# FordyceLab/magnify

Hardware: AMD Instinct MI355X
Metric: megapixels/sec through flatfield+segment+ROI-reduce; markers/sec (higher is better)
Workload: dtype u16

## Files before the change

### include/magnify_hip.h

```cpp
#ifndef MAGNIFY_HIP_H
#define MAGNIFY_HIP_H

#include <stddef.h>
#include <stdint.h>

#ifdef __cplusplus
extern "C" {
#endif

#define MG_OK 0
#define MG_EINVAL (-1)
#define MG_ELAUNCH (-2)
#define MG_EIO (-3)

#define MG_U8 0
#define MG_U16 1
#define MG_F32 2
#define MG_F64 3

#define MG_NO_EDGE 100.0f
#define MG_SCORE_SKIPPED (-2.0f)


int mg_version(void);


int mg_circle_points(int r, int four_connected, int32_t* out_rc, int cap);
int mg_disk_halfwidths(int r, int32_t* out);
int mg_cv_disk_halfwidths(int r, int32_t* out);
int mg_perimeter_table(int min_r, int max_r, int32_t* out_rc, double* out_expected, int32_t* out_starts, int cap);


int64_t mg_flatfield_max_scratch_floats(int dtype, int ty, int tx);
int mg_flatfield_bound(const void* d_flat, int flat_dtype, int dtype, int ty, int tx, float* d_scratch,
                       int64_t scratch_floats, void* stream);
int mg_flatfield_max(const void* d_tiles, int dtype, int64_t n_tiles, int n_groups, int ty, int tx,
                     double dark, const void* d_dark, int dark_dtype,
                     double flat, const void* d_flat, int flat_dtype,
                     double* d_max2, float* d_scratch, int64_t scratch_floats, void* stream);

int mg_flatfield_is_identity(int dtype, double dark, const void* d_dark, double flat, const void* d_flat);

int mg_flatfield_apply_stitch(const void* d_tiles, int dtype, int64_t n_planes, int n_tile_rows, int n_tile_cols,
                              int ty, int tx, int overlap, int apply_flatfield, int planes_per_group,
                              double dark, const void* d_dark, int dark_dtype,
                              double flat, const void* d_flat, int flat_dtype,
                              const double* d_max2, void* d_image, double* d_minmax, void* stream);

int mg_plane_minmax(const void* d_src, int dtype, int n_planes, int64_t plane_stride, int h, int w,
                    int64_t row_stride, double* d_minmax, void* stream);

int64_t mg_shading_workspace_bytes(int n, int w);
int64_t mg_shading_offset(int n, int w, int field);
int mg_shading_downsample(const void* d_tiles, int dtype, int64_t n, int ty, int tx, int w, float* d_out, void* stream);
int mg_shading_prepare(void* d_ws, int n, int w, void* stream);
int mg_shading_dct2(void* d_ws, int n, int w, const double* d_in, double* d_out, int inverse, void* stream);
int mg_shading_alm_begin(void* d_ws, int n, int w, int get_darkfield, int max_iterations, double mu, double lam_f,
                         double lam_d, double tol, double norm_f, double b_up, void* stream);
int mg_shading_alm_iterate(void* d_ws, int n, int w, int k, int get_darkfield, void* stream);
int mg_shading_reweight(void* d_ws, int n, int w, double epsilon, void* stream);
int mg_shading_upsample(const double* d_flat_w, const double* d_dark_w, int w, int ty, int tx, double* d_partial,
                        float* d_flat, float* d_dark, void* stream);
int mg_shading_apply_stitch(const void* d_tiles, int dtype, int n_fields, int64_t planes_per_field, int n_tile_rows,
                            int n_tile_cols, int ty, int tx, int overlap, const float* d_flat, const float* d_dark,
                            void* d_image, double* d_minmax, void* stream);


int mg_to_uint8_blur(const void* d_src, int dtype, int n_planes, int64_t plane_stride, int h, int w,
                     int64_t row_stride, const double* d_minmax, uint8_t* d_blur, uint8_t* d_u8, void* stream);

int mg_scharr_hist(const uint8_t* d_blur, int n_planes, int h, int w, int mode, const uint32_t* d_base,
                   uint32_t* d_hist, uint32_t* d_scratch, int64_t scratch_words, void* stream);
int64_t mg_scharr_hist_scratch_words(int n_planes, int h, int w, int mode);

int mg_to_uint8_blur_hist(const void* d_src, int dtype, int n_planes, int64_t plane_stride, int h, int w,
                          int64_t row_stride, const double* d_minmax, uint8_t* d_blur, uint8_t* d_u8, uint32_t* d_hist,
                          uint32_t* d_scratch, int64_t scratch_words, void* stream);
int64_t mg_blur_hist_scratch_words(int n_planes, int h, int w);

int mg_edge_thresholds(const uint32_t* d_hist, int n_planes, const int64_t* ranks4, float gamma_low, float gamma_high,
                       int32_t* d_thresh, float* d_quantiles, int32_t* d_unresolved, int32_t* d_state,
                       uint32_t* d_win_base, void* stream);
int mg_edge_thresholds_window(const uint32_t* d_hist_win, int n_planes, int pass, float gamma_low, float gamma_high,
                              int32_t* d_state, uint32_t* d_win_base, int32_t* d_thresh, float* d_quantiles,
                              int32_t* d_unresolved, void* stream);


int mg_canny_nms(const uint8_t* d_blur, int n_planes, int h, int w, const int32_t* d_thresh, uint32_t* d_weak,
                 uint32_t* d_strong, uint32_t* d_class, int64_t words_per_plane, void* stream);

int mg_canny_hysteresis(const uint32_t* d_weak, uint32_t* d_strong, int64_t words_per_plane, int n_planes, int h,
                        int w, uint32_t* d_changed, const uint8_t* d_flags_in, uint8_t* d_flags_out, void* stream);
int mg_hysteresis_tiles(int h, int w, int* tiles_x, int* tiles_y);

int mg_unpack_bits(const uint32_t* d_bits, int64_t words_per_plane, int n_planes, int64_t n_bits, uint8_t* d_out,
                   void* stream);

int64_t mg_edge_grid_scan_words(int n_planes, int h, int w, int grid);
int mg_edge_grid(const uint32_t* d_edge_bits, int64_t words_per_plane, int n_planes, int h, int w, int grid,
                 int32_t* d_cell_counts, int32_t* d_cell_starts, int32_t* d_num_edges, int32_t* d_coords,
                 int64_t coord_cap, uint64_t* d_scan_state, int32_t* d_edge_totals, int phases, void* stream);

int mg_edge_angles(const uint8_t* d_blur, int n_planes, int h, int w, const int32_t* d_coords, int64_t coord_cap,
                   const int32_t* d_num_edges, float* d_angle, void* stream);


int mg_dedup_layout(int h, int w, int min_r, int max_r, int* n_tile_rows, int* n_tile_cols, int64_t* n_layers,
                    int64_t* bitmap_words);

int mg_candidate_circles(const int32_t* d_coords, int64_t coord_cap, const int32_t* d_cell_starts,
                         const int32_t* d_cell_counts, const int32_t* d_num_edges, int n_planes, int h, int w,
                         int grid, const uint64_t* d_seeds, int64_t num_iter, int min_r, int max_r,
                         uint32_t* d_bitmap, int64_t bitmap_words, float* d_raw, void* stream);

int mg_candidate_keys(const int32_t* d_coords, int64_t coord_cap, const int32_t* d_cell_starts,
                      const int32_t* d_cell_counts, const int32_t* d_num_edges, int n_planes, int h, int w, int grid,
                      const uint64_t* d_seeds, int64_t num_iter, int min_r, int max_r, uint32_t* d_keys, float* d_raw,
                      void* stream);

int mg_keys_to_circles(const uint32_t* d_keys, int64_t num_iter, const int32_t* d_cell_starts,
                       const int32_t* d_cell_counts, const int32_t* d_num_edges, int n_planes, int h, int w, int grid,
                       int min_r, int max_r, uint32_t* d_unique_keys, int64_t circle_cap, int32_t* d_tile_ranges,
                       int32_t* d_num_circles, int32_t* d_layer_starts, int counters_clear, void* stream);

int mg_bitmap_to_circles(uint32_t* d_bitmap, int64_t bitmap_words, int n_planes, int h, int w, int min_r,
                         int max_r, int32_t* d_layer_offsets, int32_t* d_circles, int64_t circle_cap,
                         int32_t* d_num_circles, void* stream);

int mg_score_circles(const float* d_angle, const uint32_t* d_edge_bits, const uint32_t* d_class_bits,
                     int64_t words_per_plane, int n_planes, int h, int w, int32_t* d_circles, int64_t circle_cap,
                     const int32_t* d_layer_offsets, const uint32_t* d_unique_keys, const int32_t* d_tile_ranges,
                     int min_r, int max_r, const int32_t* d_per_rc, const double* d_per_expected,
                     const int32_t* d_per_starts, int per_total, float min_roundness, int write_skipped,
                     int dedup_centres, float* d_scores, int32_t* d_alive, int32_t* d_num_alive, int32_t* d_max_rc,
                     int32_t* d_num_scored, void* stream);

int mg_score_keyed_supported(int min_r, int max_r);
int mg_score_pair_table(uint64_t* out_entries, int cap);
int mg_score_pairs(int r, int32_t* out_rc, int cap);
int mg_score_circles_keyed(const uint8_t* d_blur, const float* d_angle, const uint32_t* d_edge_bits,
                           const uint32_t* d_class_bits, int64_t words_per_plane, int n_planes, int h, int w,
                           int32_t* d_circles, int64_t circle_cap, const uint32_t* d_unique_keys,
                           const int32_t* d_layer_starts, int min_r, int max_r, const int32_t* d_per_rc,
                           const double* d_per_expected, const int32_t* d_per_starts, int per_total,
                           const uint64_t* d_pair_table, float min_roundness, int write_skipped, float* d_scores,
                           int32_t* d_alive, int32_t* d_num_alive, int32_t* d_max_rc, int32_t* d_num_scored,
                           int32_t* d_surv_list, int64_t surv_cap, int32_t* d_num_surv, int counters_clear,
                           void* stream);

int mg_nms_rounds(const int32_t* d_circles, int64_t circle_cap, const float* d_scores, const int32_t* d_alive,
                  const int32_t* d_num_alive, const int32_t* d_max_rc, int n_planes, int min_dist,
                  const int32_t* d_ring_rc, int ring_len, uint64_t* d_grid, int64_t grid_cap, uint8_t* d_state,
                  int32_t* d_undecided, int64_t undecided_stride, int n_rounds, int counters_clear,
                  const uint32_t* d_tie_keys, int64_t max_alive, const int32_t* d_skip, void* stream);

int mg_nms_same_centre(const int32_t* d_circles, int64_t circle_cap, const float* d_scores, const int32_t* d_alive,
                       const int32_t* d_num_alive, const int32_t* d_max_rc, int n_planes, int min_dist, uint64_t* d_grid,
                       int64_t grid_cap, uint8_t* d_state, const uint32_t* d_tie_keys, int64_t max_alive,
                       const int32_t* d_skip, void* stream);

int mg_nms_cleanup(const int32_t* d_circles, int64_t circle_cap, const float* d_scores, const int32_t* d_alive,
                   const int32_t* d_num_alive, const int32_t* d_max_rc, int n_planes, int min_dist,
                   const int32_t* d_ring_rc, int ring_len, uint64_t* d_grid, int64_t grid_cap, uint8_t* d_state,
                   int64_t max_alive, const int32_t* d_skip, void* stream);

int mg_nms_sparse(const int32_t* d_circles, int64_t circle_cap, const float* d_scores, const int32_t* d_alive,
                  const int32_t* d_num_alive, const int32_t* d_max_rc, int n_planes, int min_dist, const uint32_t* d_dbits,
                  uint8_t* d_state, const uint32_t* d_tie_keys, int32_t* d_done, void* stream);
int mg_nms_sparse_max_dist(void);

int mg_collect_circles(const int32_t* d_circles, int64_t circle_cap, const float* d_scores, const int32_t* d_alive,
                       const int32_t* d_num_alive, const uint8_t* d_state, int keep_all, int n_planes,
                       int32_t* d_out, float* d_out_scores, int64_t out_cap, int32_t* d_num_out,
                       int32_t* d_scratch, const uint32_t* d_tie_keys, int counters_clear, void* stream);


int mg_circle_labels(const int32_t* d_beads, int64_t bead_cap, const int32_t* d_num_beads, int n_planes, int h,
                     int w, const int32_t* d_halfwidths, int max_r, int32_t* d_labels, int reset, void* stream);

int mg_roi_gather_reduce(const void* d_image, int dtype, int n_c, int n_t, int h, int w, const int32_t* d_beads,
                         int m, int roi_len, const int32_t* d_labels, void* d_roi, uint8_t* d_fg, uint8_t* d_bg,
                         double* d_sums, int32_t* d_counts, void* stream);

int mg_roi_gather_reduce_batched(const void* d_image, int dtype, int64_t assay_stride, int n_c, int n_t, int h, int w,
                                 const int32_t* d_beads, const int32_t* d_marker_assay,
                                 const int32_t* d_marker_local, int m, int roi_len, const int32_t* d_labels,
                                 void* d_roi, uint8_t* d_fg, uint8_t* d_bg, double* d_sums, int32_t* d_counts,
                                 void* stream);

int mg_counts_to_offsets(const int32_t* d_counts, int n, int cap, int32_t* d_offsets, void* stream);

int mg_marker_table(const int32_t* d_beads, int64_t bead_stride, const int32_t* d_assay_offsets, int n_assays, int m,
                    int assay_offset, const int32_t* d_counts, const double* d_sums, int n_c, int n_t, int t_index,
                    double* d_table, void* stream);

int mg_roi_segment_reduce(const void* d_image, int dtype, int64_t assay_stride, int n_c, int n_t, int h, int w,
                          int time_major, const int32_t* d_beads, int64_t bead_stride, const int32_t* d_assay_offsets,
                          int n_assays, int m, const int32_t* d_order, int roi_len, const int32_t* d_halfwidths, int max_r,
                          void* d_roi, uint8_t* d_fg, uint8_t* d_bg, double* d_sums, int32_t* d_counts, void* stream);

int mg_roi_window_order(const int32_t* d_beads, int64_t bead_stride, const int32_t* d_assay_offsets, int n_assays, int m,
                        int32_t* d_order, void* stream);

int mg_roi_masked_median(const void* d_roi, int dtype, const uint8_t* d_mask, int64_t mask_stride_m,
                         int64_t mask_stride_t, int m, int n_c, int n_t, int roi_len, double* d_median, void* stream);
int mg_roi_masked_median_u16(const uint16_t* d_roi, const uint8_t* d_mask, int m, int n_c, int n_t, int roi_len,
                             double* d_median, void* stream);


int mg_cluster1d_costs(const double* d_sorted_points, int n_points, int n_offsets, int n_clusters,
                       double cluster_length, const double* d_ideal, double penalty, double* d_costs, void* stream);

int mg_button_masks(const int32_t* d_centers, const int32_t* d_radii, int m, int roi_len, int outer_r, int inner_r,
                    const int32_t* d_cv_halfwidths, int hw_stride, int max_table_r, uint8_t* d_fg, uint8_t* d_bg,
                    void* stream);

int mg_masked_sums(const void* d_roi, int dtype, const uint8_t* d_fg, const uint8_t* d_bg, int m, int n_ct,
                   int roi_len, double* d_sums, int32_t* d_counts, void* stream);


int mg_stream_probe(const void* d_src, void* d_dst, int64_t n_bytes, int mode, uint32_t* d_sink, int blocks, void* stream);


int mg_host_read_runs(const int32_t* fds, const int64_t* offsets, const int64_t* nbytes, void* const* dsts, int n,
                      int n_threads, int64_t* failed);
int mg_host_write_runs(const int32_t* fds, const int64_t* offsets, const int64_t* nbytes, void* const* srcs, int n,
                       int n_threads, int64_t* failed);

#ifdef __cplusplus
}
#endif
#endif
```

### magnify_amd/csrc/mg_flatfield.hip

```cpp
#include <math.h>

#include "mg_common.h"

namespace {

template <typename T>
struct VecOf;
template <>
struct VecOf<uint8_t> {
  static constexpr int N = 16;
};
template <>
struct VecOf<uint16_t> {
  static constexpr int N = 8;
};
template <>
struct VecOf<float> {
  static constexpr int N = 4;
};
template <>
struct VecOf<double> {
  static constexpr int N = 2;
};

template <typename T, int N>
__device__ __forceinline__ void load_vec(const T* p, T (&v)[N]) {
  if ((reinterpret_cast<uintptr_t>(p) & 15) == 0) {
    const uint4 raw = *reinterpret_cast<const uint4*>(p);
    __builtin_memcpy(v, &raw, 16);
  } else {
#pragma unroll
    for (int j = 0; j < N; ++j) v[j] = p[j];
  }
}
template <typename T, int N>
__device__ __forceinline__ void store_vec(T* p, const T (&v)[N]) {
  if ((reinterpret_cast<uintptr_t>(p) & 15) == 0) {
    uint4 raw;
    __builtin_memcpy(&raw, v, 16);
    *reinterpret_cast<uint4*>(p) = raw;
  } else {
#pragma unroll
    for (int j = 0; j < N; ++j) p[j] = v[j];
  }
}

typedef uint32_t mg_u32x4 __attribute__((ext_vector_type(4)));
template <typename T, int N>
__device__ __forceinline__ void load_vec16(const T* p, T (&v)[N], bool nt) {
  const mg_u32x4* q = reinterpret_cast<const mg_u32x4*>(p);
  const mg_u32x4 raw = nt ? __builtin_nontemporal_load(q) : *q;
  __builtin_memcpy(v, &raw, 16);
}
template <typename T, int N>
__device__ __forceinline__ void store_vec16(T* p, const T (&v)[N], bool nt) {
  mg_u32x4 raw;
  __builtin_memcpy(&raw, v, 16);
  mg_u32x4* q = reinterpret_cast<mg_u32x4*>(p);
  if (nt) __builtin_nontemporal_store(raw, q);
  else *q = raw;
}

template <typename T>
__device__ __forceinline__ T cast_trunc(double v);
template <>
__device__ __forceinline__ uint8_t cast_trunc<uint8_t>(double v) {
  return (uint8_t)(unsigned int)v;
}
template <>
__device__ __forceinline__ uint16_t cast_trunc<uint16_t>(double v) {
  return (uint16_t)(unsigned int)v;
}
template <>
__device__ __forceinline__ float cast_trunc<float>(double v) {
  return (float)v;
}
template <>
__device__ __forceinline__ double cast_trunc<double>(double v) {
  return v;
}

template <typename T>
struct IsIntegral {
  static constexpr bool value = false;
};
template <>
struct IsIntegral<uint8_t> {
  static constexpr bool value = true;
};
template <>
struct IsIntegral<uint16_t> {
  static constexpr bool value = true;
};

__device__ __forceinline__ void block_atomic_max2(double m1, double m2, double* out) {
  __shared__ double s1[16], s2[16];
  m1 = mg_wave_nanmax(m1);
  m2 = mg_wave_nanmax(m2);
  const int lane = threadIdx.x & 63, wave = threadIdx.x >> 6;
  if (lane == 0) {
    s1[wave] = m1;
    s2[wave] = m2;
  }
  __syncthreads();
  if (threadIdx.x == 0) {
    const int nw = (blockDim.x + 63) >> 6;
    for (int i = 1; i < nw; ++i) {
      m1 = mg_nanmax(m1, s1[i]);
      m2 = mg_nanmax(m2, s2[i]);
    }
    mg_atomic_nanmax(out, m1);
    mg_atomic_nanmax(out + 1, m2);
  }
}

__device__ __forceinline__ bool flat_in_range(double fl) { return fl > 1e-30 && fl < 1e30; }

__device__ __forceinline__ void max_step(double t, double fl, bool fast_m2, double& m1, double& m2) {
  m1 = mg_nanmax(m1, t);
  if (fast_m2) return;
  if (flat_in_range(fl) && t == t) {
    if (t == 0.0) {
      m2 = mg_nanmax(m2, 0.0);
      return;
    }
    const double qa = t * (double)__builtin_amdgcn_rcpf((float)fl);
    if (m2 == m2 && qa < m2 * (1.0 - 1e-6)) return;
  }
  m2 = mg_nanmax(m2, t / fl);
}

template <int N>
__device__ __forceinline__ void load_field(const void* __restrict__ img, int dt, int64_t p, double scalar,
                                           double (&out)[N]) {
  if (!img) {
#pragma unroll
    for (int j = 0; j < N; ++j) out[j] = scalar;
  } else if (dt == MG_F32) {
    const float* f = (const float*)img + p;
    if ((N % 4) == 0 && (reinterpret_cast<uintptr_t>(f) & 15) == 0) {
#pragma unroll
      for (int q = 0; q < N / 4; ++q) {
        const float4 v = reinterpret_cast<const float4*>(f)[q];
        out[4 * q] = v.x;
        out[4 * q + 1] = v.y;
        out[4 * q + 2] = v.z;
        out[4 * q + 3] = v.w;
      }
    } else {
#pragma unroll
      for (int j = 0; j < N; ++j) out[j] = f[j];
    }
  } else {
    const double* d = (const double*)img + p;
#pragma unroll
    for (int j = 0; j < N; ++j) out[j] = d[j];
  }
}

template <typename T>
__global__ __launch_bounds__(256) void k_flatfield_max(const T* __restrict__ tiles, int64_t tiles_per_group,
                                                        int64_t tile_elems, double dark,
                                                        const void* __restrict__ d_dark, int dark_dt, double flat,
                                                        const void* __restrict__ d_flat, int flat_dt,
                                                        double* __restrict__ out) {
  constexpr int N = VecOf<T>::N;
  const int group = blockIdx.y;
  tiles += (int64_t)group * tiles_per_group * tile_elems;
  out += 2 * group;
  const bool fast_m2 = (d_flat == nullptr) && (flat > 0.0);
  double m1 = -INFINITY, m2 = -INFINITY;
  const int64_t nvec = tile_elems / N;
  const int64_t stride = (int64_t)gridDim.x * blockDim.x;
  for (int64_t v = (int64_t)blockIdx.x * blockDim.x + threadIdx.x; v < nvec; v += stride) {
    double dk[N], fl[N];
    load_field<N>(d_dark, dark_dt, v * N, dark, dk);
    load_field<N>(d_flat, flat_dt, v * N, flat, fl);
    for (int64_t g = 0; g < tiles_per_group; ++g) {
      T x[N];
      load_vec<T, N>(tiles + g * tile_elems + v * N, x);
#pragma unroll
      for (int j = 0; j < N; ++j) {
        double t = (double)x[j] - dk[j];
        t = t < 0.0 ? 0.0 : t;
        max_step(t, fl[j], fast_m2, m1, m2);
      }
    }
  }
  for (int64_t p = nvec * N + (int64_t)blockIdx.x * blockDim.x + threadIdx.x; p < tile_elems; p += stride) {
    const double dk = d_dark ? mg_load_f64(d_dark, dark_dt, p) : dark;
    const double fl = d_flat ? mg_load_f64(d_flat, flat_dt, p) : flat;
    for (int64_t g = 0; g < tiles_per_group; ++g) {
      double t = (double)tiles[g * tile_elems + p] - dk;
      t = t < 0.0 ? 0.0 : t;
      max_step(t, fl, fast_m2, m1, m2);
    }
  }
  if (fast_m2) m2 = (m1 == -INFINITY) ? m1 : m1 / flat;
  block_atomic_max2(m1, m2, out);
// ... 125 lines not shown
  constexpr int N = VecOf<T>::N;
  constexpr int UV = 2;
  const int group = blockIdx.y;
  tiles += (int64_t)group * tiles_per_group * tile_elems;
  out += 2 * group;
  const float dk_f = (float)dark;
  uint32_t xmax = 0;
  bool any = false;
  double m2 = -INFINITY;
  float thr = -INFINITY;
  const int64_t nvec = tile_elems / N;
  const int64_t stride = (int64_t)gridDim.x * blockDim.x;
  const int64_t vend = nvec;
  constexpr int PUBLISHERS = 32;
  float gthr = -INFINITY;
  int trip = 0;
  const bool publish = SHARE && blockIdx.x < PUBLISHERS && (int64_t)(blockIdx.x + 1) * blockDim.x <= nvec;
  for (int64_t v0 = (int64_t)blockIdx.x * blockDim.x + threadIdx.x; v0 < nvec; v0 += UV * stride) {
    float rcm[UV];
#pragma unroll
    for (int u = 0; u < UV; ++u) rcm[u] = d_rcmax[min(v0 + u * stride, nvec - 1)];
    if (SHARE && trip > 0 && (trip & (trip - 1)) == 0) {
      const double gm = __hip_atomic_load(out + 1, __ATOMIC_RELAXED, __HIP_MEMORY_SCOPE_AGENT);
      if (gm == gm && gm < 1e30 && gm > -INFINITY) gthr = fmaxf(gthr, (float)gm * (1.0f - 1e-5f));
    }
    any = true;
    for (int64_t g0 = 0; g0 < tiles_per_group; g0 += 4) {
      T x4[UV][4][N];
#pragma unroll
      for (int u = 0; u < UV; ++u)
#pragma unroll
        for (int q = 0; q < 4; ++q)
          load_vec16<T, N>(tiles + min(g0 + q, tiles_per_group - 1) * tile_elems + min(v0 + u * stride, nvec - 1) * N, x4[u][q],
                           true);
#pragma unroll
      for (int u = 0; u < UV; ++u) {
        const int64_t v = v0 + u * stride;
        if (v >= vend) break;
#pragma unroll
        for (int q = 0; q < 4; ++q) {
          if (g0 + q >= tiles_per_group) break;
          uint32_t cm = 0;
#pragma unroll
          for (int j = 0; j < N; ++j) cm = max(cm, (uint32_t)x4[u][q][j]);
          xmax = max(xmax, cm);
          const float tf = fmaxf((float)cm - dk_f, 0.0f);
          if (rcm[u] >= 0.0f && tf * rcm[u] <= fmaxf(thr, gthr)) continue;
          float fl[N];
#pragma unroll
          for (int k4 = 0; k4 < N / 4; ++k4) {
            const float4 f = reinterpret_cast<const float4*>(d_flat + v * N)[k4];
            fl[4 * k4] = f.x, fl[4 * k4 + 1] = f.y, fl[4 * k4 + 2] = f.z, fl[4 * k4 + 3] = f.w;
          }
#pragma unroll
          for (int j = 0; j < N; ++j) {
            const uint32_t xi = (uint32_t)x4[u][q][j];
            const float t_f = fmaxf((float)xi - dk_f, 0.0f);
            const bool in_range = fl[j] > 1e-30f && fl[j] < 1e30f;
            if (in_range && t_f * __builtin_amdgcn_rcpf(fl[j]) <= fmaxf(thr, gthr)) continue;
            double t = (double)xi - dark;
            t = t < 0.0 ? 0.0 : t;
            m2 = mg_nanmax(m2, t / (double)fl[j]);
            thr = (m2 == m2 && m2 < 1e30) ? (float)m2 * (1.0f - 1e-5f) : -INFINITY;
          }
        }
      }
    }
    if (trip == 0 && publish) {
      const double wm = mg_wave_nanmax(m2);
      if ((threadIdx.x & 63) == 0 && wm == wm && wm > -INFINITY) mg_atomic_nanmax(out + 1, wm);
    }
    ++trip;
  }
  double m1 = -INFINITY;
  if (any) {
    m1 = (double)xmax - dark;
    m1 = m1 < 0.0 ? 0.0 : m1;
  }
  block_atomic_max2(m1, m2, out);
}

constexpr int ROWS_PER_BLOCK = 32;

__device__ __forceinline__ double refined_rcp(double fl) {
  if (!flat_in_range(fl)) return 0.0;
  double r = (double)__builtin_amdgcn_rcpf((float)fl);
  r = r * (2.0 - fl * r);
  r = r * (2.0 - fl * r);
  return r;
}

template <typename T>
__device__ __forceinline__ T correct_pixel(double t, double fl, double r, double m1, double m2, double k, bool fast_ok) {
  if (IsIntegral<T>::value && fast_ok && r != 0.0) {
    if (t == 0.0) return (T)0;
    const double v = t * r * k;
    const double fv = floor(v);
    const double fr = v - fv;
    if (fr > 1e-6 && fr < 1.0 - 1e-6 && v < 4.0e9) return (T)(unsigned int)fv;
  }
  double e = t / fl;
  e = e * m1;
  e = e / m2;
  return cast_trunc<T>(e);
}

template <typename T, int N>
__device__ __forceinline__ void correct_chunk(const T (&x)[N], const double (&dk)[N], const double (&fl)[N],
                                              const double (&r)[N], double m1, double m2, double k, bool fast_ok, T (&o)[N]) {
  double t[N];
  bool unsure = !fast_ok || !IsIntegral<T>::value;
#pragma unroll
  for (int j = 0; j < N; ++j) {
    t[j] = (double)x[j] - dk[j];
    t[j] = t[j] < 0.0 ? 0.0 : t[j];
    if (!IsIntegral<T>::value) continue;
    const double v = t[j] * r[j] * k;
    const double fv = floor(v);
    const double fr = v - fv;
    o[j] = (T)(unsigned int)fv;
    unsure |= !((fr > 1e-6 && fr < 1.0 - 1e-6 && v < 4.0e9) || t[j] == 0.0) || r[j] == 0.0;
  }
  if (unsure) {
#pragma unroll
    for (int j = 0; j < N; ++j) {
      double e = t[j] / fl[j];
      e = e * m1;
      e = e / m2;
      o[j] = cast_trunc<T>(e);
    }
  }
}

constexpr int PLANES_PER_BLOCK = 8;

template <typename T, bool APPLY>
__global__ __launch_bounds__(256) void k_apply_stitch(const T* __restrict__ tiles, int n_planes, int n_tr, int n_tc,
                                                       int ty, int tx, int clip, int hy, int hx, int planes_per_group,
                                                       double dark, const void* __restrict__ d_dark, int dark_dt,
                                                       double flat, const void* __restrict__ d_flat, int flat_dt,
                                                       const double* __restrict__ d_max2, T* __restrict__ image,
                                                       double* __restrict__ d_minmax, int rows_per_block) {
  constexpr int N = VecOf<T>::N;
  constexpr int PB = PLANES_PER_BLOCK;
  const int plane0 = blockIdx.z * PB;
  const int np = min(PB, n_planes - plane0);
  const int h_out = n_tr * hy, w_out = n_tc * hx;
  const int ox0 = (blockIdx.x * blockDim.x + threadIdx.x) * N;
  double m1[PB], m2[PB], kk[PB];
  bool fast_ok[PB];
#pragma unroll
  for (int b = 0; b < PB; ++b) {
    m1[b] = 0.0, m2[b] = 1.0, kk[b] = 1.0, fast_ok[b] = false;
    if (APPLY && b < np) {
      const int group = (plane0 + b) / planes_per_group;
      m1[b] = d_max2[2 * group];
      m2[b] = d_max2[2 * group + 1];
      kk[b] = m1[b] / m2[b];
      fast_ok[b] = kk[b] > 0.0 && kk[b] < 1e30 && m1[b] > 0.0 && m1[b] < 1e300 && m2[b] > 0.0 && m2[b] < 1e300;
    }
  }
  double vmin[PB], vmax[PB];
  uint32_t imin[PB], imax[PB];
#pragma unroll
  for (int b = 0; b < PB; ++b) vmin[b] = INFINITY, vmax[b] = -INFINITY, imin[b] = 0xFFFFFFFFu, imax[b] = 0u;
  const int64_t tile_elems = (int64_t)ty * tx;
  if (ox0 < w_out)
  for (int yg = blockIdx.y; yg * rows_per_block < h_out; yg += gridDim.y) {
    const int row_end = min((yg + 1) * rows_per_block, h_out);
    const int tc0 = ox0 / hx;
    const int x0 = ox0 - tc0 * hx + clip;
    const bool one_tile = (ox0 + N <= w_out) && (x0 - clip + N <= hx);
    for (int oy = yg * rows_per_block; oy < row_end; ++oy) {
      const int tr = oy / hy;
      const int y = oy - tr * hy + clip;
      int64_t pix[N], toff[N];
      const int cnt = one_tile ? N : min(N, w_out - ox0);
#pragma unroll
      for (int j = 0; j < N; ++j) {
        const int ox = ox0 + (one_tile ? j : min(j, cnt - 1));
        const int tc = one_tile ? tc0 : ox / hx;
        const int xx = one_tile ? x0 + j : ox - tc * hx + clip;
        pix[j] = (int64_t)y * tx + xx;
        toff[j] = ((int64_t)tr * n_tc + tc) * tile_elems;
      }
      double dk[N], fl[N], rr[N];
      if (APPLY) {
        if (one_tile) {
          load_field<N>(d_dark, dark_dt, pix[0], dark, dk);
          load_field<N>(d_flat, flat_dt, pix[0], flat, fl);
        } else {
#pragma unroll
          for (int j = 0; j < N; ++j) {
            dk[j] = d_dark ? mg_load_f64(d_dark, dark_dt, pix[j]) : dark;
            fl[j] = d_flat ? mg_load_f64(d_flat, flat_dt, pix[j]) : flat;
          }
        }
#pragma unroll
        for (int j = 0; j < N; ++j) rr[j] = IsIntegral<T>::value ? refined_rcp(fl[j]) : 0.0;
      }
#pragma unroll
      for (int b = 0; b < PB; ++b) {
        if (b >= np) break;
        const int64_t plane_base = (int64_t)(plane0 + b) * n_tr * n_tc * tile_elems;
        T x[N], o[N];
        if (one_tile) {
          load_vec<T, N>(tiles + plane_base + toff[0] + pix[0], x);
        } else {
#pragma unroll
          for (int j = 0; j < N; ++j) x[j] = tiles[plane_base + toff[j] + pix[j]];
        }
#pragma unroll
        for (int j = 0; j < N; ++j) {
          if (APPLY) {
            double t = (double)x[j] - dk[j];
            t = t < 0.0 ? 0.0 : t;
            o[j] = correct_pixel<T>(t, fl[j], rr[j], m1[b], m2[b], kk[b], fast_ok[b]);
          } else {
            o[j] = x[j];
          }
          if (d_minmax && j < cnt) {
            if (IsIntegral<T>::value) {
              imin[b] = min(imin[b], (uint32_t)o[j]);
              imax[b] = max(imax[b], (uint32_t)o[j]);
            } else {
              const double ov = (double)o[j];
              vmin[b] = mg_nanmin(vmin[b], ov);
              vmax[b] = mg_nanmax(vmax[b], ov);
            }
          }
        }
        T* dst = image + ((int64_t)(plane0 + b) * h_out + oy) * w_out + ox0;
        if (cnt == N) {
          store_vec<T, N>(dst, o);
        } else {
          for (int j = 0; j < cnt; ++j) dst[j] = o[j];
        }
      }
    }
  }
  if (d_minmax) mg_block_minmax<PB>(vmin, vmax, imin, imax, np, d_minmax, plane0);
}

__device__ __forceinline__ double uniform_f64(double v) {
  const unsigned long long u = (unsigned long long)__double_as_longlong(v);
  const uint32_t lo = __builtin_amdgcn_readfirstlane((uint32_t)u), hi = __builtin_amdgcn_readfirstlane((uint32_t)(u >> 32));
  return __longlong_as_double((long long)(((unsigned long long)hi << 32) | lo));
}

typedef unsigned short mg_u16x2 __attribute__((ext_vector_type(2)));
template <typename T, int N>
__device__ __forceinline__ void sub_dark_int(const T (&x)[N], uint32_t d, uint32_t (&ti)[N]) {
#pragma unroll
  for (int j = 0; j < N; ++j) {
    const uint32_t xi = (uint32_t)x[j];
    ti[j] = xi > d ? xi - d : 0u;
  }
}
template <>
__device__ __forceinline__ void sub_dark_int<uint16_t, 8>(const uint16_t (&x)[8], uint32_t d, uint32_t (&ti)[8]) {
  uint32_t w[4];
  __builtin_memcpy(w, x, 16);
  const mg_u16x2 dd = {(unsigned short)d, (unsigned short)d};
#pragma unroll
  for (int q = 0; q < 4; ++q) {
    const mg_u16x2 r = __builtin_elementwise_sub_sat(__builtin_bit_cast(mg_u16x2, w[q]), dd);
    ti[2 * q] = r.x;
    ti[2 * q + 1] = r.y;
  }
}

template <typename T, int N>
__device__ __forceinline__ bool fast_chunk_int(const uint32_t (&ti)[N], const double (&rk)[N], T (&o)[N]) {
  bool unsure = false;
#pragma unroll
  for (int j = 0; j < N; ++j) {
    const double v = (double)ti[j] * rk[j];
    const double fr = __builtin_amdgcn_fract(v);
    o[j] = (T)(unsigned int)v;
    unsure |= !(fr > 1e-6 && fr < 1.0 - 1e-6) && ti[j] != 0u;
  }
  return unsure;
}
template <typename T, int N>
__device__ __forceinline__ bool fast_chunk_f64(const double (&t)[N], const double (&rk)[N], T (&o)[N]) {
  bool unsure = false;
#pragma unroll
  for (int j = 0; j < N; ++j) {
    const double v = t[j] * rk[j];
    const double fr = __builtin_amdgcn_fract(v);
    o[j] = (T)(unsigned int)v;
    unsure |= !(fr > 1e-6 && fr < 1.0 - 1e-6) && t[j] != 0.0;
  }
  return unsure;
}

template <typename T, bool APPLY, bool INT_DARK>
__global__ __launch_bounds__(256) void k_apply_stitch_aligned(const T* __restrict__ tiles, int n_planes, int n_tr,
                                                               int n_tc, int ty, int tx, int clip, int hy, int hx,
                                                               int planes_per_group, double dark,
                                                               const void* __restrict__ d_dark, int dark_dt,
                                                               double flat, const void* __restrict__ d_flat,
                                                               int flat_dt, const double* __restrict__ d_max2,
                                                               T* __restrict__ image, double* __restrict__ d_minmax,
                                                               int rows_per_block) {
  constexpr int N = VecOf<T>::N;
  constexpr int PB = PLANES_PER_BLOCK;
  int bx = blockIdx.x, by = blockIdx.y, bz = blockIdx.z;
  if (APPLY && gridDim.z >= 16 && ((gridDim.x * gridDim.y) & 7) == 0) {
    const uint32_t lin = blockIdx.x + gridDim.x * (blockIdx.y + gridDim.y * blockIdx.z);
    const uint32_t xcd = lin & 7, slot = lin >> 3;
    bz = slot % gridDim.z;
    const uint32_t xy = (slot / gridDim.z) * 8 + xcd;
    bx = xy % gridDim.x;
    by = xy / gridDim.x;
  }
  const int plane0 = bz * PB;
  const int np = min(PB, n_planes - plane0);
  const int h_out = n_tr * hy, w_out = n_tc * hx;
  const int ox0 = (bx * blockDim.x + threadIdx.x) * N;
  uint32_t imin[PB], imax[PB];
#pragma unroll
  for (int b = 0; b < PB; ++b) imin[b] = 0xFFFFFFFFu, imax[b] = 0u;
  const int64_t tile_elems = (int64_t)ty * tx, plane_elems = (int64_t)n_tr * n_tc * tile_elems;
  double kka[PB];
  uint32_t ok_mask = 0;
#pragma unroll
  for (int b = 0; b < PB; ++b) {
    kka[b] = 1.0;
    if (APPLY && b < np) {
      const int group = (plane0 + b) / planes_per_group;
      const double m1 = d_max2[2 * group], m2 = d_max2[2 * group + 1];
      const double kk = m1 / m2;
      kka[b] = uniform_f64(kk);
      const bool ok = kk > 0.0 && kk < 1e30 && m1 > 0.0 && m1 < 1e300 && m2 > 0.0 && m2 < 1e300;
      ok_mask |= ok ? (1u << b) : 0u;
    }
  }
  ok_mask = __builtin_amdgcn_readfirstlane(ok_mask);
  const uint32_t dark_i = INT_DARK ? (uint32_t)dark : 0u;
  if (ox0 < w_out)
  for (int yg = by; yg * rows_per_block < h_out; yg += gridDim.y) {
    const int row_end = min((yg + 1) * rows_per_block, h_out);
    const int tc0 = ox0 / hx;
    const int x0 = ox0 - tc0 * hx + clip;
    for (int oy = yg * rows_per_block; oy < row_end; ++oy) {
      const int tr = oy / hy;
      const int64_t p0 = (int64_t)(oy - tr * hy + clip) * tx + x0;
      const int64_t src0 = ((int64_t)tr * n_tc + tc0) * tile_elems + p0;
      double dk[N], fl[N], rr[N];
      bool flat_bad = false;
      if (APPLY) {
        if (!INT_DARK) load_field<N>(d_dark, dark_dt, p0, dark, dk);
        load_field<N>(d_flat, flat_dt, p0, flat, fl);
#pragma unroll
        for (int j = 0; j < N; ++j) {
          rr[j] = refined_rcp(fl[j]);
          flat_bad |= rr[j] == 0.0;
        }
      }
      T xin[PB][N];
#pragma unroll
      for (int b = 0; b < PB; ++b)
        if (b < np) load_vec16<T, N>(tiles + (int64_t)(plane0 + b) * plane_elems + src0, xin[b], false);
      double rk[N];
      double kk_of_rk = -1.0;
      bool rk_large = true;
#pragma unroll
      for (int b = 0; b < PB; ++b) {
        if (b >= np) break;
        T o[N];
        T(&x)[N] = xin[b];
        if (APPLY) {
          if (kka[b] != kk_of_rk) {
            kk_of_rk = kka[b];
            rk_large = false;
#pragma unroll
            for (int j = 0; j < N; ++j) {
              rk[j] = rr[j] * kk_of_rk;
              rk_large |= !(rk[j] < 61035.0);
            }
          }
          const bool rk_bad = rk_large || flat_bad || !((ok_mask >> b) & 1u);
          bool unsure;
          uint32_t ti[N];
          double t[N];
          if (INT_DARK) {
            sub_dark_int<T, N>(x, dark_i, ti);
            unsure = fast_chunk_int<T, N>(ti, rk, o);
          } else {
#pragma unroll
            for (int j = 0; j < N; ++j) {
              t[j] = (double)x[j] - dk[j];
              t[j] = t[j] < 0.0 ? 0.0 : t[j];
            }
            unsure = fast_chunk_f64<T, N>(t, rk, o);
          }
          if (unsure || rk_bad) {
            const int group = (plane0 + b) / planes_per_group;
            const double m1 = d_max2[2 * group], m2 = d_max2[2 * group + 1];
#pragma unroll
            for (int j = 0; j < N; ++j) {
              const double tj = INT_DARK ? (double)ti[j] : t[j];
              double e = tj / fl[j];
              e = e * m1;
              e = e / m2;
              o[j] = cast_trunc<T>(e);
            }
          }
        } else {
#pragma unroll
          for (int j = 0; j < N; ++j) o[j] = x[j];
        }
        if (d_minmax) {
#pragma unroll
          for (int j = 0; j < N; ++j) {
            imin[b] = min(imin[b], (uint32_t)o[j]);
            imax[b] = max(imax[b], (uint32_t)o[j]);
          }
        }
        store_vec16<T, N>(image + ((int64_t)(plane0 + b) * h_out + oy) * w_out + ox0, o, false);
      }
    }
  }
  if (d_minmax) mg_block_minmax_u32<PB>(imin, imax, np, d_minmax, plane0);
}

template <typename T>
__global__ __launch_bounds__(256) void k_plane_minmax(const T* __restrict__ src, int64_t plane_stride, int h, int w,
                                                       int64_t row_stride, double* __restrict__ d_minmax) {
  constexpr int N = VecOf<T>::N;
  const int plane = blockIdx.y;
  const T* base = src + (int64_t)plane * plane_stride;
  double vmin = INFINITY, vmax = -INFINITY;
  uint32_t imin = 0xFFFFFFFFu, imax = 0u;
  const int vec_per_row = (w + N - 1) / N;
  const int64_t total = (int64_t)h * vec_per_row;
  const int64_t stride = (int64_t)gridDim.x * blockDim.x;
  int64_t i = (int64_t)blockIdx.x * blockDim.x + threadIdx.x;
  if (IsIntegral<T>::value && w % N == 0 && (reinterpret_cast<uintptr_t>(base) & 15) == 0 && (row_stride * (int64_t)sizeof(T)) % 16 == 0) {
    for (; i < total; i += 4 * stride) {
      T x[4][N];
#pragma unroll
      for (int q = 0; q < 4; ++q) {
        const int64_t iq = min(i + q * stride, total - 1);
        const int r = (int)(iq / vec_per_row);
        const int c0 = (int)(iq - (int64_t)r * vec_per_row) * N;
        load_vec16<T, N>(base + (int64_t)r * row_stride + c0, x[q], false);
      }
#pragma unroll
      for (int q = 0; q < 4; ++q)
#pragma unroll
        for (int j = 0; j < N; ++j) {
          imin = min(imin, (uint32_t)x[q][j]);
          imax = max(imax, (uint32_t)x[q][j]);
        }
    }
    i = total;
  }
  for (; i < total; i += stride) {
    const int r = (int)(i / vec_per_row);
    const int c0 = (int)(i - (int64_t)r * vec_per_row) * N;
    const T* p = base + (int64_t)r * row_stride + c0;
    if (c0 + N <= w) {
      T x[N];
      load_vec<T, N>(p, x);
#pragma unroll
      for (int j = 0; j < N; ++j) {
        vmin = mg_nanmin(vmin, (double)x[j]);
        vmax = mg_nanmax(vmax, (double)x[j]);
      }
    } else {
      for (int j = 0; c0 + j < w; ++j) {
        vmin = mg_nanmin(vmin, (double)p[j]);
        vmax = mg_nanmax(vmax, (double)p[j]);
      }
    }
  }
  mg_block_minmax<1>(&vmin, &vmax, &imin, &imax, 1, d_minmax, plane);
}

template <typename T>
int launch_max(const void* d_tiles, int64_t tiles_per_group, int n_groups, int64_t tile_elems, double dark,
               const void* d_dark, int dark_dt, double flat, const void* d_flat, int flat_dt, double* d_max2,
               float* d_scratch, int64_t scratch_floats, hipStream_t s) {
  if (tiles_per_group == 0 || n_groups == 0 || tile_elems == 0) return MG_OK;
  const int64_t nvec = tile_elems / VecOf<T>::N + 1;
  const int per_group = std::min(512, std::max(1, 4096 / n_groups));
  int blocks = (int)std::min<int64_t>((nvec + 255) / 256, per_group);
  const int64_t group_elems = tiles_per_group * tile_elems;
  if (IsIntegral<T>::value && !d_dark && !d_flat && flat > 0.0 && flat < 1e300 && fabs(dark) < 1e300 &&
      (reinterpret_cast<uintptr_t>(d_tiles) & 15) == 0 && (group_elems * (int64_t)sizeof(T)) % 16 == 0) {
    const int64_t gvec = group_elems / VecOf<T>::N;
    const int gb = (int)std::max<int64_t>(1, std::min<int64_t>(gvec / 256, std::min(512, std::max(64, 2048 / n_groups))));
    hipLaunchKernelGGL((k_flatfield_max_int<T>), dim3(gb, n_groups), dim3(256), 0, s, (const T*)d_tiles, group_elems, dark,
                       flat, d_max2);
    MG_CHECK_LAUNCH();
    return MG_OK;
  }
  if (IsIntegral<T>::value && !d_dark && d_flat && flat_dt == MG_F32 && tile_elems % VecOf<T>::N == 0 &&
      (reinterpret_cast<uintptr_t>(d_flat) & 15) == 0 && (reinterpret_cast<uintptr_t>(d_tiles) & 15) == 0 &&
      fabs(dark) < 16777216.0 && (double)(float)dark == dark) {
    constexpr int N = VecOf<T>::N;
    if (d_scratch && scratch_floats >= tile_elems / N && (reinterpret_cast<uintptr_t>(d_scratch) & 3) == 0) {
      const int64_t cvec = tile_elems / N;
      const int per = (int)std::max<int64_t>(1, std::min<int64_t>((cvec + 255) / 256, std::max(1, 1536 / n_groups)));
      const int64_t chunks_per_lane = (cvec + (int64_t)per * 256 - 1) / ((int64_t)per * 256) * tiles_per_group;
      if (chunks_per_lane < 512)
        hipLaunchKernelGGL((k_flatfield_max_lean<T, true>), dim3(per, n_groups), dim3(256), 0, s, (const T*)d_tiles,
                           tiles_per_group, tile_elems, dark, (const float*)d_flat, d_scratch, d_max2);
      else
        hipLaunchKernelGGL((k_flatfield_max_lean<T, false>), dim3(per, n_groups), dim3(256), 0, s, (const T*)d_tiles,
                           tiles_per_group, tile_elems, dark, (const float*)d_flat, d_scratch, d_max2);
      MG_CHECK_LAUNCH();
      return MG_OK;
    }
    hipLaunchKernelGGL((k_flatfield_max_fast<T>), dim3(blocks, n_groups), dim3(256), 0, s, (const T*)d_tiles,
                       tiles_per_group, tile_elems, dark, (const float*)d_flat, d_max2);
    MG_CHECK_LAUNCH();
    return MG_OK;
  }
  hipLaunchKernelGGL((k_flatfield_max<T>), dim3(blocks, n_groups), dim3(256), 0, s, (const T*)d_tiles, tiles_per_group,
                     tile_elems, dark, d_dark, dark_dt, flat, d_flat, flat_dt, d_max2);
  MG_CHECK_LAUNCH();
  return MG_OK;
}

template <typename T>
int launch_apply(const void* d_tiles, int64_t n_planes, int n_tr, int n_tc, int ty, int tx, int overlap, int apply,
                 int planes_per_group, double dark, const void* d_dark, int dark_dt, double flat, const void* d_flat, int flat_dt,
                 const double* d_max2, void* d_image, double* d_minmax, hipStream_t s) {
  const auto [clip, hy, hx, h_out, w_out] = mg_stitch_geom(ty, tx, overlap, n_tr, n_tc);
  if (n_planes == 0 || h_out == 0 || w_out == 0) return MG_OK;
  constexpr int N = VecOf<T>::N;
  if (n_planes > 0x7FFFFFF0) return MG_EINVAL;
  int rows = ROWS_PER_BLOCK;
  const int64_t cols_planes = (int64_t)((w_out + 256 * N - 1) / (256 * N)) * ((n_planes + PLANES_PER_BLOCK - 1) / PLANES_PER_BLOCK);
  while (rows > 2 && cols_planes * ((h_out + rows - 1) / rows) < 2048) rows /= 2;
  int y_blocks = (h_out + rows - 1) / rows;
  if (rows < ROWS_PER_BLOCK) y_blocks = (int)std::min<int64_t>(y_blocks, std::max<int64_t>(1, 1024 / std::max<int64_t>(1, cols_planes)));
  dim3 grid((w_out + 256 * N - 1) / (256 * N), y_blocks,
            (unsigned)((n_planes + PLANES_PER_BLOCK - 1) / PLANES_PER_BLOCK));
  if (grid.y > 65535 || grid.z > 65535) return MG_EINVAL;
  const bool aligned = IsIntegral<T>::value && hx % N == 0 && tx % N == 0 && clip % N == 0 &&
                       (reinterpret_cast<uintptr_t>(d_tiles) & 15) == 0 && (reinterpret_cast<uintptr_t>(d_image) & 15) == 0 &&
                       (!d_flat || (reinterpret_cast<uintptr_t>(d_flat) & 15) == 0) &&
                       (!d_dark || (reinterpret_cast<uintptr_t>(d_dark) & 15) == 0);
  if (aligned) {
    const bool int_dark = apply && !d_dark && dark >= 0.0 && dark <= 65535.0 && dark == (double)(uint32_t)dark;
#define MG_ALIGNED(AP, ID) \
    hipLaunchKernelGGL((k_apply_stitch_aligned<T, AP, ID>), grid, dim3(256), 0, s, (const T*)d_tiles, (int)n_planes, n_tr, \
                       n_tc, ty, tx, clip, hy, hx, planes_per_group, dark, d_dark, dark_dt, flat, d_flat, flat_dt, \
                       d_max2, (T*)d_image, d_minmax, rows)
    if (!apply)
      MG_ALIGNED(false, false);
    else if (int_dark)
      MG_ALIGNED(true, true);
    else
      MG_ALIGNED(true, false);
#undef MG_ALIGNED
    MG_CHECK_LAUNCH();
    return MG_OK;
  }
  if (apply)
    hipLaunchKernelGGL((k_apply_stitch<T, true>), grid, dim3(256), 0, s, (const T*)d_tiles, (int)n_planes, n_tr, n_tc,
                       ty, tx, clip, hy, hx, planes_per_group, dark, d_dark, dark_dt, flat, d_flat, flat_dt, d_max2,
                       (T*)d_image, d_minmax, rows);
  else
    hipLaunchKernelGGL((k_apply_stitch<T, false>), grid, dim3(256), 0, s, (const T*)d_tiles, (int)n_planes, n_tr, n_tc,
                       ty, tx, clip, hy, hx, planes_per_group, dark, d_dark, dark_dt, flat, d_flat, flat_dt, d_max2,
                       (T*)d_image, d_minmax, rows);
  MG_CHECK_LAUNCH();
  return MG_OK;
}

template <typename T>
int launch_minmax(const void* d_src, int n_planes, int64_t plane_stride, int h, int w, int64_t row_stride,
                  double* d_minmax, hipStream_t s) {
  if (n_planes == 0 || h == 0 || w == 0) return MG_OK;
  const int64_t total = (int64_t)h * ((w + VecOf<T>::N - 1) / VecOf<T>::N);
  int bx = (int)std::min<int64_t>((total + 255) / 256, 1024);
  hipLaunchKernelGGL((k_plane_minmax<T>), dim3(bx, n_planes), dim3(256), 0, s, (const T*)d_src, plane_stride, h, w,
                     row_stride, d_minmax);
  MG_CHECK_LAUNCH();
  return MG_OK;
}

bool df_dtype_ok(const void* p, int dt) { return p == nullptr || dt == MG_F32 || dt == MG_F64; }

}

extern "C" int mg_version(void) { return 1; }

extern "C" int64_t mg_flatfield_max_scratch_floats(int dtype, int ty, int tx) {
  if (ty <= 0 || tx <= 0) return -1;
  const int n = dtype == MG_U8 ? 16 : dtype == MG_U16 ? 8 : 0;
  return n ? ((int64_t)ty * tx + n - 1) / n : 0;
}

extern "C" int mg_flatfield_bound(const void* d_flat, int flat_dtype, int dtype, int ty, int tx, float* d_scratch,
                                  int64_t scratch_floats, void* stream) {
  if (!d_flat || !d_scratch || ty <= 0 || tx <= 0 || flat_dtype != MG_F32) return MG_EINVAL;
  const int64_t need = mg_flatfield_max_scratch_floats(dtype, ty, tx);
  const int64_t tile_elems = (int64_t)ty * tx;
  const int n = dtype == MG_U8 ? 16 : dtype == MG_U16 ? 8 : 0;
  if (need <= 0 || scratch_floats < need || tile_elems % n || (reinterpret_cast<uintptr_t>(d_flat) & 15) ||
      (reinterpret_cast<uintptr_t>(d_scratch) & 3))
    return MG_EINVAL;
  hipStream_t s = mg_stream(stream);
  const int64_t cvec = tile_elems / n;
  const dim3 grid((unsigned)std::min<int64_t>((cvec + 255) / 256, 2048));
  if (n == 16)
    hipLaunchKernelGGL((k_flat_rcmax<16>), grid, dim3(256), 0, s, (const float*)d_flat, cvec, d_scratch);
  else
    hipLaunchKernelGGL((k_flat_rcmax<8>), grid, dim3(256), 0, s, (const float*)d_flat, cvec, d_scratch);
  MG_CHECK_LAUNCH();
  return MG_OK;
}

extern "C" int mg_flatfield_max(const void* d_tiles, int dtype, int64_t n_tiles, int n_groups, int ty, int tx,
                                double dark, const void* d_dark, int dark_dtype, double flat, const void* d_flat,
                                int flat_dtype, double* d_max2, float* d_scratch, int64_t scratch_floats, void* stream) {
  if (!d_tiles || !d_max2 || n_tiles < 0 || ty <= 0 || tx <= 0 || n_groups <= 0 || n_groups > 65535) return MG_EINVAL;
  if (n_tiles % n_groups) return MG_EINVAL;
  if (!df_dtype_ok(d_dark, dark_dtype) || !df_dtype_ok(d_flat, flat_dtype)) return MG_EINVAL;
  const int64_t tile_elems = (int64_t)ty * tx, tpg = n_tiles / n_groups;
  hipStream_t s = mg_stream(stream);
  return mg_dispatch_pixel(dtype, [&](auto t) {
    return launch_max<decltype(t)>(d_tiles, tpg, n_groups, tile_elems, dark, d_dark, dark_dtype, flat, d_flat, flat_dtype,
                                   d_max2, d_scratch, scratch_floats, s);
  });
}

extern "C" int mg_flatfield_is_identity(int dtype, double dark, const void* d_dark, double flat, const void* d_flat) {
  return (dtype == MG_U8 || dtype == MG_U16) && !d_dark && !d_flat && dark == 0.0 && flat == 1.0;
}

extern "C" int mg_flatfield_apply_stitch(const void* d_tiles, int dtype, int64_t n_planes, int n_tile_rows,
                                         int n_tile_cols, int ty, int tx, int overlap, int apply_flatfield,
                                         int planes_per_group, double dark, const void* d_dark, int dark_dtype,
                                         double flat, const void* d_flat, int flat_dtype, const double* d_max2,
                                         void* d_image, double* d_minmax, void* stream) {
  if (!d_tiles || !d_image || n_planes < 0 || n_tile_rows <= 0 || n_tile_cols <= 0 || ty <= 0 || tx <= 0)
    return MG_EINVAL;
  if (overlap < 0 || overlap >= ty || overlap >= tx) return MG_EINVAL;
  if (apply_flatfield && mg_flatfield_is_identity(dtype, dark, d_dark, flat, d_flat)) apply_flatfield = 0;
  if (apply_flatfield && (!d_max2 || planes_per_group <= 0)) return MG_EINVAL;
  if (!df_dtype_ok(d_dark, dark_dtype) || !df_dtype_ok(d_flat, flat_dtype)) return MG_EINVAL;
  hipStream_t s = mg_stream(stream);
  return mg_dispatch_pixel(dtype, [&](auto t) {
    return launch_apply<decltype(t)>(d_tiles, n_planes, n_tile_rows, n_tile_cols, ty, tx, overlap, apply_flatfield,
                                     planes_per_group > 0 ? planes_per_group : 1, dark, d_dark, dark_dtype, flat, d_flat,
                                     flat_dtype, d_max2, d_image, d_minmax, s);
  });
}

extern "C" int mg_plane_minmax(const void* d_src, int dtype, int n_planes, int64_t plane_stride, int h, int w,
                               int64_t row_stride, double* d_minmax, void* stream) {
  if (!d_src || !d_minmax || n_planes < 0 || h < 0 || w < 0) return MG_EINVAL;
  if (n_planes > 65535) return MG_EINVAL;
  hipStream_t s = mg_stream(stream);
  return mg_dispatch_pixel(dtype, [&](auto t) {
    return launch_minmax<decltype(t)>(d_src, n_planes, plane_stride, h, w, row_stride, d_minmax, s);
  });
}
```

### magnify_amd/csrc/mg_roi.hip

```cpp
#include <math.h>

#include <stdlib.h>

#include "mg_common.h"

namespace {

constexpr int NT = 256;

__global__ __launch_bounds__(NT) void k_circle_labels(const int32_t* __restrict__ d_beads, int64_t bead_cap,
                                                      const int32_t* __restrict__ d_num_beads, int h, int w,
                                                      const int32_t* __restrict__ d_halfwidths, int max_r,
                                                      int32_t* __restrict__ d_labels, int reset) {
  const int plane = blockIdx.y;
  const int i = blockIdx.x;
  if (i >= d_num_beads[plane]) return;
  const int32_t* b = d_beads + ((int64_t)plane * bead_cap + i) * 3;
  const int row = b[0], col = b[1], r = b[2];
  if (r < 2 || r > max_r) return;
  const int32_t* hw = d_halfwidths + (int64_t)r * (2 * max_r + 1);
  int32_t* lab = d_labels + (int64_t)plane * h * w;
  const int side = 2 * r + 1;
  for (int p = threadIdx.x; p < side * side; p += NT) {
    const int dy = p / side - r, dx = p % side - r;
    if (abs(dx) > hw[dy + r]) continue;
    const int y = row + dy, x = col + dx;
    if (y < 0 || y >= h || x < 0 || x >= w) continue;
    int32_t* cell = &lab[(int64_t)y * w + x];
    if (reset) {
      *cell = -1;
      continue;
    }
    const int old = atomicCAS(cell, -1, i);
    if (old != -1 && old != i) *cell = -2;
  }
}

__device__ __forceinline__ void window(int c, int len, int size, int& lo) {
  c = min(max(c, -(1 << 28)), 1 << 28);
  int a = c - len / 2, b = c + (len - len / 2);
  if (a < 0) {
    b -= a;
    a = 0;
  }
  if (b > size) a -= b - size;
  lo = a;
}

struct DiskMasks {
  uint32_t* any;
  uint32_t* multi;
  uint32_t* own;
  int wpr;
  __device__ __forceinline__ void flags(int ry, int rx, uint32_t& f, uint32_t& b) const {
    const int i = ry * wpr + (rx >> 5), sh = rx & 31;
    f = ((own[i] & ~multi[i]) >> sh) & 1u;
    b = (~any[i] >> sh) & 1u;
  }
};

__device__ __forceinline__ void mask_row(const DiskMasks& m, int ry, int xa, int xb, bool is_own) {
  for (int wd = xa >> 5; wd <= (xb >> 5); ++wd) {
    const int lo = max(xa, 32 * wd) - 32 * wd, hi = min(xb, 32 * wd + 31) - 32 * wd;
    const uint32_t bits = (hi - lo == 31) ? 0xFFFFFFFFu : (((1u << (hi - lo + 1)) - 1u) << lo);
    const uint32_t old = atomicOr(&m.any[ry * m.wpr + wd], bits);
    if (old & bits) atomicOr(&m.multi[ry * m.wpr + wd], old & bits);
    if (is_own) atomicOr(&m.own[ry * m.wpr + wd], bits);
  }
}
__device__ __forceinline__ void mask_disk_row(const DiskMasks& m, int ry, int len, int top, int left, int yj, int xj,
                                              int rj, bool is_own, const int32_t* __restrict__ hwtab, int max_r) {
  const int dy = top + ry - yj;
  if (dy < -rj || dy > rj) return;
  const int hwid = hwtab[(int64_t)rj * (2 * max_r + 1) + dy + rj];
  if (hwid < 0) return;
  const int xa = max(xj - hwid, left) - left, xb = min(xj + hwid, left + len - 1) - left;
  if (xa <= xb) mask_row(m, ry, xa, xb, is_own);
}

constexpr int NBR_CAP = 96;

__device__ __forceinline__ DiskMasks build_disk_masks(uint32_t* base, int len, int top, int left,
                                                      const int32_t* __restrict__ beads, int nb, int local,
                                                      const int32_t* __restrict__ hwtab, int max_r) {
  __shared__ int s_nn;
  __shared__ int s_nbr[NBR_CAP][3];
  DiskMasks m;
// ... 91 lines not shown
  const int cy = d_beads[3 * gb], cx = d_beads[3 * gb + 1];
  int top, left;
  window(cy, len, h, top);
  window(cx, len, w, left);
  const int n = len * len;
  const int lane = threadIdx.x & 63, wave = threadIdx.x >> 6;
  const int32_t* lab = d_labels ? d_labels + (int64_t)assay * h * w : nullptr;
  DiskMasks dm{};
  if (d_halfwidths)
    dm = build_disk_masks(reinterpret_cast<uint32_t*>(flags + ((n + 3) & ~3)), len, top, left,
                          d_beads + 3 * bead0, d_assay_offsets[assay + 1] - first, local, d_halfwidths, max_r);
  int cf = 0, cb = 0;
  for (int p = threadIdx.x; p < n; p += NT) {
    const int ry = p / len, rx = p - ry * len;
    uint8_t f = 0, b = 0;
    if (d_halfwidths) {
      uint32_t ff, bb;
      dm.flags(ry, rx, ff, bb);
      f = (uint8_t)ff;
      b = (uint8_t)bb;
    } else if (lab) {
      const int v = lab[(int64_t)(top + ry) * w + (left + rx)];
      f = v == local;
      b = v == -1;
    }
    flags[p] = f | (b << 1);
    if (d_fg) d_fg[(int64_t)g * n + p] = f;
    if (d_bg) d_bg[(int64_t)g * n + p] = b;
    cf += f;
    cb += b;
  }
  cf = mg_wave_sum_i32(cf);
  cb = mg_wave_sum_i32(cb);
  if (lane == 0) {
    s_cnt[0][wave] = cf;
    s_cnt[1][wave] = cb;
  }
  __syncthreads();
  if (threadIdx.x == 0 && d_counts) {
    d_counts[2 * (int64_t)g] = s_cnt[0][0] + s_cnt[0][1] + s_cnt[0][2] + s_cnt[0][3];
    d_counts[2 * (int64_t)g + 1] = s_cnt[1][0] + s_cnt[1][1] + s_cnt[1][2] + s_cnt[1][3];
  }
  const T* img = d_image + (int64_t)assay * assay_stride;
  for (int ct = 0; ct < n_c * n_t; ++ct) {
    const T* plane = img + (int64_t)(time_major ? (ct % n_t) * n_c + ct / n_t : ct) * h * w;
    T* out = d_roi ? d_roi + ((int64_t)g * n_c * n_t + ct) * n : nullptr;
    ACC sf = 0, sb = 0;
    for (int p = threadIdx.x; p < n; p += NT) {
      const int ry = p / len, rx = p - ry * len;
      const T v = plane[(int64_t)(top + ry) * w + (left + rx)];
      if (out) out[p] = v;
      const uint8_t fl = flags[p];
      if (fl & 1) sf += (ACC)v;
      if (fl & 2) sb += (ACC)v;
    }
    if (d_sums) {
#pragma unroll
      for (int off = 32; off > 0; off >>= 1) {
        sf += __shfl_xor(sf, off);
        sb += __shfl_xor(sb, off);
      }
      __syncthreads();
      if (lane == 0) {
        s_red[0][wave] = sf;
        s_red[1][wave] = sb;
      }
      __syncthreads();
      if (threadIdx.x == 0) {
        double* o = d_sums + ((int64_t)g * n_c * n_t + ct) * 2;
        o[0] = (double)(s_red[0][0] + s_red[0][1] + s_red[0][2] + s_red[0][3]);
        o[1] = (double)(s_red[1][0] + s_red[1][1] + s_red[1][2] + s_red[1][3]);
      }
    }
  }
}

typedef unsigned short roi_us2 __attribute__((ext_vector_type(2)));

__device__ __forceinline__ uint32_t roi_dot2(uint32_t v, uint32_t m, uint32_t acc) {
  return __builtin_amdgcn_udot2(__builtin_bit_cast(roi_us2, v), __builtin_bit_cast(roi_us2, m), acc, false);
}
__device__ __forceinline__ uint32_t roi_pair(uint32_t b) { return (b & 1u) | ((b & 2u) << 15); }

template <int U, int CTB, bool PIPE>
__global__ __launch_bounds__(NT) void k_roi_u16_even(const uint16_t* __restrict__ d_image, int64_t assay_stride,
                                                     int n_c, int n_t, int h, int w,
                                                     const int32_t* __restrict__ d_beads,
                                                     const int32_t* __restrict__ d_marker_assay,
                                                     const int32_t* __restrict__ d_marker_local, int len,
                                                     const int32_t* __restrict__ d_labels,
                                                     const int32_t* __restrict__ d_assay_offsets, int n_assays, int64_t bead_stride, int time_major,
                                                     const int32_t* __restrict__ d_order,
                                                     const int32_t* __restrict__ d_halfwidths, int max_r,
                                                     uint16_t* __restrict__ d_roi, uint8_t* __restrict__ d_fg,
                                                     uint8_t* __restrict__ d_bg, double* __restrict__ d_sums,
                                                     int32_t* __restrict__ d_counts) {
  extern __shared__ __attribute__((aligned(4))) uint8_t smem[];
  constexpr int WV = NT / 64;
  __shared__ uint32_t s_red[2][CTB][WV];
  __shared__ int s_cnt[2][WV];
  int g = blockIdx.x, assay, first = 0, local;
  int64_t bead0 = 0, gb = g;
  if (d_assay_offsets) {
    if (g >= d_assay_offsets[n_assays]) return;
    if (d_order) g = d_order[g];
    int lo = 0, hi = n_assays;
    while (hi - lo > 1) {
      const int mid = (lo + hi) >> 1;
      if (d_assay_offsets[mid] <= g) lo = mid;
      else hi = mid;
    }
    assay = lo;
    first = d_assay_offsets[assay];
    local = g - first;
    bead0 = bead_stride ? (int64_t)assay * bead_stride : first;
    gb = bead0 + local;
  } else {
    assay = d_marker_assay ? d_marker_assay[g] : 0;
    local = d_marker_local ? d_marker_local[g] : g;
  }
  int top, left;
  window(d_beads[3 * gb], len, h, top);
  window(d_beads[3 * gb + 1], len, w, left);
  const int n = len * len, half = len >> 1;
  const int lane = threadIdx.x & 63, wave = threadIdx.x >> 6;
  const int x = 2 * lane;
  const bool act = lane < half;
  const int wpr = (len + 31) >> 5, words = len * wpr;
  uint32_t* base = reinterpret_cast<uint32_t*>(smem);
  uint32_t* fgw = base + 2 * words;
  uint32_t* bgw = base;
  int cf = 0, cb = 0;
  if (d_halfwidths) {
    const DiskMasks dm = build_disk_masks(base, len, top, left, d_beads + 3 * bead0, d_assay_offsets[assay + 1] - first,
                                          local, d_halfwidths, max_r);
    for (int i = threadIdx.x; i < words; i += NT) {
      const int wd = i % wpr;
      const uint32_t valid = (len - 32 * wd >= 32) ? 0xFFFFFFFFu : ((1u << (len - 32 * wd)) - 1u);
      const uint32_t f = dm.own[i] & ~dm.multi[i], b = ~dm.any[i] & valid;
      fgw[i] = f;
      bgw[i] = b;
      cf += __popc(f);
      cb += __popc(b);
    }
  } else {
    for (int i = threadIdx.x; i < 3 * words; i += NT) base[i] = 0u;
    __syncthreads();
    if (d_labels) {
      const int32_t* lab = d_labels + (int64_t)assay * h * w;
      for (int ry = wave; ry < len; ry += WV) {
        if (!act) continue;
        const int32_t* lp = lab + (int64_t)(top + ry) * w + left + x;
        const int v0 = lp[0], v1 = lp[1];
        const uint32_t f = (uint32_t)(v0 == local) | ((uint32_t)(v1 == local) << 1);
        const uint32_t b = (uint32_t)(v0 == -1) | ((uint32_t)(v1 == -1) << 1);
        if (f) atomicOr(&fgw[ry * wpr + (x >> 5)], f << (x & 31));
        if (b) atomicOr(&bgw[ry * wpr + (x >> 5)], b << (x & 31));
        cf += __popc(f);
        cb += __popc(b);
      }
    }
  }
  cf = mg_wave_sum_i32(cf);
  cb = mg_wave_sum_i32(cb);
  if (lane == 0) {
    s_cnt[0][wave] = cf;
    s_cnt[1][wave] = cb;
  }
  __syncthreads();
  if (threadIdx.x == 0 && d_counts) {
    d_counts[2 * (int64_t)g] = s_cnt[0][0] + s_cnt[0][1] + s_cnt[0][2] + s_cnt[0][3];
    d_counts[2 * (int64_t)g + 1] = s_cnt[1][0] + s_cnt[1][1] + s_cnt[1][2] + s_cnt[1][3];
  }
  const int mword = x >> 5, msh = x & 31;
  if (d_fg || d_bg) {
    for (int ry = wave; ry < len; ry += WV) {
      if (!act) continue;
      const uint32_t f = (fgw[ry * wpr + mword] >> msh) & 3u, b = (bgw[ry * wpr + mword] >> msh) & 3u;
      if (d_fg) *reinterpret_cast<uint16_t*>(&d_fg[(int64_t)g * n + ry * len + x]) = (uint16_t)((f & 1u) | ((f & 2u) << 7));
      if (d_bg) *reinterpret_cast<uint16_t*>(&d_bg[(int64_t)g * n + ry * len + x]) = (uint16_t)((b & 1u) | ((b & 2u) << 7));
    }
  }
  const uint16_t* img = d_image + (int64_t)assay * assay_stride;
  const int nct = n_c * n_t;
  const int odd = left & 1;
  const uint32_t shift = odd ? 16u : 0u;
  const uint32_t lidx = (uint32_t)min(lane, half - 1 + odd);
  const int64_t plane_elems = (int64_t)h * w;
  for (int ct0 = 0; ct0 < nct; ct0 += CTB) {
    const uint32_t* plane[CTB];
    uint32_t* out[CTB];
#pragma unroll
    for (int c = 0; c < CTB; ++c) {
      const int ct = min(ct0 + c, nct - 1);
      plane[c] = reinterpret_cast<const uint32_t*>(img + (int64_t)(time_major ? (ct % n_t) * n_c + ct / n_t : ct) * plane_elems);
      out[c] = d_roi ? reinterpret_cast<uint32_t*>(d_roi + ((int64_t)g * nct + ct) * n) : nullptr;
    }
    uint32_t sf[CTB], sb[CTB];
#pragma unroll
    for (int c = 0; c < CTB; ++c) sf[c] = 0u, sb[c] = 0u;
    auto load_rows = [&](int r0, uint32_t (&dd)[U][CTB]) {
#pragma unroll
      for (int u = 0; u < U; ++u) {
        const int ry = min(r0 + u * WV, len - 1);
        const uint32_t di = (uint32_t)(((top + ry) * w + left - odd) >> 1) + lidx;
#pragma unroll
        for (int c = 0; c < CTB; ++c) dd[u][c] = plane[c][di];
      }
    };
    uint32_t dd[U][CTB], dn[U][CTB];
    load_rows(wave, dd);
    for (int r0 = wave; r0 < len; r0 += WV * U) {
      if (PIPE) {
        load_rows(r0 + WV * U, dn);
      }
#pragma unroll
      for (int u = 0; u < U; ++u) {
        const int ry = r0 + u * WV;
        if (ry >= len) break;
        const uint32_t mf = roi_pair((fgw[ry * wpr + mword] >> msh) & 3u), mb = roi_pair((bgw[ry * wpr + mword] >> msh) & 3u);
        const uint32_t oi = (uint32_t)(ry * half + lane);
#pragma unroll
        for (int c = 0; c < CTB; ++c) {
          if (ct0 + c >= nct) break;
          const uint32_t d = dd[u][c];
          const uint32_t nx = (uint32_t)__builtin_amdgcn_update_dpp(0, (int)d, 0x130, 0xF, 0xF, false);
          const uint32_t v = __builtin_amdgcn_alignbit(nx, d, shift);
          if (act) {
            if (out[c]) out[c][oi] = v;
            sf[c] = roi_dot2(v, mf, sf[c]);
            sb[c] = roi_dot2(v, mb, sb[c]);
          }
        }
      }
      if (PIPE) {
#pragma unroll
        for (int u = 0; u < U; ++u)
#pragma unroll
          for (int c = 0; c < CTB; ++c) dd[u][c] = dn[u][c];
      } else if (r0 + WV * U < len) {
        load_rows(r0 + WV * U, dd);
      }
    }
    if (d_sums) {
#pragma unroll
      for (int c = 0; c < CTB; ++c) {
        const uint32_t a = (uint32_t)mg_wave_scan_incl_i32((int)sf[c]), b = (uint32_t)mg_wave_scan_incl_i32((int)sb[c]);
        if (lane == 63) {
          s_red[0][c][wave] = a;
          s_red[1][c][wave] = b;
        }
      }
      __syncthreads();
      if ((int)threadIdx.x < 2 * CTB) {
        const int k = threadIdx.x & 1, c = threadIdx.x >> 1;
        if (ct0 + c < nct) {
          uint32_t tot = 0;
#pragma unroll
          for (int q = 0; q < WV; ++q) tot += s_red[k][c][q];
          d_sums[((int64_t)g * nct + ct0 + c) * 2 + k] = (double)tot;
        }
      }
      __syncthreads();
    }
  }
}

constexpr int RT_H = 16, RT_W = 384, RT_WPR = RT_W / 32;
constexpr int RT_CT = 4;
constexpr int RT_F = 16;
constexpr int RT_IDS = 2048;
constexpr int RTN = 512;
constexpr int RT_DISKS = 128;

struct RtFrag {
  int g;
  int top, left;
  int yj, xj, rj;
  int r0, r1;
};

__global__ __launch_bounds__(RTN) void k_roi_tiles_u16(const uint16_t* __restrict__ d_image, int64_t assay_stride, int n_c,
                                                      int n_t, int h, int w, const int32_t* __restrict__ d_beads,
                                                      int64_t bead_stride, const int32_t* __restrict__ d_assay_offsets,
                                                      int time_major, int len, const int32_t* __restrict__ d_halfwidths,
                                                      int max_r, uint16_t* __restrict__ d_roi, uint8_t* __restrict__ d_fg,
                                                      uint8_t* __restrict__ d_bg, double* __restrict__ d_sums,
                                                      int32_t* __restrict__ d_counts) {
  extern __shared__ __attribute__((aligned(16))) uint8_t rt_smem[];
  uint32_t* s_tile = reinterpret_cast<uint32_t*>(rt_smem);
  uint32_t* s_any = s_tile + RT_CT * RT_H * (RT_W / 2);
  uint32_t* s_multi = s_any + RT_H * RT_WPR;
  uint32_t* s_fg = s_multi + RT_H * RT_WPR;
  uint32_t* s_bg = s_fg + RT_F * RT_H * 4;
  uint16_t* s_ids = reinterpret_cast<uint16_t*>(s_bg + RT_F * RT_H * 4);
  int32_t* s_hw = reinterpret_cast<int32_t*>(s_ids + RT_IDS);
  __shared__ int s_nfrag, s_ndisk;
  __shared__ int s_disk[RT_DISKS][3];
  __shared__ RtFrag s_frag[RT_F];
  __shared__ int s_cnt[RT_F][2];
  const int assay = blockIdx.z, tx0 = blockIdx.x * RT_W, ty0 = blockIdx.y * RT_H;
  const int tw = min(RT_W, w - tx0), th = min(RT_H, h - ty0);
  const int first = d_assay_offsets[assay], nb = d_assay_offsets[assay + 1] - first;
  if (nb <= 0) return;
  const int32_t* beads = d_beads + 3 * (bead_stride ? (int64_t)assay * bead_stride : (int64_t)first);
  const int lane = threadIdx.x & 63, wave = threadIdx.x >> 6;
  constexpr int WV = RTN / 64;
  for (int i = threadIdx.x; i < 2 * RT_H * RT_WPR; i += RTN) s_any[i] = 0u;
  for (int i = threadIdx.x; i < (max_r + 1) * (2 * max_r + 1); i += RTN) s_hw[i] = d_halfwidths[i];
  if (threadIdx.x == 0) s_nfrag = 0, s_ndisk = 0;
  __syncthreads();
  const int side = 2 * max_r + 1;
  auto draw_row = [&](int r, int yj, int xj, int rj) {
    const int dy = ty0 + r - yj;
    if (dy < -rj || dy > rj) return;
    const int hwid = s_hw[rj * side + dy + rj];
    if (hwid < 0) return;
    const int xa = max(xj - hwid, tx0) - tx0, xb = min(xj + hwid, tx0 + tw - 1) - tx0;
    for (int wd = xa >> 5; xa <= xb && wd <= (xb >> 5); ++wd) {
      const int lo = max(xa, 32 * wd) - 32 * wd, hi = min(xb, 32 * wd + 31) - 32 * wd;
      const uint32_t bits = (hi - lo == 31) ? 0xFFFFFFFFu : (((1u << (hi - lo + 1)) - 1u) << lo);
      const uint32_t old = atomicOr(&s_any[r * RT_WPR + wd], bits);
      if (old & bits) atomicOr(&s_multi[r * RT_WPR + wd], old & bits);
    }
// ... 288 lines not shown
      s_bin = b;
      s_rank = rank - acc;
    }
    __syncthreads();
    prefix = (prefix << 8) | (K)s_bin;
    rank = s_rank;
    __syncthreads();
  }
  return prefix;
}

template <typename T>
__global__ __launch_bounds__(NT) void k_masked_median(const T* __restrict__ d_roi, const uint8_t* __restrict__ d_mask,
                                                      int64_t mask_stride_m, int64_t mask_stride_t, int n_t, int n_ct,
                                                      int n, double* __restrict__ d_median) {
  __shared__ uint32_t hist[256];
  __shared__ int s_count;
  const int g = blockIdx.x, ct = blockIdx.y;
  const T* v = d_roi + ((int64_t)g * n_ct + ct) * n;
  const uint8_t* mask = d_mask + (int64_t)g * mask_stride_m + (int64_t)(ct % n_t) * mask_stride_t;
  int c = 0;
  for (int p = threadIdx.x; p < n; p += NT) {
    typename median_key<T>::type key;
    c += mask[p] != 0 && median_key<T>::key(v[p], &key);
  }
  int total;
  mg_block_exscan(c, &total);
  if (threadIdx.x == 0) s_count = total;
  __syncthreads();
  const int cnt = s_count;
  double* out = d_median + (int64_t)g * n_ct + ct;
  if (cnt == 0) {
    if (threadIdx.x == 0) *out = __longlong_as_double(0x7FF8000000000000ll);
    return;
  }
  const auto lo = select_kth<T>(v, mask, n, (cnt - 1) / 2, hist);
  auto hi = lo;
  if ((cnt & 1) == 0) hi = select_kth<T>(v, mask, n, cnt / 2, hist);
  if (threadIdx.x == 0) *out = (median_key<T>::value(lo) + median_key<T>::value(hi)) / 2.0;
}

template <typename T>
int launch_median(const void* d_roi, const uint8_t* d_mask, int64_t sm, int64_t st, int m, int n_c, int n_t, int len,
                  double* d_median, hipStream_t s) {
  hipLaunchKernelGGL((k_masked_median<T>), dim3(m, n_c * n_t), dim3(NT), 0, s, (const T*)d_roi, d_mask, sm, st, n_t,
                     n_c * n_t, len * len, d_median);
  MG_CHECK_LAUNCH();
  return MG_OK;
}

template <typename T, typename ACC>
int launch_roi(const void* d_image, int64_t assay_stride, int n_c, int n_t, int h, int w, const int32_t* d_beads,
               const int32_t* d_marker_assay, const int32_t* d_marker_local, dim3 grid, int len,
               const int32_t* d_labels, const int32_t* d_assay_offsets, int n_assays, int64_t bead_stride, int time_major,
               const int32_t* d_order, const int32_t* d_halfwidths,
               int max_r, void* d_roi, uint8_t* d_fg, uint8_t* d_bg, double* d_sums, int32_t* d_counts, hipStream_t s) {
  hipLaunchKernelGGL((k_roi<T, ACC>), grid, dim3(NT), roi_lds_bytes(len, d_halfwidths != nullptr), s,
                     (const T*)d_image, assay_stride, n_c, n_t, h, w, d_beads, d_marker_assay, d_marker_local, len,
                     d_labels, d_assay_offsets, n_assays, bead_stride, time_major, d_order, d_halfwidths, max_r, (T*)d_roi, d_fg, d_bg, d_sums, d_counts);
  MG_CHECK_LAUNCH();
  return MG_OK;
}

}

extern "C" int mg_circle_labels(const int32_t* d_beads, int64_t bead_cap, const int32_t* d_num_beads, int n_planes,
                                int h, int w, const int32_t* d_halfwidths, int max_r, int32_t* d_labels,
                                int reset, void* stream) {
  if (!d_beads || !d_num_beads || !d_halfwidths || !d_labels || n_planes < 0 || n_planes > 65535 || bead_cap < 0 ||
      max_r < 0)
    return MG_EINVAL;
  if (n_planes == 0 || bead_cap == 0) return MG_OK;
  hipLaunchKernelGGL(k_circle_labels, dim3((unsigned)bead_cap, n_planes), dim3(NT), 0, mg_stream(stream), d_beads,
                     bead_cap, d_num_beads, h, w, d_halfwidths, max_r, d_labels, reset);
  MG_CHECK_LAUNCH();
  return MG_OK;
}

namespace {
int roi_dispatch(const void* d_image, int dtype, int64_t assay_stride, int n_c, int n_t, int h, int w,
                 const int32_t* d_beads, const int32_t* d_marker_assay, const int32_t* d_marker_local, int m, int roi_len,
                 const int32_t* d_labels, const int32_t* d_assay_offsets, int64_t bead_stride, int time_major, int n_assays,
                 const int32_t* d_order, const int32_t* d_halfwidths, int max_r, void* d_roi, uint8_t* d_fg, uint8_t* d_bg,
                 double* d_sums, int32_t* d_counts, void* stream) {
  if (!d_image || !d_beads || m < 0 || roi_len <= 0 || n_c <= 0 || n_t <= 0) return MG_EINVAL;
  if (roi_len > h || roi_len > w || roi_lds_bytes(roi_len, d_halfwidths != nullptr) > 60000) return MG_EINVAL;
  if (m == 0) return MG_OK;
  hipStream_t s = mg_stream(stream);
  const dim3 grid(m);
  const char* tiles_env = getenv("MG_ROI_TILES");
  const bool tiles = tiles_env && tiles_env[0] == '1';
  if (tiles && dtype == MG_U16 && d_halfwidths && d_assay_offsets && !d_labels && (roi_len & 1) == 0 && roi_len <= 126 &&
      (w & 7) == 0 && (assay_stride & 7) == 0 && (int64_t)h * w < (1LL << 31) && n_assays > 0 && n_assays <= 65535 &&
      (bead_stride ? bead_stride : (int64_t)m) <= 65535 && max_r >= 2 && (max_r + 1) * (2 * max_r + 1) * 4 <= 27 * 53 * 4 + 8192 &&
      (reinterpret_cast<uintptr_t>(d_image) & 15) == 0 && (!d_roi || (reinterpret_cast<uintptr_t>(d_roi) & 3) == 0) &&
      (!d_fg || (reinterpret_cast<uintptr_t>(d_fg) & 1) == 0) && (!d_bg || (reinterpret_cast<uintptr_t>(d_bg) & 1) == 0)) {
    const int nct = n_c * n_t;
    if (d_sums && mg_zero_async(d_sums, (size_t)m * nct * 2 * sizeof(double), s) != hipSuccess) return MG_ELAUNCH;
    if (d_counts && mg_zero_async(d_counts, (size_t)m * 2 * sizeof(int32_t), s) != hipSuccess) return MG_ELAUNCH;
    static bool attr_set = false;
    if (!attr_set) {
      if (hipFuncSetAttribute(reinterpret_cast<const void*>(k_roi_tiles_u16), hipFuncAttributeMaxDynamicSharedMemorySize,
                              (int)RT_LDS + 27 * 53 * 4 + 8192) != hipSuccess)
        return MG_ELAUNCH;
      attr_set = true;
    }
    hipLaunchKernelGGL(k_roi_tiles_u16, dim3((w + RT_W - 1) / RT_W, (h + RT_H - 1) / RT_H, n_assays), dim3(RTN), RT_LDS + (size_t)(max_r + 1) * (2 * max_r + 1) * 4, s,
                       (const uint16_t*)d_image, assay_stride, n_c, n_t, h, w, d_beads, bead_stride, d_assay_offsets,
                       time_major, roi_len, d_halfwidths, max_r, (uint16_t*)d_roi, d_fg, d_bg, d_sums, d_counts);
    MG_CHECK_LAUNCH();
    return MG_OK;
  }
  if (dtype == MG_U16 && (roi_len & 1) == 0 && roi_len <= 126 && (w & 1) == 0 && (assay_stride & 1) == 0 &&
      (int64_t)h * w < (1LL << 31) &&
      (reinterpret_cast<uintptr_t>(d_image) & 3) == 0 && (!d_roi || (reinterpret_cast<uintptr_t>(d_roi) & 3) == 0) &&
      (!d_fg || (reinterpret_cast<uintptr_t>(d_fg) & 1) == 0) && (!d_bg || (reinterpret_cast<uintptr_t>(d_bg) & 1) == 0)) {
    hipLaunchKernelGGL((k_roi_u16_even<2, 4, true>), grid, dim3(NT), (size_t)mask_words(roi_len) * 4, s,
                       (const uint16_t*)d_image, assay_stride, n_c, n_t, h, w, d_beads, d_marker_assay, d_marker_local,
                       roi_len, d_labels, d_assay_offsets, n_assays, bead_stride, time_major, d_order, d_halfwidths, max_r, (uint16_t*)d_roi, d_fg, d_bg,
                       d_sums, d_counts);
    MG_CHECK_LAUNCH();
    return MG_OK;
  }
  return mg_dispatch_pixel(dtype, [&](auto t) {
    using T = decltype(t);
    return launch_roi<T, mg_acc_t<T>>(d_image, assay_stride, n_c, n_t, h, w, d_beads, d_marker_assay, d_marker_local, grid,
                                      roi_len, d_labels, d_assay_offsets, n_assays, bead_stride, time_major, d_order,
                                      d_halfwidths, max_r, d_roi, d_fg, d_bg, d_sums, d_counts, s);
  });
}
}

namespace {
__global__ __launch_bounds__(1024) void k_counts_to_offsets(const int32_t* __restrict__ d_counts, int n, int cap,
                                                            int32_t* __restrict__ d_offsets) {
  int carry = 0;
  for (int i0 = 0; i0 < n; i0 += 1024) {
    const int i = i0 + (int)threadIdx.x;
    const int v = i < n ? min(max(d_counts[i], 0), cap) : 0;
    int total;
    const int ex = mg_block_exscan(v, &total);
    if (i < n) d_offsets[i] = carry + ex;
    carry += total;
  }
  if (threadIdx.x == 0) d_offsets[n] = carry;
}
}

extern "C" int mg_counts_to_offsets(const int32_t* d_counts, int n, int cap, int32_t* d_offsets, void* stream) {
  if (!d_counts || !d_offsets || n < 0 || cap < 0) return MG_EINVAL;
  hipLaunchKernelGGL(k_counts_to_offsets, dim3(1), dim3(1024), 0, mg_stream(stream), d_counts, n, cap, d_offsets);
  MG_CHECK_LAUNCH();
  return MG_OK;
}

namespace {
__global__ __launch_bounds__(256) void k_marker_table(const int32_t* __restrict__ d_beads, int64_t bead_stride,
                                                      const int32_t* __restrict__ d_assay_offsets, int n_assays,
                                                      int assay_offset, const int32_t* __restrict__ d_counts,
                                                      const double* __restrict__ d_sums, int n_c, int n_t, int t_index,
                                                      double* __restrict__ d_table) {
  const int total = d_assay_offsets[n_assays];
  const int width = 6 + 2 * n_c;
  for (int g = blockIdx.x * blockDim.x + threadIdx.x; g < total; g += gridDim.x * blockDim.x) {
    int lo = 0, hi = n_assays;
    while (hi - lo > 1) {
      const int mid = (lo + hi) >> 1;
      if (d_assay_offsets[mid] <= g) lo = mid;
      else hi = mid;
    }
    const int local = g - d_assay_offsets[lo];
    const int32_t* b = bead_stride > 0 ? d_beads + ((int64_t)lo * bead_stride + local) * 3 : d_beads + (int64_t)g * 3;
    double* row = d_table + (int64_t)g * width;
    row[0] = (double)(assay_offset + lo);
    row[1] = (double)b[0], row[2] = (double)b[1], row[3] = (double)b[2];
    row[4] = (double)d_counts[2 * g], row[5] = (double)d_counts[2 * g + 1];
    for (int c = 0; c < n_c; ++c) {
      const double* sm = d_sums + (((int64_t)g * n_c + c) * n_t + t_index) * 2;
      row[6 + c] = sm[0];
      row[6 + n_c + c] = sm[1];
    }
  }
}
}

extern "C" int mg_marker_table(const int32_t* d_beads, int64_t bead_stride, const int32_t* d_assay_offsets, int n_assays,
                               int m, int assay_offset, const int32_t* d_counts, const double* d_sums, int n_c, int n_t,
                               int t_index, double* d_table, void* stream) {
  if (!d_assay_offsets || n_assays <= 0 || n_assays > 65535 || m < 0 || bead_stride < 0 || n_c <= 0 || n_t <= 0 ||
      t_index < 0 || t_index >= n_t)
    return MG_EINVAL;
  if (m == 0) return MG_OK;
  if (!d_beads || !d_counts || !d_sums || !d_table) return MG_EINVAL;
  hipLaunchKernelGGL(k_marker_table, dim3((unsigned)std::min((m + 255) / 256, 2048)), dim3(256), 0, mg_stream(stream),
                     d_beads, bead_stride, d_assay_offsets, n_assays, assay_offset, d_counts, d_sums, n_c, n_t, t_index,
                     d_table);
  MG_CHECK_LAUNCH();
  return MG_OK;
}

extern "C" int mg_roi_gather_reduce_batched(const void* d_image, int dtype, int64_t assay_stride, int n_c, int n_t,
                                            int h, int w, const int32_t* d_beads, const int32_t* d_marker_assay,
                                            const int32_t* d_marker_local, int m, int roi_len,
                                            const int32_t* d_labels, void* d_roi, uint8_t* d_fg, uint8_t* d_bg,
                                            double* d_sums, int32_t* d_counts, void* stream) {
  return roi_dispatch(d_image, dtype, assay_stride, n_c, n_t, h, w, d_beads, d_marker_assay, d_marker_local, m, roi_len,
                      d_labels, nullptr, 0, 0, 0, nullptr, nullptr, 0, d_roi, d_fg, d_bg, d_sums, d_counts, stream);
}

namespace {
constexpr int ORDER_CAP = 8192;
constexpr int ORDER_BAND = 6;
constexpr int ORDER_PARTS = 8;

__global__ __launch_bounds__(NT) void k_window_order(const int32_t* __restrict__ d_beads, int64_t bead_stride,
                                                     const int32_t* __restrict__ d_assay_offsets, int m,
                                                     int32_t* __restrict__ d_order) {
  __shared__ __attribute__((aligned(16))) uint32_t keys[ORDER_CAP];
  const int assay = blockIdx.x;
  const int first = d_assay_offsets[assay];
  const int n = min(d_assay_offsets[assay + 1], m) - first;
  if (n <= 0) return;
  if (n > ORDER_CAP) {
    for (int i = blockIdx.y * NT + threadIdx.x; i < n; i += ORDER_PARTS * NT) d_order[first + i] = first + i;
    return;
  }
  const int32_t* b = d_beads + 3 * (bead_stride ? (int64_t)assay * bead_stride : (int64_t)first);
  const int n4 = (n + 3) & ~3, nq = n4 >> 2;
  for (int i = threadIdx.x; i < n4; i += NT) {
    uint32_t k = 0xFFFFFFFFu;
    if (i < n) {
      const int row = min(max(b[3 * i], 0), (1 << 20) - 1), col = min(max(b[3 * i + 1], 0), (1 << 17) - 1);
      k = ((uint32_t)(row >> ORDER_BAND) << 17) | (uint32_t)col;
    }
    keys[i] = k;
  }
  __syncthreads();
  const uint4* k4 = reinterpret_cast<const uint4*>(keys);
  for (int i0 = blockIdx.y * NT; i0 < n; i0 += ORDER_PARTS * NT) {
    const int i = i0 + threadIdx.x;
    const int w0 = __builtin_amdgcn_readfirstlane(i0 + (int)(threadIdx.x & ~63u));
    const int q_lo = min(w0 >> 2, nq), q_hi = min((w0 + 63) >> 2, nq - 1);
    const uint32_t ki = keys[min(i, n - 1)];
    int rank = 0;
    for (int q = 0; q < q_lo; ++q) {
      const uint4 v = k4[q];
      rank += (v.x <= ki) + (v.y <= ki) + (v.z <= ki) + (v.w <= ki);
    }
    for (int q = q_lo; q <= q_hi; ++q) {
      const uint4 v = k4[q];
      const int j = 4 * q;
      rank += (v.x < ki || (v.x == ki && j < i)) + (v.y < ki || (v.y == ki && j + 1 < i)) +
              (v.z < ki || (v.z == ki && j + 2 < i)) + (v.w < ki || (v.w == ki && j + 3 < i));
    }
    for (int q = q_hi + 1; q < nq; ++q) {
      const uint4 v = k4[q];
      rank += (v.x < ki) + (v.y < ki) + (v.z < ki) + (v.w < ki);
    }
    if (i < n) d_order[first + rank] = first + i;
  }
}
}

extern "C" int mg_roi_window_order(const int32_t* d_beads, int64_t bead_stride, const int32_t* d_assay_offsets,
                                   int n_assays, int m, int32_t* d_order, void* stream) {
  if (!d_beads || !d_assay_offsets || !d_order || n_assays <= 0 || n_assays > 65535 || m < 0 || bead_stride < 0)
    return MG_EINVAL;
  if (m == 0) return MG_OK;
  hipLaunchKernelGGL(k_window_order, dim3(n_assays, ORDER_PARTS), dim3(NT), 0, mg_stream(stream), d_beads, bead_stride,
                     d_assay_offsets, m, d_order);
  MG_CHECK_LAUNCH();
  return MG_OK;
}

extern "C" int mg_roi_segment_reduce(const void* d_image, int dtype, int64_t assay_stride, int n_c, int n_t, int h,
                                     int w, int time_major, const int32_t* d_beads, int64_t bead_stride,
                                     const int32_t* d_assay_offsets, int n_assays, int m, const int32_t* d_order,
                                     int roi_len, const int32_t* d_halfwidths, int max_r, void* d_roi, uint8_t* d_fg,
                                     uint8_t* d_bg, double* d_sums, int32_t* d_counts, void* stream) {
  if (!d_assay_offsets || !d_halfwidths || n_assays <= 0 || n_assays > 65535 || max_r < 0 || bead_stride < 0)
    return MG_EINVAL;
  return roi_dispatch(d_image, dtype, assay_stride, n_c, n_t, h, w, d_beads, nullptr, nullptr, m, roi_len, nullptr,
                      d_assay_offsets, bead_stride, time_major, n_assays, d_order, d_halfwidths, max_r, d_roi, d_fg, d_bg,
                      d_sums, d_counts, stream);
}

extern "C" int mg_roi_gather_reduce(const void* d_image, int dtype, int n_c, int n_t, int h, int w,
                                    const int32_t* d_beads, int m, int roi_len, const int32_t* d_labels, void* d_roi,
                                    uint8_t* d_fg, uint8_t* d_bg, double* d_sums, int32_t* d_counts, void* stream) {
  return mg_roi_gather_reduce_batched(d_image, dtype, 0, n_c, n_t, h, w, d_beads, nullptr, nullptr, m, roi_len,
                                      d_labels, d_roi, d_fg, d_bg, d_sums, d_counts, stream);
}

extern "C" int mg_roi_masked_median(const void* d_roi, int dtype, const uint8_t* d_mask, int64_t mask_stride_m,
                                    int64_t mask_stride_t, int m, int n_c, int n_t, int roi_len, double* d_median,
                                    void* stream) {
  if (!d_roi || !d_mask || !d_median || m < 0 || n_c <= 0 || n_t <= 0 || roi_len <= 0) return MG_EINVAL;
  if (mask_stride_m < 0 || mask_stride_t < 0 || (int64_t)n_c * n_t > 65535) return MG_EINVAL;
  if (m == 0) return MG_OK;
  hipStream_t s = mg_stream(stream);
  return mg_dispatch_pixel(dtype, [&](auto t) {
    return launch_median<decltype(t)>(d_roi, d_mask, mask_stride_m, mask_stride_t, m, n_c, n_t, roi_len, d_median, s);
  });
}

extern "C" int mg_roi_masked_median_u16(const uint16_t* d_roi, const uint8_t* d_mask, int m, int n_c, int n_t,
                                        int roi_len, double* d_median, void* stream) {
  return mg_roi_masked_median(d_roi, MG_U16, d_mask, (int64_t)roi_len * roi_len, 0, m, n_c, n_t, roi_len, d_median, stream);
}
```

### magnify_amd/hotpath.py

```python
from __future__ import annotations

import math
import os
from collections import namedtuple

import numpy as np
import torch

from . import _native as nat

GRID_LENGTH = 20


def _ptr(t):
    return 0 if t is None else t.data_ptr()


def _stream():
    return torch._C._cuda_getCurrentRawStream(torch._C._cuda_getDevice())


class StageTimer:

    def __init__(self, allow_graphs=False):
# ... 90 lines not shown
        if tuple(arr.shape) != (ty, tx):
            raise ValueError(f"flat/dark field image must have the tile shape {(ty, tx)}")
        arr = arr.to(device=device, dtype=torch.float32 if arr.dtype == torch.float32 else torch.float64).contiguous()
    return 0.0, arr, nat.dtype_code(arr.dtype)


def flatfield_is_identity(dtype, flatfield=1.0, darkfield=0.0) -> bool:
    scalar = lambda v: np.isscalar(v) or (isinstance(v, np.ndarray) and v.ndim == 0)
    if not (scalar(flatfield) and scalar(darkfield)):
        return False
    return bool(nat.lib().mg_flatfield_is_identity(nat.dtype_code(dtype), float(darkfield), 0, float(flatfield), 0))


def flatfield_max(tiles: torch.Tensor, flatfield=1.0, darkfield=0.0, n_groups=1) -> torch.Tensor:
    require_gpu()
    ty, tx = tiles.shape[-2:]
    tiles = tiles.contiguous()
    dk, dkt, dkc = _df_operand(darkfield, ty, tx, tiles.device)
    fl, flt, flc = _df_operand(flatfield, ty, tx, tiles.device)
    max2 = torch.full((n_groups, 2), -math.inf, dtype=torch.float64, device=tiles.device)
    n_tiles = tiles.numel() // (ty * tx)
    code = nat.dtype_code(tiles.dtype)
    f32_image = flt is not None and flt.dtype == torch.float32 and dkt is None and (ty * tx) % (16 // tiles.element_size()) == 0
    words = int(nat.lib().mg_flatfield_max_scratch_floats(code, ty, tx)) if f32_image else 0
    scratch = None
    if words > 0:
        name = f"flatfield_max_scratch@{_stream()}"
        scratch = pooled(name, words, (), torch.float32, tiles.device)
        same = flt is flatfield
        key = (id(flatfield), flatfield._version, flt.data_ptr(), scratch.data_ptr(), code, ty, tx) if same else None
        if key is None or _BOUND_OF.get(name, (None, None))[0] != key:
            _call("mg_flatfield_bound", flt.data_ptr(), flc, code, ty, tx, scratch.data_ptr(), words, _stream())
            _BOUND_OF[name] = (key, flatfield if same else None)
    _call("mg_flatfield_max", tiles.data_ptr(), code, n_tiles, n_groups, ty, tx, dk, _ptr(dkt),
                                         dkc, fl, _ptr(flt), flc, max2.data_ptr(), _ptr(scratch), words, _stream())
    return max2


_BOUND_OF = {}


def stitch_geometry(ty: int, tx: int, overlap: int):
    clip, rem = overlap // 2, overlap % 2
    return clip, ty - 2 * clip - rem, tx - 2 * clip - rem


def flatfield_stitch(tiles: torch.Tensor, overlap: int, flatfield=1.0, darkfield=0.0, apply_flatfield=True,
                     max2: torch.Tensor | None = None, want_minmax=True, out: torch.Tensor | None = None,
                     minmax_out: torch.Tensor | None = None, n_groups=1):
    require_gpu()
    if overlap < 0:
        raise ValueError("Overlap must be non-negative.")
    c, t, nr, nc, ty, tx = tiles.shape
    if overlap >= ty or overlap >= tx:
        raise ValueError(f"Overlap ({overlap}) must be smaller than tile size ({ty}x{tx}).")
    tiles = tiles.contiguous()
    _, hy, hx = stitch_geometry(ty, tx, overlap)
    dk, dkt, dkc = _df_operand(darkfield, ty, tx, tiles.device)
    fl, flt, flc = _df_operand(flatfield, ty, tx, tiles.device)
    if (c * t) % n_groups:
        raise ValueError("n_groups must divide the number of planes")
    if apply_flatfield and flatfield_is_identity(tiles.dtype, flatfield, darkfield):
        apply_flatfield = False
    if apply_flatfield and max2 is None:
        max2 = flatfield_max(tiles, flatfield, darkfield, n_groups)
    if out is None:
        image = torch.empty((c, t, nr * hy, nc * hx), dtype=tiles.dtype, device=tiles.device)
    else:
        image = out
        assert image.is_contiguous() and image.numel() == c * t * nr * hy * nc * hx and image.dtype == tiles.dtype
    minmax = None
    if want_minmax:
        if minmax_out is None:
            minmax = torch.empty((c * t, 2), dtype=torch.float64, device=tiles.device)
        else:
            minmax = minmax_out
            assert minmax.is_contiguous() and minmax.numel() == c * t * 2 and minmax.dtype == torch.float64
        minmax.view(-1, 2).copy_(_minmax_init(c * t, tiles.device))
    _call("mg_flatfield_apply_stitch", tiles.data_ptr(), nat.dtype_code(tiles.dtype), c * t, nr, nc, ty, tx,
                                                  overlap, int(bool(apply_flatfield)), (c * t) // n_groups, dk, _ptr(dkt), dkc, fl,
                                                  _ptr(flt), flc, _ptr(max2), image.data_ptr(), _ptr(minmax),
                                                  _stream())
    return image, minmax


_MINMAX_INIT = {}


def _minmax_init(n, device):
    key = (int(n), str(device))
    t = _MINMAX_INIT.get(key)
    if t is None:
        if len(_MINMAX_INIT) > 16:
            _MINMAX_INIT.clear()
        t = torch.tensor([math.inf, -math.inf], dtype=torch.float64, device=device).repeat(int(n), 1)
        _MINMAX_INIT[key] = t
    return t


def plane_minmax(planes: torch.Tensor) -> torch.Tensor:
    require_gpu()
    p, h, w = planes.shape
    assert planes.stride(2) == 1 or w <= 1
    out = _minmax_init(p, planes.device).clone()
    _call("mg_plane_minmax", planes.data_ptr(), nat.dtype_code(planes.dtype), p, planes.stride(0), h, w,
                                        planes.stride(1), out.data_ptr(), _stream())
    return out




def _grad_of(m: int) -> np.float32:
    return np.sqrt(np.float32(m))


def quantile_indexes(n: int, q: float):
    qf = np.float32(q)
    vi = (n - 1) * qf
    prev = np.floor(vi)
    nxt = prev + 1
    if vi >= n - 1:
        prev_i = nxt_i = n - 1
    elif vi < 0:
        prev_i = nxt_i = 0
    else:
        prev_i, nxt_i = int(prev), int(nxt)
    gamma = np.float32(vi - prev)
    return prev_i, nxt_i, gamma


def lerp_f32(a: np.float32, b: np.float32, t: np.float32) -> np.float32:
    diff = np.float32(b - a)
    if t >= 0.5:
        return np.float32(b - diff * np.float32(1 - t))
    return np.float32(a + diff * t)


def canny_int_thresholds(lo: float, hi: float):
    lo, hi = float(lo), float(hi)
    if lo > hi:
        lo, hi = hi, lo
    lo, hi = min(32767.0, lo), min(32767.0, hi)
    if lo > 0:
        lo *= lo
    if hi > 0:
        hi *= hi
    return int(math.floor(lo)), int(math.floor(hi))


COARSE_SHIFT = 13
COARSE_BINS = 4096
FINE_BINS = 1 << COARSE_SHIFT
COMBINED_BINS = FINE_BINS + COARSE_BINS




class CircleFinder:

    MAX_GROUP = 64
    MAX_CAPTURES = 12
    (ROW_EDGES, ROW_EDGE_TOTALS, ROW_UNRESOLVED, ROW_ALIVE, ROW_OUT, ROW_SCORED, ROW_SURV, ROW_CIRCLES) = range(8)
    ROW_CHANGED, ROW_UNDECIDED, STATUS_ROWS = 8, 8 + MAX_GROUP, 8 + 2 * MAX_GROUP
    Plan = namedtuple("Plan", "win sweeps rounds")
    Request = namedtuple("Request", "planes minmax low_q high_q min_roundness min_dist seeds keep_raw keep_u8 passthrough_u8")
    REPLAY_STATE = ("_last_layer", "coord_cap", "u8", "raw", "_tie_keys", "_quantiles", "_gammas")
# ... 646 lines not shown
    return _HALF_CACHE[key]


_LABEL_POOL = {}


def circle_labels(beads_per_assay, h, w, device="cuda", reuse=False):
    require_gpu()
    a = len(beads_per_assay)
    cap = max(1, max((len(b) for b in beads_per_assay), default=1))
    host = np.zeros((a, cap, 3), dtype=np.int32)
    counts = np.zeros(a, dtype=np.int32)
    max_r = 2
    for k, b in enumerate(beads_per_assay):
        b = np.asarray(b).reshape(-1, 3)
        host[k, : len(b)] = b
        counts[k] = len(b)
        if len(b):
            max_r = max(max_r, int(b[:, 2].max()))
    key = (a, h, w, str(device))
    if reuse and key in _LABEL_POOL:
        labels = _LABEL_POOL.pop(key)
    else:
        labels = torch.full((a, h, w), -1, dtype=torch.int32, device=device)
    d_beads = torch.from_numpy(host).to(device)
    d_counts = torch.from_numpy(counts).to(device)
    tab = _halfwidth_table(max_r, device)
    _call("mg_circle_labels", d_beads.data_ptr(), cap, d_counts.data_ptr(), a, h, w, tab.data_ptr(), max_r,
          labels.data_ptr(), 0, _stream())
    labels._mg_state = (d_beads, cap, d_counts, a, h, w, tab, max_r, key)
    return labels


def release_labels(labels):
    d_beads, cap, d_counts, a, h, w, tab, max_r, key = labels._mg_state
    _call("mg_circle_labels", d_beads.data_ptr(), cap, d_counts.data_ptr(), a, h, w, tab.data_ptr(), max_r,
          labels.data_ptr(), 1, _stream(), stage="mg_circle_labels_reset")
    _LABEL_POOL[key] = labels


_STAGING = {}


def _upload_i32(values, device):
    n = len(values)
    ring = _STAGING.get((n, str(device)))
    if ring is None:
        ring = _STAGING[(n, str(device))] = [[torch.empty((n,), dtype=torch.int32).pin_memory() for _ in range(3)], 0]
    ring[1] = (ring[1] + 1) % 3
    host = ring[0][ring[1]]
    host.numpy()[:] = values
    return host.to(device, non_blocking=True)


_NMS_SPARSE = os.environ.get("MG_NMS_SPARSE", "1") != "0"


def _ring_difference_bits(ring, d):
    ring = np.asarray(ring, dtype=np.int64)
    side = 4 * d + 1
    diff = (ring[:, None, :] - ring[None, :, :]).reshape(-1, 2) + 2 * d
    flat = np.unique(diff[:, 0] * side + diff[:, 1])
    bits = np.zeros(((side * side + 31) // 32,), dtype=np.uint32)
    np.bitwise_or.at(bits, flat >> 5, np.uint32(1) << (flat & 31).astype(np.uint32))
    return bits.view(np.int32)


_ROI_ORDER = os.environ.get("MG_ROI_ORDER", "1") != "0"
_ROI_ORDER_MIN = int(os.environ.get("MG_ROI_ORDER_MIN", "200000"))


def _window_order(d_beads, bead_stride, d_off, n_assays, m, pool_tag, planes=1):
    if not _ROI_ORDER or m <= 0 or m * planes < _ROI_ORDER_MIN:
        return None
    dev = d_beads.device
    d_order = (pooled("roi_order" + pool_tag, m, (), torch.int32, dev) if pool_tag is not None
               else torch.empty((m,), dtype=torch.int32, device=dev))
    _call("mg_roi_window_order", d_beads.data_ptr(), int(bead_stride), d_off.data_ptr(), n_assays, m, d_order.data_ptr(), _stream())
    return d_order


def roi_gather_reduce(images: torch.Tensor, centers_per_assay, roi_len: int, labels: torch.Tensor | None,
                      want_roi=True, want_masks=True, want_sums=True, reuse_buffers=False, disks=False,
                      device_tables=None, time_major=False, device_counts=None, pool_tag=""):
    require_gpu()
    if time_major:
        if not disks:
            raise ValueError("time_major needs the bead-table masks (disks=True)")
        a, t, c, h, w = images.shape
    else:
        a, c, t, h, w = images.shape
    images = images.contiguous()
    dev = images.device
    if device_counts is not None:
        d_counts, cap, bound = device_counts
        assert device_tables is not None and disks and d_counts.dtype == torch.int32 and d_counts.numel() == a
        sizes, m, offsets = None, (a * int(cap) if bound is None else max(1, min(int(bound), a * int(cap)))), None
    else:
        sizes = [int(n) for n in device_tables[1]] if device_tables is not None else [len(b) for b in centers_per_assay]
        m = int(sum(sizes))
        offsets = np.concatenate([[0], np.cumsum(sizes)]).astype(np.int64)
    res = {"offsets": offsets, "bound": m}
    L = int(roi_len)
    alloc = ((lambda name, n, tail, dt, d: pooled(name + pool_tag, n, tail, dt, d)) if reuse_buffers
             else (lambda name, n, tail, dt, d: torch.empty((n,) + tuple(tail), dtype=dt, device=d)))
    res["roi"] = alloc("roi", m, (c, t, L, L), images.dtype, dev) if want_roi else None
    res["fg"] = alloc("fg", m, (L, L), torch.uint8, dev) if want_masks else None
    res["bg"] = alloc("bg", m, (L, L), torch.uint8, dev) if want_masks else None
    res["sums"] = alloc("sums", m, (c, t, 2), torch.float64, dev) if want_sums else None
    res["counts"] = alloc("counts", m, (2,), torch.int32, dev) if want_sums else None
    if m == 0:
        return res
    if device_tables is not None:
        d_tab, _, max_r = device_tables
        assert disks and d_tab.dtype == torch.int32 and d_tab.is_contiguous() and d_tab.shape[0] == a
        max_r = max(int(max_r), 2)
        tab = _halfwidth_table(max_r, dev)
        if device_counts is not None:
            d_off = pooled("roi_offsets" + pool_tag, a + 1, (), torch.int32, dev)
            _call("mg_counts_to_offsets", d_counts.data_ptr(), a, min(int(cap), d_tab.shape[1]), d_off.data_ptr(), _stream())
        else:
            d_off = _upload_i32(offsets, dev)
        res["device_tables"] = (d_tab, int(d_tab.shape[1]), d_off)
        d_order = _window_order(d_tab, d_tab.shape[1], d_off, a, m, pool_tag if reuse_buffers else None, c * t)
        _call("mg_roi_segment_reduce", images.data_ptr(), nat.dtype_code(images.dtype), c * t * h * w, c, t, h, w,
              int(time_major), d_tab.data_ptr(), d_tab.shape[1], d_off.data_ptr(), a, m, _ptr(d_order), L, tab.data_ptr(), max_r,
              _ptr(res["roi"]), _ptr(res["fg"]), _ptr(res["bg"]), _ptr(res["sums"]), _ptr(res["counts"]), _stream())
        return res
    beads = np.zeros((m, 3), dtype=np.int32)
    assay = np.zeros(m, dtype=np.int32)
    local = np.zeros(m, dtype=np.int32)
    for k, b in enumerate(centers_per_assay):
        b = np.asarray(b)
        lo, hi = offsets[k], offsets[k + 1]
        if hi > lo:
            beads[lo:hi, : 3 if disks else 2] = b[:, : 3 if disks else 2]
            assay[lo:hi] = k
            local[lo:hi] = np.arange(hi - lo)
    d_beads = torch.from_numpy(beads).to(dev)
    if disks:
        max_r = max(int(beads[:, 2].max()), 2)
        tab = _halfwidth_table(max_r, dev)
        d_off = torch.from_numpy(offsets.astype(np.int32)).to(dev)
        d_order = _window_order(d_beads, 0, d_off, a, m, pool_tag if reuse_buffers else None, c * t)
        _call("mg_roi_segment_reduce", images.data_ptr(), nat.dtype_code(images.dtype), c * t * h * w, c, t, h, w,
              int(time_major), d_beads.data_ptr(), 0, d_off.data_ptr(), a, m, _ptr(d_order), L, tab.data_ptr(), max_r,
              _ptr(res["roi"]), _ptr(res["fg"]), _ptr(res["bg"]), _ptr(res["sums"]), _ptr(res["counts"]), _stream())
        return res
    d_assay = torch.from_numpy(assay).to(dev)
    d_local = torch.from_numpy(local).to(dev)
    _call("mg_roi_gather_reduce_batched", 
        images.data_ptr(), nat.dtype_code(images.dtype), c * t * h * w, c, t, h, w, d_beads.data_ptr(),
        d_assay.data_ptr(), d_local.data_ptr(), m, L, _ptr(labels), _ptr(res["roi"]), _ptr(res["fg"]),
        _ptr(res["bg"]), _ptr(res["sums"]), _ptr(res["counts"]), _stream())
    return res


def finish_roi(res, counts):
    counts = np.asarray(counts, dtype=np.int64)
    m = int(counts.sum())
    if m > res["bound"]:
        return None
    out = {k: (v[:m] if isinstance(v, torch.Tensor) else v) for k, v in res.items()}
    out["offsets"] = np.concatenate([[0], np.cumsum(counts)]).astype(np.int64)
    return out


def marker_table(out: dict, assay_offset: int, n_channels: int) -> torch.Tensor:
    require_gpu()
    offsets = out.get("offsets")
    if offsets is None:
        offsets = np.concatenate([[0], np.cumsum([len(b) for b in out["beads"]])])
    offsets = np.asarray(offsets, dtype=np.int64)
    m, a = int(offsets[-1]), len(offsets) - 1
    sums, counts = out["sums"], out["counts"]
    dev = sums.device
    tab = torch.empty((m, 6 + 2 * n_channels), dtype=torch.float64, device=dev)
    if m == 0:
        return tab
    assert sums.shape[1] == n_channels and sums.is_contiguous() and counts.is_contiguous()
    tables = out.get("device_tables")
    if tables is not None:
        d_beads, stride, d_off = tables
    else:
        beads = [np.asarray(b, dtype=np.int32).reshape(-1, 3) for b in out["beads"]]
        d_beads, stride, d_off = _upload_i32(np.concatenate(beads).reshape(-1), dev), 0, _upload_i32(offsets, dev)
    _call("mg_marker_table", d_beads.data_ptr(), stride, d_off.data_ptr(), a, m, int(assay_offset), counts.data_ptr(),
          sums.data_ptr(), n_channels, int(sums.shape[2]), 0, tab.data_ptr(), _stream())
    return tab


def masked_median(roi: torch.Tensor, mask: torch.Tensor) -> torch.Tensor:
    require_gpu()
    m, c, t, L, _ = roi.shape
    roi = roi.contiguous()
    if mask.dtype == torch.bool:
        mask = mask.view(torch.uint8)
    if mask.dim() == 3:
        mask = mask.contiguous()
        sm, st = L * L, 0
    else:
        if mask.shape[1] not in (1, t):
            raise ValueError(f"masked_median: {mask.shape[1]} mask timepoints for {t} roi timepoints")
        if mask.stride(3) != 1 or mask.stride(2) != L or (m > 1 and mask.stride(0) < L * L):
            mask = mask.contiguous()
        sm, st = (mask.stride(0) if m > 1 else L * L), (mask.stride(1) if mask.shape[1] == t and t > 1 else 0)
    out = torch.empty((m, c, t), dtype=torch.float64, device=roi.device)
    if m == 0:
        return out
    _call("mg_roi_masked_median", roi.data_ptr(), nat.dtype_code(roi.dtype), mask.data_ptr(), sm, st, m, c, t, L,
          out.data_ptr(), _stream())
    return out


def masked_median_u16(roi: torch.Tensor, mask: torch.Tensor) -> torch.Tensor:
    require_gpu()
    m, c, t, L, _ = roi.shape
    out = torch.empty((m, c, t), dtype=torch.float64, device=roi.device)
    _call("mg_roi_masked_median_u16", roi.contiguous().data_ptr(), mask.contiguous().data_ptr(), m, c, t, L,
          out.data_ptr(), _stream())
    return out



_CV_CACHE = {}


def _cv_table(max_r: int, device):
    key = (max_r, str(device))
    if key not in _CV_CACHE:
        tab = np.full((max_r + 1, max_r + 1), -1, dtype=np.int32)
        for r in range(max_r + 1):
            tab[r, : r + 1] = nat.cv_disk_halfwidths(r)
        _CV_CACHE[key] = torch.from_numpy(tab).to(device)
    return _CV_CACHE[key]


def cluster_1d(points, total_length, num_clusters, cluster_length, ideal_num_points, penalty, device="cuda"):
# ... 46 lines not shown
```

### magnify_amd/stack.py

```python
from __future__ import annotations


import math
import os

import numpy as np
import torch

from . import hotpath as hp


class StackProcessor:

    def __init__(self, n_t, n_c, h, w, dtype=torch.uint16, min_bead_diameter=10, max_bead_diameter=50,
                 low_edge_quantile=0.1, high_edge_quantile=0.9, num_iter=5_000_000, min_roundness=0.3,
                 roi_length=None, search_channels=(0,), mode="P", plane_batch=None, device="cuda", n_streams=1,
                 sub_batches=None, tile_grid=None, overlap=0):
        hp.require_gpu()
        if min_bead_diameter > max_bead_diameter:
            raise ValueError("min_bead_diameter must be <= max_bead_diameter.")
        self.T, self.C, self.h, self.w = n_t, n_c, h, w
        self.overlap = int(overlap)
        self.tile_grid = tuple(int(v) for v in tile_grid) if tile_grid is not None else (1, 1, h, w)
        if tile_grid is None and overlap:
            raise ValueError("overlap needs tile_grid")
        if stitched_shape(*self.tile_grid, self.overlap) != (h, w):
            raise ValueError(f"tile_grid {self.tile_grid} with overlap {overlap} stitches to "
                             f"{stitched_shape(*self.tile_grid, self.overlap)}, not to {(h, w)}")
        self.min_r = math.floor(min_bead_diameter / 2)
        self.max_r = math.ceil(max_bead_diameter / 2)
        self.L = roi_length if roi_length is not None else 2 * max_bead_diameter
        self.low_q, self.high_q = low_edge_quantile, high_edge_quantile
        self.num_iter, self.min_roundness = num_iter, min_roundness
        self.search_channels = list(search_channels)
        self.mode = mode
        self.dev = torch.device(device)
        self.n_assays = n_t if mode == "P" else 1
        self.n_streams = n_streams if (self.n_assays >= 2 * n_streams and not plane_batch) else 1
        self.step_stats = []
        self._roi_bound = None
        self.pool_tag = ""
        self.placement = None
        self._trial_blocks = None
        self._placed = False
        self.stage = None
        if self.n_streams > 1:
            divisors = [d for d in range(1, self.n_assays + 1) if self.n_assays % d == 0]
            self.n_streams = max(d for d in divisors if d <= self.n_streams)
            n_sub = max([d for d in divisors if self.n_streams <= d <= (sub_batches or self.n_streams)] or [self.n_streams])
            per = self.n_assays // n_sub
            self.ranges = [(i, i + per) for i in range(0, self.n_assays, per)]
            self.streams = [torch.cuda.Stream(device=device) for _ in range(self.n_streams)]
            self.finders = [hp.CircleFinder(per, h, w, self.min_r, self.max_r, num_iter, device=device)
                            for _ in range(self.n_streams)]
            for f in self.finders:
                f._graphs = None
            self.finder = self.finders[0]
            self.batch = per
        else:
            self.batch = min(self.n_assays, plane_batch or self.n_assays)
            self.finder = hp.CircleFinder(self.batch, h, w, self.min_r, self.max_r, num_iter, device=device)
        self.image = torch.empty((n_t, n_c, h, w), dtype=dtype, device=self.dev)
        self.minmax = torch.empty((n_t, n_c, 2), dtype=torch.float64, device=self.dev)

    def flatfield(self, stack: torch.Tensor, flatfield=1.0, darkfield=0.0, max2=None):
        T, C = self.T, self.C
        tiles = stack.view(T * C, 1, *self.tile_grid)
        hp.flatfield_stitch(tiles, self.overlap, flatfield, darkfield, out=self.image, minmax_out=self.minmax, max2=max2,
                            n_groups=T if self.mode == "P" else 1)
        return self.image

    def detect(self, seed=0):
        T, h, w = self.T, self.h, self.w
        assays = list(range(self.n_assays))
        beads = [np.empty((0, 3), dtype=np.int32) for _ in assays]
        if self.n_streams > 1:
            return self._detect_streams(seed, beads)
        for k, ch in enumerate(self.search_channels):
            done = 0
            while done < len(assays):
                lo = min(done, len(assays) - self.batch)
                ids = assays[lo : lo + self.batch]
                planes = self.image[lo : lo + self.batch, ch]
                mm = self.minmax[lo : lo + self.batch, ch].contiguous()
                seeds = [(seed + 1000003 * a + 7919 * k) & 0xFFFFFFFFFFFFFFFF for a in ids]
                res, _ = self.finder.find(planes, mm, self.low_q, self.high_q, self.min_roundness, self.min_r, seeds,
                                          stable_input=True)
                for j, a in enumerate(ids):
                    if a >= done:
                        beads[a] = np.concatenate([beads[a], dedup_against(beads[a], res[j][0], 2 * self.min_r)])
                done = lo + self.batch
        return beads

    def _detect_streams(self, seed, beads, stack=None, flatfield=1.0, darkfield=0.0):
        import threading

        main = torch.cuda.current_stream()
        errors = []
        self.step_stats = []
        T, C, h, w = self.T, self.C, self.h, self.w
        host = stack is not None and not stack.is_cuda
        if host:
            if self.stage is None:
                self.stage = torch.empty((T, C) + self.tile_grid, dtype=stack.dtype, device=self.dev)
            tiles = self.stage.view(T * C, 1, *self.tile_grid)
        else:
            tiles = stack.view(T * C, 1, *self.tile_grid) if stack is not None else None

        def work(k):
            try:
                stream = self.streams[k]
                stream.wait_stream(main)
                with torch.cuda.stream(stream):
                    for lo, hi in self.ranges[k :: self.n_streams]:
                        if host:
                            self.stage.view(stack.shape)[lo:hi].copy_(stack[lo:hi], non_blocking=True)
                        if tiles is not None:
                            hp.flatfield_stitch(tiles[lo * C : hi * C], self.overlap, flatfield, darkfield, out=self.image[lo:hi],
                                                minmax_out=self.minmax[lo:hi], n_groups=hi - lo)
                        for j, ch in enumerate(self.search_channels):
                            planes = self.image[lo:hi, ch]
                            mm = self.minmax[lo:hi, ch].contiguous()
                            seeds = [(seed + 1000003 * a + 7919 * j) & 0xFFFFFFFFFFFFFFFF for a in range(lo, hi)]
                            res, _ = self.finders[k].find(planes, mm, self.low_q, self.high_q, self.min_roundness,
                                                          self.min_r, seeds)
                            for i, a in enumerate(range(lo, hi)):
                                beads[a] = np.concatenate([beads[a], dedup_against(beads[a], res[i][0], 2 * self.min_r)])
                            f = self.finders[k]
                            self.step_stats.append((torch.stack([f.num_circles.sum(), f.num_alive.sum(), f.num_scored.sum()]),
                                                    int(f.n_edges_host.sum()), dict(f.stats)))
                main.wait_stream(stream)
            except Exception as exc:
                errors.append(exc)

        threads = [threading.Thread(target=work, args=(k,)) for k in range(self.n_streams)]
        for t in threads:
            t.start()
        for t in threads:
            t.join()
        if errors:
            raise errors[0]
        return beads

    def segment_reduce(self, beads, want_roi=True, image=None, pool_tag=None):
        T, C, h, w = self.T, self.C, self.h, self.w
        image = self.image if image is None else image
        tag = self.pool_tag if pool_tag is None else pool_tag
        if self.mode == "P":
            return hp.roi_gather_reduce(image.view(T, C, 1, h, w), beads, self.L, None, want_roi=want_roi,
                                        reuse_buffers=True, disks=True, pool_tag=tag)
        return hp.roi_gather_reduce(image.view(1, T, C, h, w), beads, self.L, None, want_roi=want_roi,
                                    reuse_buffers=True, disks=True, time_major=True, pool_tag=tag)

    def __call__(self, stack, flatfield=1.0, darkfield=0.0, seed=0, want_roi=True):
        if self.n_streams > 1 and self.mode == "P":
            beads = [np.empty((0, 3), dtype=np.int32) for _ in range(self.n_assays)]
            beads = self._detect_streams(seed, beads, stack, flatfield, darkfield)
        else:
            if not stack.is_cuda:
                stack = stack.to(self.dev, non_blocking=True)
            tries = self._placement_tries()
            if tries:
                self._trial_image_blocks(stack, flatfield, darkfield, tries[0])
            else:
                self.flatfield(stack, flatfield, darkfield)
            if self.mode == "P" and len(self.search_channels) == 1 and self.batch >= self.n_assays:
                out = self._detect_reduce_on_device(seed, want_roi)
                return self._trial_roi_sets(out, want_roi, tries[1]) if tries else out
            beads = self.detect(seed)
            if tries:
                out = self._trial_pairs(lambda img, tag: self.segment_reduce(beads, want_roi, img, tag), tries[1],
                                        markers=sum(len(b) for b in beads))
                out["beads"] = beads
                return out
        out = self.segment_reduce(beads, want_roi=want_roi)
        out["beads"] = beads
        return out

    def _placement_tries(self):
        if self._placed:
            return None
        self._placed = True
        try:
            n_img, n_set = (int(v) for v in os.environ.get("MG_PLACEMENT_TRIES", "6,3").split(","))
        except ValueError:
            return None
        block = self.image.numel() * self.image.element_size()
        if (n_img < 2 and n_set < 2) or self.pool_tag or self.n_streams > 1 or block < (1 << 31):
            return None
        free, _ = torch.cuda.mem_get_info(self.dev)
        planes = self.C if self.mode == "P" else self.C * self.T
        roi_set = self.n_assays * 2500 * self.L * self.L * (2 * planes + 2)
        if free < (max(n_img, 1) + 1) * block + (max(n_set, 1) + 1) * roi_set:
            return None
        self.placement = {}
        return max(n_img, 1), max(n_set, 1)

    def _timed(self, fn, reps=2):
        best = float("inf")
        for _ in range(reps):
            a, b = torch.cuda.Event(enable_timing=True), torch.cuda.Event(enable_timing=True)
            a.record()
            fn()
            b.record()
            b.synchronize()
            best = min(best, a.elapsed_time(b))
        return best

    def _trial_image_blocks(self, stack, flatfield, darkfield, tries):
        blocks, times = [], []
        for k in range(tries):
            if k:
                try:
                    self.image = torch.empty_like(self.image)
                except torch.OutOfMemoryError:
                    break
            blocks.append(self.image)
            times.append(self._timed(lambda: self.flatfield(stack, flatfield, darkfield)))
        self.image = blocks[int(np.argmin(times))]
        self._trial_blocks = blocks
        self.placement.update(flatfield_ms=[round(t, 3) for t in times])

    def _trial_roi_sets(self, out, want_roi, tries):
        tabs = out.get("device_tables")
        if tabs is None:
            self._trial_blocks = None
            torch.cuda.empty_cache()
            self.placement.update(image_block=int(np.argmin(self.placement["flatfield_ms"])))
            return out
        T, C, h, w = self.T, self.C, self.h, self.w
        counts = [len(b) for b in out["beads"]]
        res = self._trial_pairs(lambda img, tag: hp.roi_gather_reduce(
            img.view(T, C, 1, h, w), None, self.L, None, want_roi=want_roi, reuse_buffers=True, disks=True,
            device_tables=(tabs[0], counts, self.max_r), pool_tag=tag), tries, markers=int(sum(counts)))
        res["beads"] = out["beads"]
        return res

    def _trial_pairs(self, run, tries, markers=None):
        blocks, self._trial_blocks = self._trial_blocks, None
        flat_ms = self.placement["flatfield_ms"]
        hp.drop_pool_tags([""])
        torch.cuda.empty_cache()
        if markers is not None:
            planes = self.C if self.mode == "P" else self.C * self.T
            set_bytes = int(1.3 * markers * self.L * self.L * (2 * planes + 2)) + (64 << 20)
            free, _ = torch.cuda.mem_get_info(self.dev)
            tries = int(min(tries, max(0, free - (8 << 30)) // set_bytes))
        tags = ["#place%d" % k for k in range(tries)]
        roi_ms = None
        if tries >= 2:
            try:
                roi_ms = [[self._timed(lambda: run(img, tag)) for tag in tags] for img in blocks]
            except torch.OutOfMemoryError:
                roi_ms = None
        if roi_ms is None:
            hp.drop_pool_tags(tags)
            self.image = blocks[int(np.argmin(flat_ms))]
            del blocks
            torch.cuda.empty_cache()
            self.placement.update(image_block=int(np.argmin(flat_ms)), roi_ms=None, roi_set=None)
            return run(self.image, self.pool_tag)
        total = np.asarray(roi_ms) + np.asarray(flat_ms)[:, None]
        bi, bj = (int(v) for v in np.unravel_index(int(np.argmin(total)), total.shape))
        hp.drop_pool_tags([t for k, t in enumerate(tags) if k != bj])
        self.image, self.pool_tag = blocks[bi], tags[bj]
        del blocks
        torch.cuda.empty_cache()
        self.placement.update(roi_ms=[[round(t, 3) for t in row] for row in roi_ms], image_block=bi, roi_set=bj)
        return run(self.image, self.pool_tag)

    def _detect_reduce_on_device(self, seed, want_roi):
        T, C, h, w = self.T, self.C, self.h, self.w
        ch = self.search_channels[0]
        seeds = [(seed + 1000003 * a) & 0xFFFFFFFFFFFFFFFF for a in range(self.n_assays)]
        roi_pass = lambda d_out, d_num, cap: hp.roi_gather_reduce(
            self.image.view(T, C, 1, h, w), None, self.L, None, want_roi=want_roi, reuse_buffers=True, disks=True,
            device_tables=(d_out, None, self.max_r), device_counts=(d_num, cap, self._roi_bound), pool_tag=self.pool_tag)
        counts, (d_beads, d_scores, _) = self.finder.find(self.image[:, ch], self.minmax[:, ch], self.low_q,
                                                           self.high_q, self.min_roundness, self.min_r, seeds,
                                                           host_results=False, follow=roi_pass, stable_input=True)
        out = hp.finish_roi(self.finder.follow_result, counts)
        if out is None:
            out = hp.roi_gather_reduce(self.image.view(T, C, 1, h, w), None, self.L, None, want_roi=want_roi,
                                       reuse_buffers=True, disks=True, device_tables=(d_beads, counts, self.max_r),
                                       pool_tag=self.pool_tag)
        self._roi_bound = int(1.1 * int(np.sum(counts))) + 16 * self.n_assays
        out["beads"] = [r[0] for r in self.finder.fetch_results(counts, d_beads, d_scores, overlap=True)]
        return out


def stitched_shape(rows, cols, tile_y, tile_x, overlap):
    _, hy, hx = hp.stitch_geometry(tile_y, tile_x, overlap)
    return rows * hy, cols * hx


def process_stream(chunks, flatfield=1.0, darkfield=0.0, seed=0, want_roi=False, prefetch=2, overlap=0, sink=None,
                   first_timepoint=None, **processor_kwargs):
    import queue
    import threading

    prefetch = max(1, int(prefetch))
    ring = getattr(chunks, "ring", None)
    if ring is not None and ring < prefetch + 2:
        raise ValueError(f"process_stream(prefetch={prefetch}) holds up to {prefetch + 2} blocks, the reader cycles "
                         f"through {ring}: pass ring >= {prefetch + 2} to iter_time_chunks")
    if first_timepoint is None:
        first_timepoint = int(getattr(chunks, "first_timepoint", 0))
    q = queue.Queue(maxsize=prefetch)
    stop, cancelled = object(), threading.Event()

    def produce():
        try:
            for item in chunks:
                while not cancelled.is_set():
                    try:
                        q.put(item, timeout=0.2)
                        break
                    except queue.Full:
                        continue
                if cancelled.is_set():
                    break
            else:
                q.put(stop)
        except BaseException as exc:
            q.put(exc)
        finally:
            if cancelled.is_set() and hasattr(chunks, "close"):
                chunks.close()

    producer = threading.Thread(target=produce, daemon=True)
    producer.start()
    import sys

    old_interval = sys.getswitchinterval()
    sys.setswitchinterval(min(old_interval, 2e-4))
    procs, done, n_chunk, copied = {}, int(first_timepoint), 0, [None, None]
    try:
        while True:
            item = q.get()
            if item is stop:
                return
            if isinstance(item, BaseException):
                raise item
            block = item[-1] if isinstance(item, tuple) else item
            if not isinstance(block, torch.Tensor):
                block = torch.from_numpy(np.ascontiguousarray(block))
            key = (tuple(block.shape), block.dtype)
            if key not in procs:
                if block.dim() == 6:
                    t, c = block.shape[:2]
                    h, w = stitched_shape(*block.shape[2:], overlap)
                    procs[key] = StackProcessor(t, c, h, w, dtype=block.dtype, mode="P", tile_grid=tuple(block.shape[2:]),
                                                overlap=overlap, **processor_kwargs)
                else:
                    t, c, h, w = block.shape
                    procs[key] = StackProcessor(t, c, h, w, dtype=block.dtype, mode="P", **processor_kwargs)
            t = block.shape[0]
            parity = n_chunk & 1
            if copied[parity] is not None:
                torch.cuda.current_stream().wait_event(copied[parity])
            procs[key].pool_tag = f"#{parity}"
            out = procs[key](block, flatfield, darkfield, seed=(seed + 1000003 * done) & 0xFFFFFFFFFFFFFFFF, want_roi=want_roi)
            out["first_timepoint"] = done
            for k in ("sums", "counts"):
                if out.get(k) is not None:
                    out[k] = out[k].clone()
            if isinstance(item, tuple) and len(item) == 3:
                out["time"], out["channel"] = item[0], item[1]
# ... 68 lines not shown
```

Measured before the change: 204,500.

## Defer flatfield of non-search channels and fuse correction into ROI segment-reduce

Flatfield-stitches only a subset of planes (the search channels) up front through a plane-mask kernel variant. The remaining channels are corrected on the fly from raw tiles inside a new ROI segment-reduce kernel. The aim is to avoid writing and rereading full corrected images for channels that are only sampled at marker windows. In exchange, per-pixel correction moves into the gather kernel, adding more templates and more complex raw-tile indexing.

```diff
diff --git a/include/magnify_hip.h b/include/magnify_hip.h
--- a/include/magnify_hip.h
+++ b/include/magnify_hip.h
@@ -46,6 +46,12 @@
                               double dark, const void* d_dark, int dark_dtype,
                               double flat, const void* d_flat, int flat_dtype,
                               const double* d_max2, void* d_image, double* d_minmax, void* stream);
+
+int mg_flatfield_apply_stitch_planes(const void* d_tiles, int dtype, int64_t n_planes, int n_tile_rows, int n_tile_cols,
+                                     int ty, int tx, int overlap, int planes_per_group, int plane_mask,
+                                     double dark, const void* d_dark, int dark_dtype,
+                                     double flat, const void* d_flat, int flat_dtype,
+                                     const double* d_max2, void* d_image, double* d_minmax, void* stream);
 
 int mg_plane_minmax(const void* d_src, int dtype, int n_planes, int64_t plane_stride, int h, int w,
                     int64_t row_stride, double* d_minmax, void* stream);
@@ -199,6 +205,14 @@
                           int n_assays, int m, const int32_t* d_order, int roi_len, const int32_t* d_halfwidths, int max_r,
                           void* d_roi, uint8_t* d_fg, uint8_t* d_bg, double* d_sums, int32_t* d_counts, void* stream);
 
+int mg_roi_segment_reduce_raw(const void* d_image, const void* d_raw, int dtype, int64_t assay_stride, int n_c, int n_t,
+                              int h, int w, int time_major, int raw_channel_mask, double dark, double flat,
+                              const float* d_flat, const double* d_max2, int planes_per_group,
+                              const int32_t* d_beads, int64_t bead_stride, const int32_t* d_assay_offsets,
+                              int n_assays, int m, const int32_t* d_order, int roi_len, const int32_t* d_halfwidths,
+                              int max_r, void* d_roi, uint8_t* d_fg, uint8_t* d_bg, double* d_sums, int32_t* d_counts,
+                              void* stream);
+
 int mg_roi_window_order(const int32_t* d_beads, int64_t bead_stride, const int32_t* d_assay_offsets, int n_assays, int m,
                         int32_t* d_order, void* stream);
 
diff --git a/magnify_amd/csrc/mg_flatcorr.h b/magnify_amd/csrc/mg_flatcorr.h
--- /dev/null
+++ b/magnify_amd/csrc/mg_flatcorr.h
@@ -0,0 +1,154 @@
+#pragma once
+#include "mg_common.h"
+
+namespace {
+
+template <typename T>
+__device__ __forceinline__ T cast_trunc(double v);
+template <>
+__device__ __forceinline__ uint8_t cast_trunc<uint8_t>(double v) {
+  return (uint8_t)(unsigned int)v;
+}
+template <>
+__device__ __forceinline__ uint16_t cast_trunc<uint16_t>(double v) {
+  return (uint16_t)(unsigned int)v;
+}
+template <>
+__device__ __forceinline__ float cast_trunc<float>(double v) {
+  return (float)v;
+}
+template <>
+__device__ __forceinline__ double cast_trunc<double>(double v) {
+  return v;
+}
+
+__device__ __forceinline__ bool flat_in_range(double fl) { return fl > 1e-30 && fl < 1e30; }
+
+__device__ __forceinline__ double refined_rcp(double fl) {
+  if (!flat_in_range(fl)) return 0.0;
+  double r = (double)__builtin_amdgcn_rcpf((float)fl);
+  r = r * (2.0 - fl * r);
+  r = r * (2.0 - fl * r);
+  return r;
+}
+
+__device__ __forceinline__ double exact_quotient(double t, double fl, double m1, double m2) {
+  double e = t / fl;
+  e = e * m1;
+  e = e / m2;
+  return e;
+}
+
+__device__ __forceinline__ bool group_quotient(double m1, double m2, double& kk) {
+  kk = m1 / m2;
+  return kk > 0.0 && kk < 1e30 && m1 > 0.0 && m1 < 1e300 && m2 > 0.0 && m2 < 1e300;
+}
+
+__device__ __forceinline__ double uniform_f64(double v) {
+  const unsigned long long u = (unsigned long long)__double_as_longlong(v);
+  const uint32_t lo = __builtin_amdgcn_readfirstlane((uint32_t)u), hi = __builtin_amdgcn_readfirstlane((uint32_t)(u >> 32));
+  return __longlong_as_double((long long)(((unsigned long long)hi << 32) | lo));
+}
+
+typedef unsigned short mg_u16x2 __attribute__((ext_vector_type(2)));
+template <typename T, int N>
+__device__ __forceinline__ void sub_dark_int(const T (&x)[N], uint32_t d, uint32_t (&ti)[N]) {
+#pragma unroll
+  for (int j = 0; j < N; ++j) {
+    const uint32_t xi = (uint32_t)x[j];
+    ti[j] = xi > d ? xi - d : 0u;
+  }
+}
+template <>
+__device__ __forceinline__ void sub_dark_int<uint16_t, 8>(const uint16_t (&x)[8], uint32_t d, uint32_t (&ti)[8]) {
+  uint32_t w[4];
+  __builtin_memcpy(w, x, 16);
+  const mg_u16x2 dd = {(unsigned short)d, (unsigned short)d};
+#pragma unroll
+  for (int q = 0; q < 4; ++q) {
+    const mg_u16x2 r = __builtin_elementwise_sub_sat(__builtin_bit_cast(mg_u16x2, w[q]), dd);
+    ti[2 * q] = r.x;
+    ti[2 * q + 1] = r.y;
+  }
+}
+template <>
+__device__ __forceinline__ void sub_dark_int<uint16_t, 2>(const uint16_t (&x)[2], uint32_t d, uint32_t (&ti)[2]) {
+  uint32_t w;
+  __builtin_memcpy(&w, x, 4);
+  const mg_u16x2 dd = {(unsigned short)d, (unsigned short)d};
+  const mg_u16x2 r = __builtin_elementwise_sub_sat(__builtin_bit_cast(mg_u16x2, w), dd);
+  ti[0] = r.x;
+  ti[1] = r.y;
+}
+
+template <typename T, int N>
+__device__ __forceinline__ bool fast_chunk_int(const uint32_t (&ti)[N], const double (&rk)[N], T (&o)[N]) {
+  bool unsure = false;
+#pragma unroll
+  for (int j = 0; j < N; ++j) {
+    const double v = (double)ti[j] * rk[j];
+    const double fr = __builtin_amdgcn_fract(v);
+    o[j] = (T)(unsigned int)v;
+    unsure |= !(fr > 1e-6 && fr < 1.0 - 1e-6) && ti[j] != 0u;
+  }
+  return unsure;
+}
+template <typename T, int N>
+__device__ __forceinline__ bool fast_chunk_f64(const double (&t)[N], const double (&rk)[N], T (&o)[N]) {
+  bool unsure = false;
+#pragma unroll
+  for (int j = 0; j < N; ++j) {
+    const double v = t[j] * rk[j];
+    const double fr = __builtin_amdgcn_fract(v);
+    o[j] = (T)(unsigned int)v;
+    unsure |= !(fr > 1e-6 && fr < 1.0 - 1e-6) && t[j] != 0.0;
+  }
+  return unsure;
+}
+
+template <int N>
+__device__ __forceinline__ bool chunk_factors(const double (&rr)[N], double kk, double (&rk)[N]) {
+  bool large = false;
+#pragma unroll
+  for (int j = 0; j < N; ++j) {
+    rk[j] = rr[j] * kk;
+    large |= !(rk[j] < 61035.0);
+  }
+  return large;
+}
+
+template <typename T, int N, bool INT_DARK>
+__device__ __forceinline__ void correct_chunk_rk(const T (&x)[N], uint32_t dark_i, const double (&dk)[N],
+                                                 const double (&fl)[N], const double (&rk)[N], bool rk_bad,
+                                                 const double* __restrict__ d_max2, int plane, int planes_per_group,
+                                                 T (&o)[N]) {
+  bool unsure;
+  uint32_t ti[N];
+  double t[N];
+  if (INT_DARK) {
+    sub_dark_int<T, N>(x, dark_i, ti);
+    unsure = fast_chunk_int<T, N>(ti, rk, o);
+  } else {
+#pragma unroll
+    for (int j = 0; j < N; ++j) {
+      t[j] = (double)x[j] - dk[j];
+      t[j] = t[j] < 0.0 ? 0.0 : t[j];
+    }
+    unsure = fast_chunk_f64<T, N>(t, rk, o);
+  }
+  if (unsure || rk_bad) {
+    const int group = plane / planes_per_group;
+    const double m1 = d_max2[2 * group], m2 = d_max2[2 * group + 1];
+#pragma unroll
+    for (int j = 0; j < N; ++j) {
+      const double tj = INT_DARK ? (double)ti[j] : t[j];
+      o[j] = cast_trunc<T>(exact_quotient(tj, fl[j], m1, m2));
+    }
+  }
+}
+
+inline bool dark_is_int(const void* d_dark, double dark) {
+  return !d_dark && dark >= 0.0 && dark <= 65535.0 && dark == (double)(uint32_t)dark;
+}
+
+}
diff --git a/magnify_amd/csrc/mg_flatfield.hip b/magnify_amd/csrc/mg_flatfield.hip
--- a/magnify_amd/csrc/mg_flatfield.hip
+++ b/magnify_amd/csrc/mg_flatfield.hip
@@ -1,6 +1,7 @@
 #include <math.h>
 
 #include "mg_common.h"
+#include "mg_flatcorr.h"
 
 namespace {
 
@@ -62,25 +63,6 @@
 }
 
 template <typename T>
-__device__ __forceinline__ T cast_trunc(double v);
-template <>
-__device__ __forceinline__ uint8_t cast_trunc<uint8_t>(double v) {
-  return (uint8_t)(unsigned int)v;
-}
-template <>
-__device__ __forceinline__ uint16_t cast_trunc<uint16_t>(double v) {
-  return (uint16_t)(unsigned int)v;
-}
-template <>
-__device__ __forceinline__ float cast_trunc<float>(double v) {
-  return (float)v;
-}
-template <>
-__device__ __forceinline__ double cast_trunc<double>(double v) {
-  return v;
-}
-
-template <typename T>
 struct IsIntegral {
   static constexpr bool value = false;
 };
@@ -113,8 +95,6 @@
     mg_atomic_nanmax(out + 1, m2);
   }
 }
-
-__device__ __forceinline__ bool flat_in_range(double fl) { return fl > 1e-30 && fl < 1e30; }
 
 __device__ __forceinline__ void max_step(double t, double fl, bool fast_m2, double& m1, double& m2) {
   m1 = mg_nanmax(m1, t);
@@ -406,14 +386,6 @@
 
 constexpr int ROWS_PER_BLOCK = 32;
 
-__device__ __forceinline__ double refined_rcp(double fl) {
-  if (!flat_in_range(fl)) return 0.0;
-  double r = (double)__builtin_amdgcn_rcpf((float)fl);
-  r = r * (2.0 - fl * r);
-  r = r * (2.0 - fl * r);
-  return r;
-}
-
 template <typename T>
 __device__ __forceinline__ T correct_pixel(double t, double fl, double r, double m1, double m2, double k, bool fast_ok) {
   if (IsIntegral<T>::value && fast_ok && r != 0.0) {
@@ -423,65 +395,55 @@
     const double fr = v - fv;
     if (fr > 1e-6 && fr < 1.0 - 1e-6 && v < 4.0e9) return (T)(unsigned int)fv;
   }
-  double e = t / fl;
-  e = e * m1;
-  e = e / m2;
-  return cast_trunc<T>(e);
-}
-
-template <typename T, int N>
-__device__ __forceinline__ void correct_chunk(const T (&x)[N], const double (&dk)[N], const double (&fl)[N],
-                                              const double (&r)[N], double m1, double m2, double k, bool fast_ok, T (&o)[N]) {
-  double t[N];
-  bool unsure = !fast_ok || !IsIntegral<T>::value;
-#pragma unroll
-  for (int j = 0; j < N; ++j) {
-    t[j] = (double)x[j] - dk[j];
-    t[j] = t[j] < 0.0 ? 0.0 : t[j];
-    if (!IsIntegral<T>::value) continue;
-    const double v = t[j] * r[j] * k;
-    const double fv = floor(v);
-    const double fr = v - fv;
-    o[j] = (T)(unsigned int)fv;
-    unsure |= !((fr > 1e-6 && fr < 1.0 - 1e-6 && v < 4.0e9) || t[j] == 0.0) || r[j] == 0.0;
-  }
-  if (unsure) {
-#pragma unroll
-    for (int j = 0; j < N; ++j) {
-      double e = t[j] / fl[j];
-      e = e * m1;
-      e = e / m2;
-      o[j] = cast_trunc<T>(e);
-    }
-  }
+  return cast_trunc<T>(exact_quotient(t, fl, m1, m2));
 }
 
 constexpr int PLANES_PER_BLOCK = 8;
 
-template <typename T, bool APPLY>
+struct PlaneSel {
+  uint32_t mask;
+  int n_sel;
+};
+template <bool SUBSET>
+__device__ __forceinline__ int sel_plane(int s, int planes_per_group, PlaneSel sel) {
+  if (!SUBSET) return s;
+  const int g = s / sel.n_sel;
+  uint32_t m = sel.mask;
+  for (int k = s - g * sel.n_sel; k > 0; --k) m &= m - 1u;
+  return g * planes_per_group + __builtin_ctz(m);
+}
+struct SelBase {
+  int s0, planes_per_group;
+  PlaneSel sel;
+  __device__ __forceinline__ int operator+(int b) const { return sel_plane<true>(s0 + b, planes_per_group, sel); }
+};
+
+template <typename T, bool APPLY, bool SUBSET = false>
 __global__ __launch_bounds__(256) void k_apply_stitch(const T* __restrict__ tiles, int n_planes, int n_tr, int n_tc,
                                                        int ty, int tx, int clip, int hy, int hx, int planes_per_group,
                                                        double dark, const void* __restrict__ d_dark, int dark_dt,
                                                        double flat, const void* __restrict__ d_flat, int flat_dt,
                                                        const double* __restrict__ d_max2, T* __restrict__ image,
-                                                       double* __restrict__ d_minmax, int rows_per_block) {
+                                                       double* __restrict__ d_minmax, int rows_per_block, PlaneSel sel) {
   constexpr int N = VecOf<T>::N;
   constexpr int PB = PLANES_PER_BLOCK;
   const int plane0 = blockIdx.z * PB;
   const int np = min(PB, n_planes - plane0);
   const int h_out = n_tr * hy, w_out = n_tc * hx;
   const int ox0 = (blockIdx.x * blockDim.x + threadIdx.x) * N;
+  int pl[PB];
+#pragma unroll
+  for (int b = 0; b < PB; ++b) pl[b] = (!SUBSET || b < np) ? sel_plane<SUBSET>(plane0 + b, planes_per_group, sel) : 0;
   double m1[PB], m2[PB], kk[PB];
   bool fast_ok[PB];
 #pragma unroll
   for (int b = 0; b < PB; ++b) {
     m1[b] = 0.0, m2[b] = 1.0, kk[b] = 1.0, fast_ok[b] = false;
     if (APPLY && b < np) {
-      const int group = (plane0 + b) / planes_per_group;
+      const int group = pl[b] / planes_per_group;
       m1[b] = d_max2[2 * group];
       m2[b] = d_max2[2 * group + 1];
-      kk[b] = m1[b] / m2[b];
-      fast_ok[b] = kk[b] > 0.0 && kk[b] < 1e30 && m1[b] > 0.0 && m1[b] < 1e300 && m2[b] > 0.0 && m2[b] < 1e300;
+      fast_ok[b] = group_quotient(m1[b], m2[b], kk[b]);
     }
   }
   double vmin[PB], vmax[PB];
@@ -526,7 +488,7 @@
 #pragma unroll
       for (int b = 0; b < PB; ++b) {
         if (b >= np) break;
-        const int64_t plane_base = (int64_t)(plane0 + b) * n_tr * n_tc * tile_elems;
+        const int64_t plane_base = (int64_t)pl[b] * n_tr * n_tc * tile_elems;
         T x[N], o[N];
         if (one_tile) {
           load_vec<T, N>(tiles + plane_base + toff[0] + pix[0], x);
@@ -554,7 +516,7 @@
             }
           }
         }
-        T* dst = image + ((int64_t)(plane0 + b) * h_out + oy) * w_out + ox0;
+        T* dst = image + ((int64_t)pl[b] * h_out + oy) * w_out + ox0;
         if (cnt == N) {
           store_vec<T, N>(dst, o);
         } else {
@@ -563,63 +525,13 @@
       }
     }
   }
-  if (d_minmax) mg_block_minmax<PB>(vmin, vmax, imin, imax, np, d_minmax, plane0);
-}
-
-__device__ __forceinline__ double uniform_f64(double v) {
-  const unsigned long long u = (unsigned long long)__double_as_longlong(v);
-  const uint32_t lo = __builtin_amdgcn_readfirstlane((uint32_t)u), hi = __builtin_amdgcn_readfirstlane((uint32_t)(u >> 32));
-  return __longlong_as_double((long long)(((unsigned long long)hi << 32) | lo));
-}
-
-typedef unsigned short mg_u16x2 __attribute__((ext_vector_type(2)));
-template <typename T, int N>
-__device__ __forceinline__ void sub_dark_int(const T (&x)[N], uint32_t d, uint32_t (&ti)[N]) {
-#pragma unroll
-  for (int j = 0; j < N; ++j) {
-    const uint32_t xi = (uint32_t)x[j];
-    ti[j] = xi > d ? xi - d : 0u;
-  }
-}
-template <>
-__device__ __forceinline__ void sub_dark_int<uint16_t, 8>(const uint16_t (&x)[8], uint32_t d, uint32_t (&ti)[8]) {
-  uint32_t w[4];
-  __builtin_memcpy(w, x, 16);
-  const mg_u16x2 dd = {(unsigned short)d, (unsigned short)d};
-#pragma unroll
-  for (int q = 0; q < 4; ++q) {
-    const mg_u16x2 r = __builtin_elementwise_sub_sat(__builtin_bit_cast(mg_u16x2, w[q]), dd);
-    ti[2 * q] = r.x;
-    ti[2 * q + 1] = r.y;
-  }
-}
-
-template <typename T, int N>
-__device__ __forceinline__ bool fast_chunk_int(const uint32_t (&ti)[N], const double (&rk)[N], T (&o)[N]) {
-  bool unsure = false;
-#pragma unroll
-  for (int j = 0; j < N; ++j) {
-    const double v = (double)ti[j] * rk[j];
-    const double fr = __builtin_amdgcn_fract(v);
-    o[j] = (T)(unsigned int)v;
-    unsure |= !(fr > 1e-6 && fr < 1.0 - 1e-6) && ti[j] != 0u;
-  }
-  return unsure;
-}
-template <typename T, int N>
-__device__ __forceinline__ bool fast_chunk_f64(const double (&t)[N], const double (&rk)[N], T (&o)[N]) {
-  bool unsure = false;
-#pragma unroll
-  for (int j = 0; j < N; ++j) {
-    const double v = t[j] * rk[j];
-    const double fr = __builtin_amdgcn_fract(v);
-    o[j] = (T)(unsigned int)v;
-    unsure |= !(fr > 1e-6 && fr < 1.0 - 1e-6) && t[j] != 0.0;
-  }
-  return unsure;
-}
-
-template <typename T, bool APPLY, bool INT_DARK>
+  if (d_minmax) {
+    if (SUBSET) mg_block_minmax<PB>(vmin, vmax, imin, imax, np, d_minmax, SelBase{plane0, planes_per_group, sel});
+    else mg_block_minmax<PB>(vmin, vmax, imin, imax, np, d_minmax, plane0);
+  }
+}
+
+template <typename T, bool APPLY, bool INT_DARK, bool SUBSET = false>
 __global__ __launch_bounds__(256) void k_apply_stitch_aligned(const T* __restrict__ tiles, int n_planes, int n_tr,
                                                                int n_tc, int ty, int tx, int clip, int hy, int hx,
                                                                int planes_per_group, double dark,
@@ -627,7 +539,7 @@
                                                                double flat, const void* __restrict__ d_flat,
                                                                int flat_dt, const double* __restrict__ d_max2,
                                                                T* __restrict__ image, double* __restrict__ d_minmax,
-                                                               int rows_per_block) {
+                                                               int rows_per_block, PlaneSel sel) {
   constexpr int N = VecOf<T>::N;
   constexpr int PB = PLANES_PER_BLOCK;
   int bx = blockIdx.x, by = blockIdx.y, bz = blockIdx.z;
@@ -643,6 +555,9 @@
   const int np = min(PB, n_planes - plane0);
   const int h_out = n_tr * hy, w_out = n_tc * hx;
   const int ox0 = (bx * blockDim.x + threadIdx.x) * N;
+  int pl[PB];
+#pragma unroll
+  for (int b = 0; b < PB; ++b) pl[b] = (!SUBSET || b < np) ? sel_plane<SUBSET>(plane0 + b, planes_per_group, sel) : 0;
   uint32_t imin[PB], imax[PB];
 #pragma unroll
   for (int b = 0; b < PB; ++b) imin[b] = 0xFFFFFFFFu, imax[b] = 0u;
@@ -653,11 +568,11 @@
   for (int b = 0; b < PB; ++b) {
     kka[b] = 1.0;
     if (APPLY && b < np) {
-      const int group = (plane0 + b) / planes_per_group;
+      const int group = pl[b] / planes_per_group;
       const double m1 = d_max2[2 * group], m2 = d_max2[2 * group + 1];
-      const double kk = m1 / m2;
+      double kk;
+      const bool ok = group_quotient(m1, m2, kk);
       kka[b] = uniform_f64(kk);
-      const bool ok = kk > 0.0 && kk < 1e30 && m1 > 0.0 && m1 < 1e300 && m2 > 0.0 && m2 < 1e300;
       ok_mask |= ok ? (1u << b) : 0u;
     }
   }
@@ -686,7 +601,7 @@
       T xin[PB][N];
 #pragma unroll
       for (int b = 0; b < PB; ++b)
-        if (b < np) load_vec16<T, N>(tiles + (int64_t)(plane0 + b) * plane_elems + src0, xin[b], false);
+        if (b < np) load_vec16<T, N>(tiles + (int64_t)pl[b] * plane_elems + src0, xin[b], false);
       double rk[N];
       double kk_of_rk = -1.0;
       bool rk_large = true;
@@ -698,40 +613,10 @@
         if (APPLY) {
           if (kka[b] != kk_of_rk) {
             kk_of_rk = kka[b];
-            rk_large = false;
-#pragma unroll
-            for (int j = 0; j < N; ++j) {
-              rk[j] = rr[j] * kk_of_rk;
-              rk_large |= !(rk[j] < 61035.0);
-            }
+            rk_large = chunk_factors<N>(rr, kk_of_rk, rk);
           }
           const bool rk_bad = rk_large || flat_bad || !((ok_mask >> b) & 1u);
-          bool unsure;
-          uint32_t ti[N];
-          double t[N];
-          if (INT_DARK) {
-            sub_dark_int<T, N>(x, dark_i, ti);
-            unsure = fast_chunk_int<T, N>(ti, rk, o);
-          } else {
-#pragma unroll
-            for (int j = 0; j < N; ++j) {
-              t[j] = (double)x[j] - dk[j];
-              t[j] = t[j] < 0.0 ? 0.0 : t[j];
-            }
-            unsure = fast_chunk_f64<T, N>(t, rk, o);
-          }
-          if (unsure || rk_bad) {
-            const int group = (plane0 + b) / planes_per_group;
-            const double m1 = d_max2[2 * group], m2 = d_max2[2 * group + 1];
-#pragma unroll
-            for (int j = 0; j < N; ++j) {
-              const double tj = INT_DARK ? (double)ti[j] : t[j];
-              double e = tj / fl[j];
-              e = e * m1;
-              e = e / m2;
-              o[j] = cast_trunc<T>(e);
-            }
-          }
+          correct_chunk_rk<T, N, INT_DARK>(x, dark_i, dk, fl, rk, rk_bad, d_max2, pl[b], planes_per_group, o);
         } else {
 #pragma unroll
           for (int j = 0; j < N; ++j) o[j] = x[j];
@@ -743,11 +628,14 @@
             imax[b] = max(imax[b], (uint32_t)o[j]);
           }
         }
-        store_vec16<T, N>(image + ((int64_t)(plane0 + b) * h_out + oy) * w_out + ox0, o, false);
-      }
-    }
-  }
-  if (d_minmax) mg_block_minmax_u32<PB>(imin, imax, np, d_minmax, plane0);
+        store_vec16<T, N>(image + ((int64_t)pl[b] * h_out + oy) * w_out + ox0, o, false);
+      }
+    }
+  }
+  if (d_minmax) {
+    if (SUBSET) mg_block_minmax_u32<PB>(imin, imax, np, d_minmax, SelBase{plane0, planes_per_group, sel});
+    else mg_block_minmax_u32<PB>(imin, imax, np, d_minmax, plane0);
+  }
 }
 
 template <typename T>
@@ -853,11 +741,13 @@
 template <typename T>
 int launch_apply(const void* d_tiles, int64_t n_planes, int n_tr, int n_tc, int ty, int tx, int overlap, int apply,
                  int planes_per_group, double dark, const void* d_dark, int dark_dt, double flat, const void* d_flat, int flat_dt,
-                 const double* d_max2, void* d_image, double* d_minmax, hipStream_t s) {
+                 const double* d_max2, void* d_image, double* d_minmax, hipStream_t s, uint32_t plane_mask = 0) {
   const auto [clip, hy, hx, h_out, w_out] = mg_stitch_geom(ty, tx, overlap, n_tr, n_tc);
   if (n_planes == 0 || h_out == 0 || w_out == 0) return MG_OK;
   constexpr int N = VecOf<T>::N;
   if (n_planes > 0x7FFFFFF0) return MG_EINVAL;
+  const PlaneSel sel{plane_mask, __builtin_popcount(plane_mask)};
+  if (plane_mask) n_planes = n_planes / planes_per_group * sel.n_sel;
   int rows = ROWS_PER_BLOCK;
   const int64_t cols_planes = (int64_t)((w_out + 256 * N - 1) / (256 * N)) * ((n_planes + PLANES_PER_BLOCK - 1) / PLANES_PER_BLOCK);
   while (rows > 2 && cols_planes * ((h_out + rows - 1) / rows) < 2048) rows /= 2;
@@ -871,29 +761,37 @@
                        (!d_flat || (reinterpret_cast<uintptr_t>(d_flat) & 15) == 0) &&
                        (!d_dark || (reinterpret_cast<uintptr_t>(d_dark) & 15) == 0);
   if (aligned) {
-    const bool int_dark = apply && !d_dark && dark >= 0.0 && dark <= 65535.0 && dark == (double)(uint32_t)dark;
-#define MG_ALIGNED(AP, ID) \
-    hipLaunchKernelGGL((k_apply_stitch_aligned<T, AP, ID>), grid, dim3(256), 0, s, (const T*)d_tiles, (int)n_planes, n_tr, \
+    const bool int_dark = apply && dark_is_int(d_dark, dark);
+#define MG_ALIGNED(AP, ID, SUB) \
+    hipLaunchKernelGGL((k_apply_stitch_aligned<T, AP, ID, SUB>), grid, dim3(256), 0, s, (const T*)d_tiles, (int)n_planes, n_tr, \
                        n_tc, ty, tx, clip, hy, hx, planes_per_group, dark, d_dark, dark_dt, flat, d_flat, flat_dt, \
-                       d_max2, (T*)d_image, d_minmax, rows)
-    if (!apply)
-      MG_ALIGNED(false, false);
+                       d_max2, (T*)d_image, d_minmax, rows, sel)
+    if (plane_mask && int_dark)
+      MG_ALIGNED(true, true, true);
+    else if (plane_mask)
+      MG_ALIGNED(true, false, true);
+    else if (!apply)
+      MG_ALIGNED(false, false, false);
     else if (int_dark)
-      MG_ALIGNED(true, true);
+      MG_ALIGNED(true, true, false);
     else
-      MG_ALIGNED(true, false);
+      MG_ALIGNED(true, false, false);
 #undef MG_ALIGNED
     MG_CHECK_LAUNCH();
     return MG_OK;
   }
-  if (apply)
+  if (plane_mask)
+    hipLaunchKernelGGL((k_apply_stitch<T, true, true>), grid, dim3(256), 0, s, (const T*)d_tiles, (int)n_planes, n_tr, n_tc,
+                       ty, tx, clip, hy, hx, planes_per_group, dark, d_dark, dark_dt, flat, d_flat, flat_dt, d_max2,
+                       (T*)d_image, d_minmax, rows, sel);
+  else if (apply)
     hipLaunchKernelGGL((k_apply_stitch<T, true>), grid, dim3(256), 0, s, (const T*)d_tiles, (int)n_planes, n_tr, n_tc,
                        ty, tx, clip, hy, hx, planes_per_group, dark, d_dark, dark_dt, flat, d_flat, flat_dt, d_max2,
-                       (T*)d_image, d_minmax, rows);
+                       (T*)d_image, d_minmax, rows, sel);
   else
     hipLaunchKernelGGL((k_apply_stitch<T, false>), grid, dim3(256), 0, s, (const T*)d_tiles, (int)n_planes, n_tr, n_tc,
                        ty, tx, clip, hy, hx, planes_per_group, dark, d_dark, dark_dt, flat, d_flat, flat_dt, d_max2,
-                       (T*)d_image, d_minmax, rows);
+                       (T*)d_image, d_minmax, rows, sel);
   MG_CHECK_LAUNCH();
   return MG_OK;
 }
@@ -979,6 +877,27 @@
   });
 }
 
+extern "C" int mg_flatfield_apply_stitch_planes(const void* d_tiles, int dtype, int64_t n_planes, int n_tile_rows,
+                                                int n_tile_cols, int ty, int tx, int overlap, int planes_per_group,
+                                                int plane_mask, double dark, const void* d_dark, int dark_dtype,
+                                                double flat, const void* d_flat, int flat_dtype, const double* d_max2,
+                                                void* d_image, double* d_minmax, void* stream) {
+  if (!d_tiles || !d_image || !d_max2 || n_planes < 0 || n_tile_rows <= 0 || n_tile_cols <= 0 || ty <= 0 || tx <= 0)
+    return MG_EINVAL;
+  if (overlap < 0 || overlap >= ty || overlap >= tx) return MG_EINVAL;
+  if (planes_per_group <= 0 || planes_per_group > 31 || n_planes % planes_per_group || plane_mask < 0 ||
+      (plane_mask >> planes_per_group))
+    return MG_EINVAL;
+  if (!df_dtype_ok(d_dark, dark_dtype) || !df_dtype_ok(d_flat, flat_dtype)) return MG_EINVAL;
+  if (plane_mask == 0) return MG_OK;
+  hipStream_t s = mg_stream(stream);
+  return mg_dispatch_pixel(dtype, [&](auto t) {
+    return launch_apply<decltype(t)>(d_tiles, n_planes, n_tile_rows, n_tile_cols, ty, tx, overlap, 1, planes_per_group,
+                                     dark, d_dark, dark_dtype, flat, d_flat, flat_dtype, d_max2, d_image, d_minmax, s,
+                                     (uint32_t)plane_mask);
+  });
+}
+
 extern "C" int mg_plane_minmax(const void* d_src, int dtype, int n_planes, int64_t plane_stride, int h, int w,
                                int64_t row_stride, double* d_minmax, void* stream) {
   if (!d_src || !d_minmax || n_planes < 0 || h < 0 || w < 0) return MG_EINVAL;
diff --git a/magnify_amd/csrc/mg_roi.hip b/magnify_amd/csrc/mg_roi.hip
--- a/magnify_amd/csrc/mg_roi.hip
+++ b/magnify_amd/csrc/mg_roi.hip
@@ -3,6 +3,7 @@
 #include <stdlib.h>
 
 #include "mg_common.h"
+#include "mg_flatcorr.h"
 
 namespace {
 
@@ -260,8 +261,28 @@
 }
 __device__ __forceinline__ uint32_t roi_pair(uint32_t b) { return (b & 1u) | ((b & 2u) << 15); }
 
-template <int U, int CTB, bool PIPE>
-__global__ __launch_bounds__(NT) void k_roi_u16_even(const uint16_t* __restrict__ d_image, int64_t assay_stride,
+struct RoiRaw {
+  const uint16_t* raw;
+  const float* flat;
+  const double* max2;
+  double flat_s, dark;
+  int planes_per_group;
+  uint32_t chan_mask;
+};
+
+template <bool INT_DARK>
+__device__ __forceinline__ uint32_t roi_correct_dword(uint32_t d, uint32_t dark_i, double dark, const double (&fl)[2],
+                                                      const double (&rk)[2], bool rk_bad,
+                                                      const double* __restrict__ d_max2, int group) {
+  const uint16_t x[2] = {(uint16_t)(d & 0xFFFFu), (uint16_t)(d >> 16)};
+  const double dk[2] = {dark, dark};
+  uint16_t o[2];
+  correct_chunk_rk<uint16_t, 2, INT_DARK>(x, dark_i, dk, fl, rk, rk_bad, d_max2, group, 1, o);
+  return (uint32_t)o[0] | ((uint32_t)o[1] << 16);
+}
+
+template <int U, int CTB, bool PIPE, int FUSE = 0>
+__global__ __launch_bounds__(NT) __attribute__((amdgpu_waves_per_eu(5, 8))) void k_roi_u16_even(const uint16_t* __restrict__ d_image, int64_t assay_stride,
                                                      int n_c, int n_t, int h, int w,
                                                      const int32_t* __restrict__ d_beads,
                                                      const int32_t* __restrict__ d_marker_assay,
@@ -272,7 +293,7 @@
                                                      const int32_t* __restrict__ d_halfwidths, int max_r,
                                                      uint16_t* __restrict__ d_roi, uint8_t* __restrict__ d_fg,
                                                      uint8_t* __restrict__ d_bg, double* __restrict__ d_sums,
-                                                     int32_t* __restrict__ d_counts) {
+                                                     int32_t* __restrict__ d_counts, RoiRaw rw) {
   extern __shared__ __attribute__((aligned(4))) uint8_t smem[];
   constexpr int WV = NT / 64;
   __shared__ uint32_t s_red[2][CTB][WV];
@@ -365,32 +386,46 @@
   const uint32_t shift = odd ? 16u : 0u;
   const uint32_t lidx = (uint32_t)min(lane, half - 1 + odd);
   const int64_t plane_elems = (int64_t)h * w;
+  const int group = FUSE ? (int)(((int64_t)assay * nct) / rw.planes_per_group) : 0;
+  double kk = 1.0;
+  bool group_ok = false;
+  if (FUSE) {
+    group_ok = group_quotient(rw.max2[2 * group], rw.max2[2 * group + 1], kk);
+    kk = uniform_f64(kk);
+  }
+  const uint32_t dark_i = FUSE == 1 ? (uint32_t)rw.dark : 0u;
+  const uint16_t* rawimg = FUSE ? rw.raw + (int64_t)assay * assay_stride : nullptr;
   for (int ct0 = 0; ct0 < nct; ct0 += CTB) {
     const uint32_t* plane[CTB];
     uint32_t* out[CTB];
+    uint32_t raw_c = 0u;
 #pragma unroll
     for (int c = 0; c < CTB; ++c) {
       const int ct = min(ct0 + c, nct - 1);
-      plane[c] = reinterpret_cast<const uint32_t*>(img + (int64_t)(time_major ? (ct % n_t) * n_c + ct / n_t : ct) * plane_elems);
+      const bool is_raw = FUSE && ((rw.chan_mask >> (ct / n_t)) & 1u);
+      raw_c |= is_raw ? (1u << c) : 0u;
+      plane[c] = reinterpret_cast<const uint32_t*>((is_raw ? rawimg : img) + (int64_t)(time_major ? (ct % n_t) * n_c + ct / n_t : ct) * plane_elems);
       out[c] = d_roi ? reinterpret_cast<uint32_t*>(d_roi + ((int64_t)g * nct + ct) * n) : nullptr;
     }
     uint32_t sf[CTB], sb[CTB];
 #pragma unroll
     for (int c = 0; c < CTB; ++c) sf[c] = 0u, sb[c] = 0u;
-    auto load_rows = [&](int r0, uint32_t (&dd)[U][CTB]) {
+    auto load_rows = [&](int r0, uint32_t (&dd)[U][CTB], float2 (&ff)[U]) {
 #pragma unroll
       for (int u = 0; u < U; ++u) {
         const int ry = min(r0 + u * WV, len - 1);
         const uint32_t di = (uint32_t)(((top + ry) * w + left - odd) >> 1) + lidx;
 #pragma unroll
         for (int c = 0; c < CTB; ++c) dd[u][c] = plane[c][di];
+        if (FUSE && rw.flat) ff[u] = reinterpret_cast<const float2*>(rw.flat)[di];
       }
     };
     uint32_t dd[U][CTB], dn[U][CTB];
-    load_rows(wave, dd);
+    float2 ff[U], fn[U];
+    load_rows(wave, dd, ff);
     for (int r0 = wave; r0 < len; r0 += WV * U) {
       if (PIPE) {
-        load_rows(r0 + WV * U, dn);
+        load_rows(r0 + WV * U, dn, fn);
       }
 #pragma unroll
       for (int u = 0; u < U; ++u) {
@@ -398,10 +433,21 @@
         if (ry >= len) break;
         const uint32_t mf = roi_pair((fgw[ry * wpr + mword] >> msh) & 3u), mb = roi_pair((bgw[ry * wpr + mword] >> msh) & 3u);
         const uint32_t oi = (uint32_t)(ry * half + lane);
+        double fl[2], rk[2];
+        bool rk_bad = false;
+        if (FUSE && raw_c) {
+          fl[0] = rw.flat ? (double)ff[u].x : rw.flat_s;
+          fl[1] = rw.flat ? (double)ff[u].y : rw.flat_s;
+          const double rr[2] = {refined_rcp(fl[0]), refined_rcp(fl[1])};
+          const bool rk_large = chunk_factors<2>(rr, kk, rk);
+          rk_bad = rk_large || rr[0] == 0.0 || rr[1] == 0.0 || !group_ok;
+        }
 #pragma unroll
         for (int c = 0; c < CTB; ++c) {
           if (ct0 + c >= nct) break;
-          const uint32_t d = dd[u][c];
+          uint32_t d = dd[u][c];
+          if (FUSE && ((raw_c >> c) & 1u))
+            d = roi_correct_dword<FUSE == 1>(d, dark_i, rw.dark, fl, rk, rk_bad, rw.max2, group);
           const uint32_t nx = (uint32_t)__builtin_amdgcn_update_dpp(0, (int)d, 0x130, 0xF, 0xF, false);
           const uint32_t v = __builtin_amdgcn_alignbit(nx, d, shift);
           if (act) {
@@ -416,8 +462,12 @@
         for (int u = 0; u < U; ++u)
 #pragma unroll
           for (int c = 0; c < CTB; ++c) dd[u][c] = dn[u][c];
+        if (FUSE) {
+#pragma unroll
+          for (int u = 0; u < U; ++u) ff[u] = fn[u];
+        }
       } else if (r0 + WV * U < len) {
-        load_rows(r0 + WV * U, dd);
+        load_rows(r0 + WV * U, dd, ff);
       }
     }
     if (d_sums) {
@@ -872,12 +922,32 @@
                  const int32_t* d_beads, const int32_t* d_marker_assay, const int32_t* d_marker_local, int m, int roi_len,
                  const int32_t* d_labels, const int32_t* d_assay_offsets, int64_t bead_stride, int time_major, int n_assays,
                  const int32_t* d_order, const int32_t* d_halfwidths, int max_r, void* d_roi, uint8_t* d_fg, uint8_t* d_bg,
-                 double* d_sums, int32_t* d_counts, void* stream) {
+                 double* d_sums, int32_t* d_counts, void* stream, const RoiRaw* fuse = nullptr) {
   if (!d_image || !d_beads || m < 0 || roi_len <= 0 || n_c <= 0 || n_t <= 0) return MG_EINVAL;
   if (roi_len > h || roi_len > w || roi_lds_bytes(roi_len, d_halfwidths != nullptr) > 60000) return MG_EINVAL;
   if (m == 0) return MG_OK;
   hipStream_t s = mg_stream(stream);
   const dim3 grid(m);
+  if (fuse) {
+    const auto al = [](const void* p, uintptr_t a) { return (reinterpret_cast<uintptr_t>(p) & (a - 1)) == 0; };
+    if (dtype != MG_U16 || (roi_len & 1) || roi_len > 126 || (w & 1) || (assay_stride & 7) || (int64_t)h * w >= (1LL << 31) ||
+        time_major || !fuse->raw || !fuse->max2 || n_c > 31 || (fuse->chan_mask >> n_c) || fuse->planes_per_group <= 0 ||
+        fuse->planes_per_group % (n_c * n_t) || !al(d_image, 16) || !al(fuse->raw, 16) || !al(fuse->flat, 16) ||
+        !al(fuse->max2, 8) || (d_roi && !al(d_roi, 4)) || (d_fg && !al(d_fg, 2)) || (d_bg && !al(d_bg, 2)))
+      return MG_EINVAL;
+#define MG_ROI_FUSED(F) \
+    hipLaunchKernelGGL((k_roi_u16_even<2, 4, true, F>), grid, dim3(NT), (size_t)mask_words(roi_len) * 4, s, \
+                       (const uint16_t*)d_image, assay_stride, n_c, n_t, h, w, d_beads, d_marker_assay, d_marker_local, \
+                       roi_len, d_labels, d_assay_offsets, n_assays, bead_stride, time_major, d_order, d_halfwidths, max_r, \
+                       (uint16_t*)d_roi, d_fg, d_bg, d_sums, d_counts, *fuse)
+    if (dark_is_int(nullptr, fuse->dark))
+      MG_ROI_FUSED(1);
+    else
+      MG_ROI_FUSED(2);
+#undef MG_ROI_FUSED
+    MG_CHECK_LAUNCH();
+    return MG_OK;
+  }
   const char* tiles_env = getenv("MG_ROI_TILES");
   const bool tiles = tiles_env && tiles_env[0] == '1';
   if (tiles && dtype == MG_U16 && d_halfwidths && d_assay_offsets && !d_labels && (roi_len & 1) == 0 && roi_len <= 126 &&
@@ -908,7 +978,7 @@
     hipLaunchKernelGGL((k_roi_u16_even<2, 4, true>), grid, dim3(NT), (size_t)mask_words(roi_len) * 4, s,
                        (const uint16_t*)d_image, assay_stride, n_c, n_t, h, w, d_beads, d_marker_assay, d_marker_local,
                        roi_len, d_labels, d_assay_offsets, n_assays, bead_stride, time_major, d_order, d_halfwidths, max_r, (uint16_t*)d_roi, d_fg, d_bg,
-                       d_sums, d_counts);
+                       d_sums, d_counts, RoiRaw{});
     MG_CHECK_LAUNCH();
     return MG_OK;
   }
@@ -1075,6 +1145,22 @@
                       d_sums, d_counts, stream);
 }
 
+extern "C" int mg_roi_segment_reduce_raw(const void* d_image, const void* d_raw, int dtype, int64_t assay_stride, int n_c,
+                                         int n_t, int h, int w, int time_major, int raw_channel_mask, double dark,
+                                         double flat, const float* d_flat, const double* d_max2, int planes_per_group,
+                                         const int32_t* d_beads, int64_t bead_stride, const int32_t* d_assay_offsets,
+                                         int n_assays, int m, const int32_t* d_order, int roi_len,
+                                         const int32_t* d_halfwidths, int max_r, void* d_roi, uint8_t* d_fg, uint8_t* d_bg,
+                                         double* d_sums, int32_t* d_counts, void* stream) {
+  if (!d_assay_offsets || !d_halfwidths || n_assays <= 0 || n_assays > 65535 || max_r < 0 || bead_stride < 0 ||
+      raw_channel_mask < 0)
+    return MG_EINVAL;
+  const RoiRaw rw{(const uint16_t*)d_raw, d_flat, d_max2, flat, dark, planes_per_group, (uint32_t)raw_channel_mask};
+  return roi_dispatch(d_image, dtype, assay_stride, n_c, n_t, h, w, d_beads, nullptr, nullptr, m, roi_len, nullptr,
+                      d_assay_offsets, bead_stride, time_major, n_assays, d_order, d_halfwidths, max_r, d_roi, d_fg, d_bg,
+                      d_sums, d_counts, stream, &rw);
+}
+
 extern "C" int mg_roi_gather_reduce(const void* d_image, int dtype, int n_c, int n_t, int h, int w,
                                     const int32_t* d_beads, int m, int roi_len, const int32_t* d_labels, void* d_roi,
                                     uint8_t* d_fg, uint8_t* d_bg, double* d_sums, int32_t* d_counts, void* stream) {
diff --git a/magnify_amd/hotpath.py b/magnify_amd/hotpath.py
--- a/magnify_amd/hotpath.py
+++ b/magnify_amd/hotpath.py
@@ -196,6 +196,35 @@
                                                   _ptr(flt), flc, _ptr(max2), image.data_ptr(), _ptr(minmax),
                                                   _stream())
     return image, minmax
+
+
+def flatfield_apply_planes(tiles: torch.Tensor, overlap: int, flatfield, darkfield, max2: torch.Tensor, plane_mask: int,
+                           planes_per_group: int, out: torch.Tensor, minmax_out: torch.Tensor, init_minmax=True):
+    require_gpu()
+    c, t, nr, nc, ty, tx = tiles.shape
+    assert tiles.is_contiguous() and out.is_contiguous() and out.dtype == tiles.dtype
+    assert minmax_out.is_contiguous() and minmax_out.numel() == c * t * 2 and minmax_out.dtype == torch.float64
+    assert (c * t) % planes_per_group == 0 and max2.numel() == 2 * (c * t) // planes_per_group
+    dk, dkt, dkc = _df_operand(darkfield, ty, tx, tiles.device)
+    fl, flt, flc = _df_operand(flatfield, ty, tx, tiles.device)
+    if init_minmax:
+        minmax_out.view(-1, 2).copy_(_minmax_init(c * t, tiles.device))
+    _call("mg_flatfield_apply_stitch_planes", tiles.data_ptr(), nat.dtype_code(tiles.dtype), c * t, nr, nc, ty, tx, overlap,
+          int(planes_per_group), int(plane_mask), dk, _ptr(dkt), dkc, fl, _ptr(flt), flc, max2.data_ptr(), out.data_ptr(),
+          minmax_out.data_ptr(), _stream(), stage="mg_flatfield_apply_stitch")
+    return out, minmax_out
+
+
+RawChannels = namedtuple("RawChannels", "stack mask flatfield darkfield max2 planes_per_group complete")
+RawChannels.__doc__ = """What ``roi_gather_reduce(raw=...)`` needs to gather channels that have no corrected copy in the
+image block: the raw ``stack`` (laid out as the image block), the bit ``mask`` of those channels, the correction's
+operands (scalar dark; flat scalar or a float32 device image), the maxima ``max2`` of pass 1 with their
+``planes_per_group``, and ``complete()``: corrects those channels into the image block with the correction pass -- the
+way out when the fused kernel refuses the call (MG_EINVAL)."""
+
+
+def fused_roi_enabled() -> bool:
+    return os.environ.get("MG_FUSED_ROI", "1") != "0"
 
 
 _MINMAX_INIT = {}
@@ -1008,7 +1037,7 @@
 
 def roi_gather_reduce(images: torch.Tensor, centers_per_assay, roi_len: int, labels: torch.Tensor | None,
                       want_roi=True, want_masks=True, want_sums=True, reuse_buffers=False, disks=False,
-                      device_tables=None, time_major=False, device_counts=None, pool_tag=""):
+                      device_tables=None, time_major=False, device_counts=None, pool_tag="", raw=None):
     require_gpu()
     if time_major:
         if not disks:
@@ -1049,9 +1078,7 @@
             d_off = _upload_i32(offsets, dev)
         res["device_tables"] = (d_tab, int(d_tab.shape[1]), d_off)
         d_order = _window_order(d_tab, d_tab.shape[1], d_off, a, m, pool_tag if reuse_buffers else None, c * t)
-        _call("mg_roi_segment_reduce", images.data_ptr(), nat.dtype_code(images.dtype), c * t * h * w, c, t, h, w,
-              int(time_major), d_tab.data_ptr(), d_tab.shape[1], d_off.data_ptr(), a, m, _ptr(d_order), L, tab.data_ptr(), max_r,
-              _ptr(res["roi"]), _ptr(res["fg"]), _ptr(res["bg"]), _ptr(res["sums"]), _ptr(res["counts"]), _stream())
+        _segment_reduce(images, raw, c, t, h, w, time_major, d_tab, d_tab.shape[1], d_off, a, m, d_order, L, tab, max_r, res)
         return res
     beads = np.zeros((m, 3), dtype=np.int32)
     assay = np.zeros(m, dtype=np.int32)
@@ -1069,10 +1096,10 @@
         tab = _halfwidth_table(max_r, dev)
         d_off = torch.from_numpy(offsets.astype(np.int32)).to(dev)
         d_order = _window_order(d_beads, 0, d_off, a, m, pool_tag if reuse_buffers else None, c * t)
-        _call("mg_roi_segment_reduce", images.data_ptr(), nat.dtype_code(images.dtype), c * t * h * w, c, t, h, w,
-              int(time_major), d_beads.data_ptr(), 0, d_off.data_ptr(), a, m, _ptr(d_order), L, tab.data_ptr(), max_r,
-              _ptr(res["roi"]), _ptr(res["fg"]), _ptr(res["bg"]), _ptr(res["sums"]), _ptr(res["counts"]), _stream())
+        _segment_reduce(images, raw, c, t, h, w, time_major, d_beads, 0, d_off, a, m, d_order, L, tab, max_r, res)
         return res
+    if raw is not None:
+        raise ValueError("raw channels need the bead-table masks (disks=True)")
     d_assay = torch.from_numpy(assay).to(dev)
     d_local = torch.from_numpy(local).to(dev)
     _call("mg_roi_gather_reduce_batched", 
@@ -1080,6 +1107,29 @@
         d_assay.data_ptr(), d_local.data_ptr(), m, L, _ptr(labels), _ptr(res["roi"]), _ptr(res["fg"]),
         _ptr(res["bg"]), _ptr(res["sums"]), _ptr(res["counts"]), _stream())
     return res
+
+
+def _segment_reduce(images, raw, c, t, h, w, time_major, d_beads, bead_stride, d_off, a, m, d_order, L, tab, max_r, res):
+    tail = (d_beads.data_ptr(), int(bead_stride), d_off.data_ptr(), a, m, _ptr(d_order), L, tab.data_ptr(), max_r,
+            _ptr(res["roi"]), _ptr(res["fg"]), _ptr(res["bg"]), _ptr(res["sums"]), _ptr(res["counts"]), _stream())
+    code = nat.dtype_code(images.dtype)
+    if raw is not None and raw.mask:
+        assert raw.stack.is_contiguous() and raw.stack.numel() == images.numel() and raw.stack.dtype == images.dtype
+        assert raw.max2.numel() * raw.planes_per_group == 2 * a * c * t
+        fl, flt, _ = _df_operand(raw.flatfield, h, w, images.device)
+        assert flt is None or flt.dtype == torch.float32
+        args = (images.data_ptr(), raw.stack.data_ptr(), code, c * t * h * w, c, t, h, w, int(time_major), int(raw.mask),
+                float(raw.darkfield), fl, _ptr(flt), raw.max2.data_ptr(), int(raw.planes_per_group)) + tail
+        if TIMER is _NO_TIMER or _CAPTURING:
+            rc = nat.lib().mg_roi_segment_reduce_raw(*args)
+        else:
+            with TIMER.stage("mg_roi_segment_reduce"):
+                rc = nat.lib().mg_roi_segment_reduce_raw(*args)
+        if rc != -1:
+            nat.check(rc, "mg_roi_segment_reduce_raw")
+            return
+        raw.complete()
+    _call("mg_roi_segment_reduce", images.data_ptr(), code, c * t * h * w, c, t, h, w, int(time_major), *tail)
 
 
 def finish_roi(res, counts):
diff --git a/magnify_amd/stack.py b/magnify_amd/stack.py
--- a/magnify_amd/stack.py
+++ b/magnify_amd/stack.py
@@ -60,15 +60,76 @@
         else:
             self.batch = min(self.n_assays, plane_batch or self.n_assays)
             self.finder = hp.CircleFinder(self.batch, h, w, self.min_r, self.max_r, num_iter, device=device)
-        self.image = torch.empty((n_t, n_c, h, w), dtype=dtype, device=self.dev)
-        self.minmax = torch.empty((n_t, n_c, 2), dtype=torch.float64, device=self.dev)
+        self._image = torch.empty((n_t, n_c, h, w), dtype=dtype, device=self.dev)
+        self._minmax = torch.empty((n_t, n_c, 2), dtype=torch.float64, device=self.dev)
+        self._raw = None
+        self._deferred = False
+
+    @property
+    def image(self):
+        self._complete()
+        return self._image
+
+    @image.setter
+    def image(self, block):
+        self._image = block
+
+    @property
+    def minmax(self):
+        self._complete()
+        return self._minmax
+
+    @minmax.setter
+    def minmax(self, block):
+        self._minmax = block
+
+    def _complete(self):
+        if not self._deferred:
+            return
+        self._deferred = False
+        r = self._raw
+        hp.flatfield_apply_planes(r.stack.view(self.T * self.C, 1, *self.tile_grid), 0, r.flatfield, r.darkfield, r.max2,
+                                  r.mask, self.C, out=self._image, minmax_out=self._minmax, init_minmax=False)
+
+    def _fused_flat(self, stack, flatfield, darkfield):
+        T, C, h, w = self.T, self.C, self.h, self.w
+        scalar = lambda v: np.isscalar(v) or (isinstance(v, np.ndarray) and v.ndim == 0)
+        deferred = [c for c in range(C) if c not in self.search_channels]
+        if (not hp.fused_roi_enabled() or self.mode != "P" or self.n_streams > 1 or not deferred or C > 31
+                or not all(0 <= c < C for c in self.search_channels)
+                or not (isinstance(stack, torch.Tensor) and stack.is_cuda and stack.dtype == torch.uint16
+                        and self._image.dtype == torch.uint16 and stack.is_contiguous() and tuple(stack.shape) == (T, C, h, w))
+                or self.tile_grid != (1, 1, h, w) or self.overlap or self.L % 2 or self.L > 126 or self.L > min(h, w) or w % 2
+                or not scalar(darkfield) or stack.data_ptr() % 16 or self._image.data_ptr() % 16):
+            return None
+        if scalar(flatfield):
+            return None if hp.flatfield_is_identity(stack.dtype, flatfield, darkfield) else float(flatfield)
+        if isinstance(flatfield, np.ndarray) and flatfield.dtype == np.float32 and flatfield.shape == (h, w):
+            flatfield = torch.from_numpy(np.ascontiguousarray(flatfield)).to(self.dev)
+        if (isinstance(flatfield, torch.Tensor) and flatfield.dtype == torch.float32 and flatfield.device == stack.device
+                and tuple(flatfield.shape) == (h, w) and flatfield.is_contiguous() and flatfield.data_ptr() % 16 == 0):
+            return flatfield
+        return None
+
+    def _correct(self, stack, flatfield, darkfield, fused_flat=None):
+        if fused_flat is None:
+            return self.flatfield(stack, flatfield, darkfield)
+        T, C = self.T, self.C
+        tiles = stack.view(T * C, 1, *self.tile_grid)
+        searched = sum(1 << c for c in set(self.search_channels))
+        max2 = hp.flatfield_max(tiles, fused_flat, darkfield, n_groups=T)
+        hp.flatfield_apply_planes(tiles, 0, fused_flat, darkfield, max2, searched, C, out=self._image, minmax_out=self._minmax)
+        self._raw = hp.RawChannels(stack, ((1 << C) - 1) & ~searched, fused_flat, float(darkfield), max2, C, self._complete)
+        self._deferred = True
+        return self._image
 
     def flatfield(self, stack: torch.Tensor, flatfield=1.0, darkfield=0.0, max2=None):
         T, C = self.T, self.C
+        self._raw, self._deferred = None, False
         tiles = stack.view(T * C, 1, *self.tile_grid)
-        hp.flatfield_stitch(tiles, self.overlap, flatfield, darkfield, out=self.image, minmax_out=self.minmax, max2=max2,
+        hp.flatfield_stitch(tiles, self.overlap, flatfield, darkfield, out=self._image, minmax_out=self._minmax, max2=max2,
                             n_groups=T if self.mode == "P" else 1)
-        return self.image
+        return self._image
 
     def detect(self, seed=0):
         T, h, w = self.T, self.h, self.w
@@ -81,8 +142,8 @@
             while done < len(assays):
                 lo = min(done, len(assays) - self.batch)
                 ids = assays[lo : lo + self.batch]
-                planes = self.image[lo : lo + self.batch, ch]
-                mm = self.minmax[lo : lo + self.batch, ch].contiguous()
+                planes = self._image[lo : lo + self.batch, ch]
+                mm = self._minmax[lo : lo + self.batch, ch].contiguous()
                 seeds = [(seed + 1000003 * a + 7919 * k) & 0xFFFFFFFFFFFFFFFF for a in ids]
                 res, _ = self.finder.find(planes, mm, self.low_q, self.high_q, self.min_roundness, self.min_r, seeds,
                                           stable_input=True)
@@ -116,11 +177,11 @@
                         if host:
                             self.stage.view(stack.shape)[lo:hi].copy_(stack[lo:hi], non_blocking=True)
                         if tiles is not None:
-                            hp.flatfield_stitch(tiles[lo * C : hi * C], self.overlap, flatfield, darkfield, out=self.image[lo:hi],
-                                                minmax_out=self.minmax[lo:hi], n_groups=hi - lo)
+                            hp.flatfield_stitch(tiles[lo * C : hi * C], self.overlap, flatfield, darkfield, out=self._image[lo:hi],
+                                                minmax_out=self._minmax[lo:hi], n_groups=hi - lo)
                         for j, ch in enumerate(self.search_channels):
-                            planes = self.image[lo:hi, ch]
-                            mm = self.minmax[lo:hi, ch].contiguous()
+                            planes = self._image[lo:hi, ch]
+                            mm = self._minmax[lo:hi, ch].contiguous()
                             seeds = [(seed + 1000003 * a + 7919 * j) & 0xFFFFFFFFFFFFFFFF for a in range(lo, hi)]
                             res, _ = self.finders[k].find(planes, mm, self.low_q, self.high_q, self.min_roundness,
                                                           self.min_r, seeds)
@@ -144,26 +205,28 @@
 
     def segment_reduce(self, beads, want_roi=True, image=None, pool_tag=None):
         T, C, h, w = self.T, self.C, self.h, self.w
-        image = self.image if image is None else image
+        image = self._image if image is None else image
         tag = self.pool_tag if pool_tag is None else pool_tag
         if self.mode == "P":
             return hp.roi_gather_reduce(image.view(T, C, 1, h, w), beads, self.L, None, want_roi=want_roi,
-                                        reuse_buffers=True, disks=True, pool_tag=tag)
+                                        reuse_buffers=True, disks=True, pool_tag=tag, raw=self._raw)
         return hp.roi_gather_reduce(image.view(1, T, C, h, w), beads, self.L, None, want_roi=want_roi,
                                     reuse_buffers=True, disks=True, time_major=True, pool_tag=tag)
 
     def __call__(self, stack, flatfield=1.0, darkfield=0.0, seed=0, want_roi=True):
         if self.n_streams > 1 and self.mode == "P":
+            self._raw, self._deferred = None, False
             beads = [np.empty((0, 3), dtype=np.int32) for _ in range(self.n_assays)]
             beads = self._detect_streams(seed, beads, stack, flatfield, darkfield)
         else:
+            fused_flat = self._fused_flat(stack, flatfield, darkfield)
             if not stack.is_cuda:
                 stack = stack.to(self.dev, non_blocking=True)
             tries = self._placement_tries()
             if tries:
-                self._trial_image_blocks(stack, flatfield, darkfield, tries[0])
+                self._trial_image_blocks(stack, flatfield, darkfield, tries[0], fused_flat)
             else:
-                self.flatfield(stack, flatfield, darkfield)
+                self._correct(stack, flatfield, darkfield, fused_flat)
             if self.mode == "P" and len(self.search_channels) == 1 and self.batch >= self.n_assays:
                 out = self._detect_reduce_on_device(seed, want_roi)
                 return self._trial_roi_sets(out, want_roi, tries[1]) if tries else out
@@ -185,7 +248,7 @@
             n_img, n_set = (int(v) for v in os.environ.get("MG_PLACEMENT_TRIES", "6,3").split(","))
         except ValueError:
             return None
-        block = self.image.numel() * self.image.element_size()
+        block = self._image.numel() * self._image.element_size()
         if (n_img < 2 and n_set < 2) or self.pool_tag or self.n_streams > 1 or block < (1 << 31):
             return None
         free, _ = torch.cuda.mem_get_info(self.dev)
@@ -207,17 +270,17 @@
             best = min(best, a.elapsed_time(b))
         return best
 
-    def _trial_image_blocks(self, stack, flatfield, darkfield, tries):
+    def _trial_image_blocks(self, stack, flatfield, darkfield, tries, fused_flat=None):
         blocks, times = [], []
         for k in range(tries):
             if k:
                 try:
-                    self.image = torch.empty_like(self.image)
+                    self._image = torch.empty_like(self._image)
                 except torch.OutOfMemoryError:
                     break
-            blocks.append(self.image)
-            times.append(self._timed(lambda: self.flatfield(stack, flatfield, darkfield)))
-        self.image = blocks[int(np.argmin(times))]
+            blocks.append(self._image)
+            times.append(self._timed(lambda: self._correct(stack, flatfield, darkfield, fused_flat)))
+        self._image = blocks[int(np.argmin(times))]
         self._trial_blocks = blocks
         self.placement.update(flatfield_ms=[round(t, 3) for t in times])
 
@@ -232,7 +295,7 @@
         counts = [len(b) for b in out["beads"]]
         res = self._trial_pairs(lambda img, tag: hp.roi_gather_reduce(
             img.view(T, C, 1, h, w), None, self.L, None, want_roi=want_roi, reuse_buffers=True, disks=True,
-            device_tables=(tabs[0], counts, self.max_r), pool_tag=tag), tries, markers=int(sum(counts)))
+            device_tables=(tabs[0], counts, self.max_r), pool_tag=tag, raw=self._raw), tries, markers=int(sum(counts)))
         res["beads"] = out["beads"]
         return res
 
@@ -255,35 +318,36 @@
                 roi_ms = None
         if roi_ms is None:
             hp.drop_pool_tags(tags)
-            self.image = blocks[int(np.argmin(flat_ms))]
+            self._image = blocks[int(np.argmin(flat_ms))]
             del blocks
             torch.cuda.empty_cache()
             self.placement.update(image_block=int(np.argmin(flat_ms)), roi_ms=None, roi_set=None)
-            return run(self.image, self.pool_tag)
+            return run(self._image, self.pool_tag)
         total = np.asarray(roi_ms) + np.asarray(flat_ms)[:, None]
         bi, bj = (int(v) for v in np.unravel_index(int(np.argmin(total)), total.shape))
         hp.drop_pool_tags([t for k, t in enumerate(tags) if k != bj])
-        self.image, self.pool_tag = blocks[bi], tags[bj]
+        self._image, self.pool_tag = blocks[bi], tags[bj]
         del blocks
         torch.cuda.empty_cache()
         self.placement.update(roi_ms=[[round(t, 3) for t in row] for row in roi_ms], image_block=bi, roi_set=bj)
-        return run(self.image, self.pool_tag)
+        return run(self._image, self.pool_tag)
 
     def _detect_reduce_on_device(self, seed, want_roi):
         T, C, h, w = self.T, self.C, self.h, self.w
         ch = self.search_channels[0]
         seeds = [(seed + 1000003 * a) & 0xFFFFFFFFFFFFFFFF for a in range(self.n_assays)]
         roi_pass = lambda d_out, d_num, cap: hp.roi_gather_reduce(
-            self.image.view(T, C, 1, h, w), None, self.L, None, want_roi=want_roi, reuse_buffers=True, disks=True,
-            device_tables=(d_out, None, self.max_r), device_counts=(d_num, cap, self._roi_bound), pool_tag=self.pool_tag)
-        counts, (d_beads, d_scores, _) = self.finder.find(self.image[:, ch], self.minmax[:, ch], self.low_q,
+            self._image.view(T, C, 1, h, w), None, self.L, None, want_roi=want_roi, reuse_buffers=True, disks=True,
+            device_tables=(d_out, None, self.max_r), device_counts=(d_num, cap, self._roi_bound), pool_tag=self.pool_tag,
+            raw=self._raw)
+        counts, (d_beads, d_scores, _) = self.finder.find(self._image[:, ch], self._minmax[:, ch], self.low_q,
                                                            self.high_q, self.min_roundness, self.min_r, seeds,
                                                            host_results=False, follow=roi_pass, stable_input=True)
         out = hp.finish_roi(self.finder.follow_result, counts)
         if out is None:
-            out = hp.roi_gather_reduce(self.image.view(T, C, 1, h, w), None, self.L, None, want_roi=want_roi,
+            out = hp.roi_gather_reduce(self._image.view(T, C, 1, h, w), None, self.L, None, want_roi=want_roi,
                                        reuse_buffers=True, disks=True, device_tables=(d_beads, counts, self.max_r),
-                                       pool_tag=self.pool_tag)
+                                       pool_tag=self.pool_tag, raw=self._raw)
         self._roi_bound = int(1.1 * int(np.sum(counts))) + 16 * self.n_assays
         out["beads"] = [r[0] for r in self.finder.fetch_results(counts, d_beads, d_scores, overlap=True)]
         return out
```

Measured after the change: 212,500, median of 6. 1.04x the previous value.
